# anuragranj/cc

Hardware: AMD Instinct MI355X
Metric: train images/sec (832x256, 5-frame sample, 6-scale CC step) (higher is better)
Workload: dtype f32; 1 GPU; full CC: DispResNet6+PoseNetB6+MaskNet6+Back2Future, all losses; per_gpu_batch=4, global_batch=4, height=256, width=832, scales=6, frames=5, parallelism=dp1, hipgraph=True, trained_nets=all, rccl_ranks=1, dead_occlusion_decoders_elided=False, net_streams=2, pipeline=per_network, grad_chunks=False, deterministic=True

## Files before the change

cc_amd/config.py:

```python
align_corners = False

strict_nan_checks = False

deterministic = True

net_streams = True


grad_chunks = False

bias_table = False

loss_stream = True


class _Debug:
    no_slice_gy = False
    no_wgrad_defer = False
    no_sum_n = False
    no_wgrad_list = False
    no_wgrad_queue = False
    force_comm = False
    capture_mode = "thread_local"
    net_stream_priority = (0, 0, 0)
    chunk_inline = False
    pipe_extra = {}
    pipe_skip_tail = ()
    reduce_trace = None
    library_path = None


debug = _Debug()
```

cc_amd/csrc/conv.hip:

```cpp
#include <stdio.h>
#include <stdlib.h>
#include <stddef.h>
#include <string.h>
#include "cc_common.h"
#include "conv_internal.h"
#include "cc_tools.h"
#include "conv_tail.h"
#include "wino_weights.h"
#include "../../include/ccengine.h"
#include <vector>
#include <string>
#include <mutex>

#ifdef CC_TOOLS
namespace cctiming {
struct Rec { std::string name; double gflop; hipEvent_t e0, e1; };
static std::vector<Rec>* recs = nullptr;
static std::mutex mtx;
Scope::Scope(const char* name, double gflop, hipStream_t st, bool active) : s(st) {
    if (!recs || !active) return;
    hipEvent_t e0 = nullptr;
    (void)hipEventCreate(&e0);
    (void)hipEventCreate(&e1);
    {
// ... 129 lines not shown
    __syncthreads();
    const int l31 = lane & 31, lk = lane >> 5;
    for (int ch = 0; ch < nchunks; ch++) {
        const int buf = ch & 1;
        if (ch + 1 < nchunks) load_chunk((ch + 1) * BK);
#pragma unroll
        for (int ks = 0; ks < BK / 2; ks++) {
            float af[TM], bf[TN];
#pragma unroll
            for (int a = 0; a < TM; a++) af[a] = As[buf][(2 * ks + lk) * AP + wm * WM + a * 32 + l31];
#pragma unroll
            for (int b = 0; b < TN; b++) bf[b] = Bs[buf][(2 * ks + lk) * BN + wn * WN + b * 32 + l31];
#pragma unroll
            for (int a = 0; a < TM; a++)
#pragma unroll
                for (int b = 0; b < TN; b++)
                    acc[a][b] = __builtin_amdgcn_mfma_f32_32x32x2f32(af[a], bf[b], acc[a][b], 0, 0, 0);
        }
        if (ch + 1 < nchunks) store_chunk(buf ^ 1);
        __syncthreads();
    }

    const int y_cs = g.OH * g.OW;
#pragma unroll
    for (int b = 0; b < TN; b++) {
        const long p = p0 + wn * WN + b * 32 + l31;
        if (p >= Ntot) continue;
        const int n = (int)(p / HWt);
        const int t = (int)(p - (long)n * HWt);
        const int ty = t / g.OWt, tx = t - ty * g.OWt;
        const long pix = (long)(g.oy0 + g.so * ty) * g.OW + (g.ox0 + g.so * tx);
        float* yb = g.y + (long)n * g.y_bs + pix;
        const float* rbp = g.res ? g.res + (long)n * g.res_bs + pix : nullptr;
        const float* abp = g.add ? g.add + (long)n * g.add_bs + pix : nullptr;
#pragma unroll
        for (int a = 0; a < TM; a++) {
#pragma unroll
            for (int r = 0; r < 16; r++) {
                const int m = m0 + wm * WM + a * 32 + (r & 3) + 8 * (r >> 2) + 4 * lk;
                if (m < g.M) {
                    float v = acc[a][b][r];
                    if (g.bias) v += g.bias[m];
                    yb[(long)m * y_cs] = conv_tail(v, rbp != nullptr, rbp ? rbp[(long)m * y_cs] : 0.f, g.res_mul, g.act, g.act_a, g.act_b,
                                                   abp ? abp[(long)m * y_cs] : 0.f);
                }
            }
        }
    }
}

constexpr int TH = 4, TW = 32;

struct CP {
    const float* x; const float* wp; const float* zeros; const float* bias; const float* res; float* y; float* part;
    int B, Cin, IH, IW; long x_bs;
    int M, Mpad, Cpad;
    int Rt, St, si, dstep, dy_base, dx_base, ymin, xmin;
    int PH, PWr, PS;
    int tw16;
    int ipt, phi;
    int aligned, shift;
    int OHt, OWt, so, oy0, ox0, OH, OW; long y_bs, res_bs;
    int tiles_x, tiles_y;
    int nsplit, cps; long part_stride;
    int act; float act_a, act_b;
    int res_mul;
    const float* add; long add_bs;
    int vec4;
    int wmajor;
};

__global__ __launch_bounds__(256) void k_repack_w(const float* __restrict__ w, float* __restrict__ wp, float* __restrict__ zeros,
                                                  int M, int Cin, int Mpad, int Cpad, int T, int St, long w_sm, long w_sc,
                                                  int w0, int w_ri, int w_sj) {
    const long e = (long)blockIdx.x * 256 + threadIdx.x;
    if (blockIdx.x == 0 && threadIdx.x < 64) zeros[threadIdx.x] = 0.f;
    const long tot = (long)T * Cpad * Mpad;
    if (e >= tot) return;
    const int m = (int)(e % Mpad);
    const long r = e / Mpad;
    const int c = (int)(r % Cpad), t = (int)(r / Cpad);
    const int i = t / St, j = t - i * St;
    wp[e] = (m < M && c < Cin) ? w[(long)w0 + (long)m * w_sm + (long)c * w_sc + i * w_ri + j * w_sj] : 0.f;
}

__host__ __device__ inline int repack_ct(int T) { const int ct = 72 / T; return ct < 1 ? 1 : (ct > 64 ? 64 : ct); }
inline long repack_blocks(int Mpad, int Cpad, int T) {
    const int ct = repack_ct(T);
    return (long)((Mpad + 63) / 64) * ((Cpad + ct - 1) / ct);
}

template <int TC>
__device__ __forceinline__ void repack_body(const long* __restrict__ d, float* tile, int bid) {
    const float* __restrict__ w = reinterpret_cast<const float*>(d[0]);
    float* __restrict__ wp = reinterpret_cast<float*>(d[1]);
    const int M = (int)d[2], Cin = (int)d[3], Mpad = (int)d[4], Cpad = (int)d[5], St = (int)d[7];
    const int T = TC > 0 ? TC : (int)d[6];
    const long w_sm = d[8], w_sc = d[9], w0 = d[10], w_ri = d[11], w_sj = d[12];
    const int CT = repack_ct(T);
    const int nmt = (Mpad + 63) / 64;
    const int m0 = (bid % nmt) * 64, c0 = (bid / nmt) * CT;
    const int CTT = CT * T, n = 64 * CTT;
    const bool m_slow = w_sm > w_sc;
    for (int e0 = threadIdx.x; e0 < n; e0 += 8 * 256) {
        float v[8];
        int li[8];
#pragma unroll
// ... 216 lines not shown
                                bf[ks][1] = Pl[(4 * ks) * g.PS + (STK ? poff[1] : half)];
                            }
#pragma unroll
                            for (int ks = 0; ks < CK / 4; ks++) {
                                acc16[0] = __builtin_amdgcn_mfma_f32_16x16x4f32(af[ks], bf[ks][0], acc16[0], 0, 0, 0);
                                acc16[1] = __builtin_amdgcn_mfma_f32_16x16x4f32(af[ks], bf[ks][1], acc16[1], 0, 0, 0);
                            }
                            if (++tj == g.St) { tj = 0; ti++; }
                            continue;
                        }
                        const float* Pl = Pb + lk * g.PS + (STK ? 0 : (g.si * (rowstep * row0 + lr)) * g.PWr + g.si * lc) + tapoff;
                        const float* Al = Ab + lk * BM + wm * WM + l31;
                        float af[CK / 2][TM], bf[CK / 2][TN];
#pragma unroll
                        for (int ks = 0; ks < CK / 2; ks++) {
#ifdef CC_ABLATE_LDS
#pragma unroll
                            for (int a = 0; a < TM; a++) af[ks][a] = 1e-3f * (float)((lane & 7) + a);
#pragma unroll
                            for (int b = 0; b < TN; b++) bf[ks][b] = 1e-3f * (float)((lane & 3) + b);
#else
#pragma unroll
                            for (int a = 0; a < TM; a++) af[ks][a] = Al[(2 * ks) * BM + a * 32];
#pragma unroll
                            for (int b = 0; b < TN; b++) bf[ks][b] = Pl[(2 * ks) * g.PS + (STK ? poff[b] : (g.si * rowstep * b) * g.PWr)];
#endif
                        }
#pragma unroll
                        for (int ks = 0; ks < CK / 2; ks++) {
#pragma unroll
                            for (int a = 0; a < TM; a++)
#pragma unroll
                                for (int b = 0; b < TN; b++)
#ifdef CC_ABLATE_MFMA
                                    acc[a][b][0] = fmaf(af[ks][a], bf[ks][b], acc[a][b][0]);
#else
                                    acc[a][b] = __builtin_amdgcn_mfma_f32_32x32x2f32(af[ks][a], bf[ks][b], acc[a][b], 0, 0, 0);
#endif
                        }
                        if (++tj == g.St) { tj = 0; ti++; }
                    }
                }
                CC_WAIT_VMCNT0();
#ifndef CC_ABLATE_BARRIER
                __syncthreads();
#endif
            }
        }
    }

    const int y_cs = g.OH * g.OW;
    if constexpr (BM == 16) {
        const int HWt = g.OHt * g.OWt;
#pragma unroll
        for (int h = 0; h < 2; h++) {
            int ej, ty;
            if (!rowmap(ty0 + rowstep * row0 + (g.tw16 ? h : 0), ej, ty)) continue;
            const int tx = tx0 + (g.tw16 ? 0 : 16 * h) + (lane & 15);
            if (ty >= g.OHt || tx >= g.OWt) continue;
            const int n = STK ? n_tile + ej : n_tile;
            const long pix = (long)(g.oy0 + g.so * ty) * g.OW + (g.ox0 + g.so * tx);
#pragma unroll
            for (int r = 0; r < 4; r++) {
                const int m = m0 + 4 * (lane >> 4) + r;
                if (m >= g.M) continue;
                if (SPLIT == 1 || (SPLIT == 2 && g.nsplit > 1)) {
                    const int Wp16 = g.tiles_x * (g.tw16 ? 16 : TW), Hp16 = g.tiles_y * (g.tw16 ? 8 : TH);
                    g.part[(long)bz_in * g.part_stride + (((long)n * g.M + m) * Hp16 + ty) * Wp16 + tx] = abl_fix(acc16[h][r]);
                } else {
                    float v = abl_fix(acc16[h][r]);
                    if (g.bias) v += g.bias[m];
                    const long o = (long)n * g.y_bs + pix + (long)m * y_cs;
                    const bool hr = g.res != nullptr;
                    g.y[o] = conv_tail(v, hr, hr ? g.res[(long)n * g.res_bs + pix + (long)m * y_cs] : 0.f, g.res_mul, g.act, g.act_a, g.act_b,
                                       g.add ? g.add[(long)n * g.add_bs + pix + (long)m * y_cs] : 0.f);
                }
            }
        }
        return;
    }
    float* Tt = smem + wid * 1024;
    const int c4 = (lane & 7) * 4, rsub = lane >> 3;
    const int lr4 = g.tw16 ? (c4 >> 4) : 0, lc4 = g.tw16 ? (c4 & 15) : c4;
    const int tx = tx0 + lc4;
    const int Wp = g.tiles_x * (g.tw16 ? 16 : TW), Hp = g.tiles_y * (g.tw16 ? 8 : TH);
    const bool split = (SPLIT == 1 || (SPLIT == 2 && g.nsplit > 1));
    const bool vec = g.vec4 != 0;
    auto stage = [&](const f32x16& A) {
#pragma unroll
        for (int r = 0; r < 16; r++) Tt[((r & 3) + 8 * (r >> 2) + 4 * lk) * 32 + l31] = abl_fix(A[r]);
        __builtin_amdgcn_wave_barrier();
    };
    if (split) {
        auto tile = [&](const f32x16& A, const int a, const int b) {
            stage(A);
            int ej, ty;
            const bool rowok = rowmap(ty0 + rowstep * (row0 + b) + lr4, ej, ty);
            const bool live = rowok && ty < g.OHt && tx < g.OWt;
            float* pb = g.part + (long)bz_in * g.part_stride + (((long)(n + ej) * g.M + (m0 + wm * WM + a * 32 + rsub)) * Hp + ty) * Wp + tx;
            const long mstep = (long)8 * Hp * Wp;
#pragma unroll
            for (int k = 0; k < 4; k++) {
                const float4 v = *reinterpret_cast<const float4*>(&Tt[(8 * k + rsub) * 32 + c4]);
                if (m0 + wm * WM + a * 32 + 8 * k + rsub < g.M && live) {
                    *reinterpret_cast<float4*>(pb + k * mstep) = v;
#ifdef CC_ABLATE_STORE
                    *reinterpret_cast<volatile float4*>(pb + k * mstep) = v;
#endif
                }
            }
            __builtin_amdgcn_wave_barrier();
        };
        tile(acc[0][0], 0, 0);
        if constexpr (TN > 1) tile(acc[0][1], 0, 1);
        if constexpr (TM > 1) {
            tile(acc[1][0], 1, 0);
            if constexpr (TN > 1) tile(acc[1][1], 1, 1);
        }
        return;
    }
    const bool hr = g.res != nullptr, ha = g.add != nullptr;
    auto tile = [&](const f32x16& A, const int a, const int b) {
        stage(A);
        int ej, ty;
        const bool rowok = rowmap(ty0 + rowstep * (row0 + b) + lr4, ej, ty);
        const bool inside = rowok && ty < g.OHt && tx < g.OWt;
        const int n = STK ? n_tile + ej : n_tile;
        const long pix = (long)(g.oy0 + g.so * ty) * g.OW + (g.ox0 + g.so * tx);
#pragma unroll
        for (int k = 0; k < 4; k++) {
            const float4 v = *reinterpret_cast<const float4*>(&Tt[(8 * k + rsub) * 32 + c4]);
            const int m = m0 + wm * WM + a * 32 + 8 * k + rsub;
            if (m < g.M && inside) {
                const long o = (long)m * y_cs + pix;
                const float bias = g.bias ? g.bias[m] : 0.f;
                const float v0 = v.x + bias, v1 = v.y + bias, v2 = v.z + bias, v3 = v.w + bias;
                if (vec && tx + 3 < g.OWt) {
                    float4 rr = make_float4(0.f, 0.f, 0.f, 0.f), aa = rr;
                    if (hr) rr = *reinterpret_cast<const float4*>(g.res + (long)n * g.res_bs + o);
                    if (ha) aa = *reinterpret_cast<const float4*>(g.add + (long)n * g.add_bs + o);
                    float4 out;
                    out.x = conv_tail(v0, hr, rr.x, g.res_mul, g.act, g.act_a, g.act_b, aa.x);
                    out.y = conv_tail(v1, hr, rr.y, g.res_mul, g.act, g.act_a, g.act_b, aa.y);
                    out.z = conv_tail(v2, hr, rr.z, g.res_mul, g.act, g.act_a, g.act_b, aa.z);
                    out.w = conv_tail(v3, hr, rr.w, g.res_mul, g.act, g.act_a, g.act_b, aa.w);
                    *reinterpret_cast<float4*>(g.y + (long)n * g.y_bs + o) = out;
#ifdef CC_ABLATE_STORE
                    *reinterpret_cast<volatile float4*>(g.y + (long)n * g.y_bs + o) = out;
#endif
                } else {
                    const long st = g.so;
                    float* yo = g.y + (long)n * g.y_bs + o;
                    const float* ro = hr ? g.res + (long)n * g.res_bs + o : nullptr;
                    const float* ao = ha ? g.add + (long)n * g.add_bs + o : nullptr;
                    yo[0] = conv_tail(v0, hr, hr ? ro[0] : 0.f, g.res_mul, g.act, g.act_a, g.act_b, ao ? ao[0] : 0.f);
                    if (tx + 1 < g.OWt) yo[st] = conv_tail(v1, hr, hr ? ro[st] : 0.f, g.res_mul, g.act, g.act_a, g.act_b, ao ? ao[st] : 0.f);
                    if (tx + 2 < g.OWt) yo[2 * st] = conv_tail(v2, hr, hr ? ro[2 * st] : 0.f, g.res_mul, g.act, g.act_a, g.act_b, ao ? ao[2 * st] : 0.f);
                    if (tx + 3 < g.OWt) yo[3 * st] = conv_tail(v3, hr, hr ? ro[3 * st] : 0.f, g.res_mul, g.act, g.act_a, g.act_b, ao ? ao[3 * st] : 0.f);
                }
            }
        }
        __builtin_amdgcn_wave_barrier();
    };
    tile(acc[0][0], 0, 0);
    if constexpr (TN > 1) tile(acc[0][1], 0, 1);
    if constexpr (TM > 1) {
        tile(acc[1][0], 1, 0);
        if constexpr (TN > 1) tile(acc[1][1], 1, 1);
    }
}

__device__ __forceinline__ void conv_xcd_blocks(int wmajor, int& bx, int& by, int& bz) {
    bx = (int)blockIdx.x; by = (int)blockIdx.y; bz = (int)blockIdx.z;
    if constexpr (!(CC_XCD_MASK & 1)) return;
    if (wmajor < 0) return;
    if (wmajor) {
        const int gx = (int)gridDim.x, gy = (int)gridDim.y;
        const int w = cc_xcd_order(bx + gx * (by + gy * bz), gx * gy * (int)gridDim.z);
        const int r = w / gx;
        bx = w - r * gx;
        bz = r / gy;
        by = r - bz * gy;
    } else {
        bx = cc_xcd_order(bx, (int)gridDim.x);
    }
}

#ifndef CC_PATCH_LB
#define CC_PATCH_LB 4
#endif
template <int BM, int CK, int TPS, int SPLIT>
__global__ __launch_bounds__(256, CC_PATCH_LB) void k_conv_patch(CP g) {
    int bx, by, bz;
    conv_xcd_blocks(g.wmajor, bx, by, bz);
    conv_patch_body<BM, CK, TPS, SPLIT, 0>(g, bx, by, bz);
}
template <int BM, int TPS, int SPLIT>
__global__ __launch_bounds__(256, CC_PATCH_LB) void k_conv_patch_stk(CP g) {
    int bx, by, bz;
    conv_xcd_blocks(g.wmajor, bx, by, bz);
    conv_patch_body<BM, 8, TPS, SPLIT, 1>(g, bx, by, bz);
}

constexpr int MAXCLS = 12;
struct CPM {
    CP c[MAXCLS];
    int n;
    int bx_end[MAXCLS];
    int wmajor;
};

#if defined(__HIP_DEVICE_COMPILE__) && !defined(CC_HIPEMU)
#define CC_MULTI_DESC(a, k) (*(reinterpret_cast<const CP*>((const char*)__builtin_amdgcn_kernarg_segment_ptr() + offsetof(CPM, c)) + (k)))
#else
#define CC_MULTI_DESC(a, k) ((a).c[k])
#endif
#define CC_MULTI_BODY(BM_, CK_, TPS_, STK_)                                                                                   \
    int bx, by, bz;                                                                                                           \
    conv_xcd_blocks(a.wmajor ? 1 : -1, bx, by, bz);        \
    int k = 0, first = 0, end = a.bx_end[0];                                                                                  \
    _Pragma("unroll") for (int q = 0; q < MAXCLS - 1; q++)                                                                    \
        if (q + 1 < a.n && bx >= a.bx_end[q]) { k = q + 1; first = a.bx_end[q]; end = a.bx_end[q + 1]; }                      \
    const CP& g = CC_MULTI_DESC(a, k);                                                                                        \
    if (bz >= g.nsplit || by * BM_ >= g.Mpad) return;                             \
    bx -= first;                                                                                                              \
    if ((CC_XCD_MASK & 1) && !a.wmajor) bx = cc_xcd_order(bx, end - first);                                                   \
    conv_patch_body<BM_, CK_, TPS_, 2, STK_>(g, bx, by, bz);

template <int BM, int CK, int TPS>
__global__ __launch_bounds__(256, CC_PATCH_LB) void k_conv_patch_multi(CPM a) { CC_MULTI_BODY(BM, CK, TPS, 0) }
template <int BM, int TPS>
__global__ __launch_bounds__(256, CC_PATCH_LB) void k_conv_patch_multi_stk(CPM a) { CC_MULTI_BODY(BM, 8, TPS, 1) }

__global__ __launch_bounds__(256) void k_splitk_epilogue(const float* __restrict__ part, int nsplit, long part_stride,
                                                         const float* __restrict__ bias, const float* __restrict__ res,
                                                         float* __restrict__ y, int M, int OHt, int OWt, int so, int oy0,
                                                         int ox0, int OH, int OW, long y_bs, long res_bs, long total,
                                                         int act, float act_a, float act_b, int res_mul,
                                                         const float* add, long add_bs, int Hp, int Wp) {
    const long e = (long)blockIdx.x * 256 + threadIdx.x;
    if (e >= total) return;
    const int HWt = OHt * OWt;
    const long per = (long)M * HWt;
    const int n = (int)(e / per);
    const long r = e - (long)n * per;
    const int m = (int)(r / HWt);
    const int t = (int)(r - (long)m * HWt);
    const int ty = t / OWt, tx = t - ty * OWt;
    const long po = (((long)n * M + m) * Hp + ty) * Wp + tx;
    float v = 0.f;
    {
        for (int k = 0; k < nsplit; k += 8) {
            float p8[8];
#pragma unroll
            for (int u = 0; u < 8; u++) p8[u] = (k + u < nsplit) ? part[(long)(k + u) * part_stride + po] : 0.f;
#pragma unroll
            for (int u = 0; u < 8; u++)
                if (k + u < nsplit) v += p8[u];
        }
    }
    const long o = (long)m * OH * OW + (long)(oy0 + so * ty) * OW + (ox0 + so * tx);
    if (bias) v += bias[m];
    y[(long)n * y_bs + o] = conv_tail(v, res != nullptr, res ? res[(long)n * res_bs + o] : 0.f, res_mul, act, act_a, act_b,
                                      add ? add[(long)n * add_bs + o] : 0.f);
}

struct EPC {
    const float* part; const float* bias; const float* res; const float* add; float* y;
    int nsplit; long part_stride; int OHt, OWt, oy0, ox0; long total;
    int Hp, Wp;
    int M, so, OH, OW; long y_bs, res_bs, add_bs;
    int act; float act_a, act_b;
    int res_mul;
};
struct EPM {
    EPC c[MAXCLS];
    int n;
    int bx_end[MAXCLS];
};

__global__ __launch_bounds__(256) void k_splitk_epilogue_multi(EPM a) {
    int k = 0, first = 0;
#pragma unroll
    for (int q = 0; q < MAXCLS - 1; q++)
        if (q + 1 < a.n && (int)blockIdx.x >= a.bx_end[q]) { k = q + 1; first = a.bx_end[q]; }
    const EPC& c = a.c[k];
    const long e = (long)((int)blockIdx.x - first) * 256 + threadIdx.x;
    if (e >= c.total) return;
    const int HWt = c.OHt * c.OWt;
    const long per = (long)c.M * HWt;
    const int n = (int)(e / per);
    const long r = e - (long)n * per;
    const int m = (int)(r / HWt);
    const int t = (int)(r - (long)m * HWt);
    const int ty = t / c.OWt, tx = t - ty * c.OWt;
    const long po = (((long)n * c.M + m) * c.Hp + ty) * c.Wp + tx;
    float v = 0.f;
    {
        for (int z = 0; z < c.nsplit; z += 8) {
            float p8[8];
#pragma unroll
            for (int u = 0; u < 8; u++) p8[u] = (z + u < c.nsplit) ? c.part[(long)(z + u) * c.part_stride + po] : 0.f;
#pragma unroll
            for (int u = 0; u < 8; u++)
                if (z + u < c.nsplit) v += p8[u];
        }
    }
    const long o = (long)m * c.OH * c.OW + (long)(c.oy0 + c.so * ty) * c.OW + (c.ox0 + c.so * tx);
    if (c.bias) v += c.bias[m];
    c.y[(long)n * c.y_bs + o] = conv_tail(v, c.res != nullptr, c.res ? c.res[(long)n * c.res_bs + o] : 0.f, c.res_mul, c.act, c.act_a, c.act_b,
                                          c.add ? c.add[(long)n * c.add_bs + o] : 0.f);
}


struct ConvPlan {
    bool use_patch;
    int wino;
    ccint::WinoPlan wn;
    int Hp, Wp;
    int tw16;
    int ipt, phi;
    int bm, ck, tps, Mpad, Cpad, PH, PWr, PS, ymin, xmin, tiles_x, tiles_y, nsplit, cps, aligned, shift;
    size_t smem, wp_floats, part_floats;
    int wpad;
    size_t pad_floats;
};


inline long conv_tiles(const GG& g, const ConvPlan& p) { return (long)((g.B + p.ipt - 1) / p.ipt) * p.tiles_x * p.tiles_y; }

inline bool wino_geometry(const GG& g) {
    return g.Rt == 3 && g.St == 3 && g.si == 1 && g.so == 1 && g.oy0 == 0 && g.ox0 == 0 && (g.dstep == 1 || g.dstep == -1) &&
           g.dy0 == -g.dstep && g.dx0 == -g.dstep && g.IH == g.OH && g.IW == g.OW && g.OHt == g.OH && g.OWt == g.OW && g.Cin > 0 &&
           (long)g.B * g.Cin * g.IH * g.IW < (1l << 26);
}

inline ConvPlan plan_conv(const GG& g, int mult = 1) {
    ConvPlan p = {};
    p.ipt = 1;
    if (wino_geometry(g)) {
        const ccint::WinoPlan w = ccint::wino_plan(g.B, g.Cin, g.IH, g.IW, g.M, mult);
        if (w.ok) {
            p.wino = 1;
            p.wn = w;
            p.use_patch = true;
            p.bm = ccwino::WBM; p.ck = ccwino::WCK; p.tps = 1;
            p.Mpad = w.Mpad; p.Cpad = w.Cpad;
            p.nsplit = w.nsplit; p.cps = w.cps;
            p.Hp = w.Hp; p.Wp = w.Wp;
            p.wp_floats = w.u_floats;
            p.part_floats = w.part_floats;
            return p;
        }
        if (!cctools::env_flag("CC_NO_WINO_PAD") && (g.IW % 4) != 0 && g.IH >= 2 && g.M >= cctools::env_int("CC_WINOP_MINM", 256) &&
            g.Cin >= cctools::env_int("CC_WINOP_MINC", 256)) {
            int wp = (g.IW + 3) & ~3;
            while (!(wp / 2 >= 16 || wp / 2 == 8)) wp += 4;
            if (4 * (wp - g.IW) <= wp && (long)g.B * ((g.IH + 1) / 2) * (wp / 2) >= cctools::env_int("CC_WINOP_MINQ", 64)) {
                ccint::WinoPlan wq = ccint::wino_plan(g.B, g.Cin, g.IH, wp, g.M, mult);
                if (wq.ok) {
                    if (wq.nsplit < 2) {
                        if (wq.tile == 2) wq.tile = 1;
                        wq.cps = (wq.nchunk + 1) / 2;
                        wq.nsplit = (wq.nchunk + wq.cps - 1) / wq.cps;
// ... 158 lines not shown
template <int BM, int CK, int TPS>
inline void launch_patch(const CP& c, dim3 grid, size_t smem, hipStream_t s) {
    if constexpr (CK == 8) {
        if (stacked(c)) {
            if (c.nsplit > 1) launch_patch1_stk<BM, TPS, 1>(c, grid, smem, s);
            else launch_patch1_stk<BM, TPS, 0>(c, grid, smem, s);
            return;
        }
    }
    if (c.nsplit > 1) launch_patch1<BM, CK, TPS, 1>(c, grid, smem, s);
    else launch_patch1<BM, CK, TPS, 0>(c, grid, smem, s);
}

template <int BM, int CK, int TPS>
inline void launch_patch(const CPM& c, dim3 grid, size_t smem, hipStream_t s) {
    if constexpr (CK == 8) {
        if (stacked(c)) {
            static bool big = false;
            launch_patch_kernel(&k_conv_patch_multi_stk<BM, TPS>, big, c, grid, smem, s);
            return;
        }
    }
    static bool big = false;
    launch_patch_kernel(&k_conv_patch_multi<BM, CK, TPS>, big, c, grid, smem, s);
}

template <class ARGS>
inline void dispatch_patch(int bm, int ck, int tps, const ARGS& c, dim3 grid, size_t smem, hipStream_t s) {
    if (tps == 3) {
        if (ck == 16) {
            if (bm == 128) launch_patch<128, 16, 3>(c, grid, smem, s);
            else if (bm == 64) launch_patch<64, 16, 3>(c, grid, smem, s);
            else if (bm == 32) launch_patch<32, 16, 3>(c, grid, smem, s);
            else launch_patch<16, 16, 3>(c, grid, smem, s);
        } else {
            if (bm == 128) launch_patch<128, 8, 3>(c, grid, smem, s);
            else if (bm == 64) launch_patch<64, 8, 3>(c, grid, smem, s);
            else if (bm == 32) launch_patch<32, 8, 3>(c, grid, smem, s);
            else launch_patch<16, 8, 3>(c, grid, smem, s);
        }
    } else if (ck == 16) {
        if (bm == 128) launch_patch<128, 16, 1>(c, grid, smem, s);
        else if (bm == 64) launch_patch<64, 16, 1>(c, grid, smem, s);
        else if (bm == 32) launch_patch<32, 16, 1>(c, grid, smem, s);
        else launch_patch<16, 16, 1>(c, grid, smem, s);
    } else {
        if (bm == 128) launch_patch<128, 8, 1>(c, grid, smem, s);
        else if (bm == 64) launch_patch<64, 8, 1>(c, grid, smem, s);
        else if (bm == 32) launch_patch<32, 8, 1>(c, grid, smem, s);
        else launch_patch<16, 8, 1>(c, grid, smem, s);
    }
}

inline CP make_cp(const GG& g, const ConvPlan& p, const float* zeros, const float* wp, float* part) {
    CP c = {};
    c.x = g.x; c.wp = wp; c.zeros = zeros; c.bias = g.bias; c.res = g.res; c.y = g.y; c.part = part;
    c.B = g.B; c.Cin = g.Cin; c.IH = g.IH; c.IW = g.IW; c.x_bs = g.x_bs;
    c.M = g.M; c.Mpad = p.Mpad; c.Cpad = p.Cpad;
    c.Rt = g.Rt; c.St = g.St; c.si = g.si; c.dstep = g.dstep;
    c.dy_base = g.dy0 - p.ymin; c.dx_base = g.dx0 - p.xmin; c.ymin = p.ymin; c.xmin = p.xmin;
    c.PH = p.PH; c.PWr = p.PWr; c.PS = p.PS; c.tw16 = p.tw16; c.ipt = p.ipt; c.phi = p.phi; c.aligned = p.aligned; c.shift = p.shift;
    c.OHt = g.OHt; c.OWt = g.OWt; c.so = g.so; c.oy0 = g.oy0; c.ox0 = g.ox0; c.OH = g.OH; c.OW = g.OW;
    c.y_bs = g.y_bs; c.res_bs = g.res_bs;
    c.tiles_x = p.tiles_x; c.tiles_y = p.tiles_y;
    c.nsplit = p.nsplit; c.cps = p.cps;
    c.part_stride = (long)g.B * g.M * (p.tiles_y * (p.tw16 ? 8 : TH)) * (p.tiles_x * (p.tw16 ? 16 : TW));
    c.act = g.act; c.act_a = g.act_a; c.act_b = g.act_b; c.res_mul = g.res_mul;
    c.add = g.add; c.add_bs = g.add_bs;
#ifndef CC_CONV_WMAJOR
#define CC_CONV_WMAJOR 1
#endif
    c.wmajor = (CC_CONV_WMAJOR && (long)g.M * g.Rt * g.St > (long)g.B * g.IH * g.IW) ? 1 : 0;
    c.vec4 = (g.so == 1) && ((g.OW & 3) == 0) && ((g.ox0 & 3) == 0) && ((((uintptr_t)g.y) & 15) == 0) && ((g.y_bs & 3) == 0) &&
             (!g.res || ((((uintptr_t)g.res) & 15) == 0 && (g.res_bs & 3) == 0)) &&
             (!g.add || ((((uintptr_t)g.add) & 15) == 0 && (g.add_bs & 3) == 0));
    return c;
}

inline ccint::WinoGeom wino_geom(const GG& g) {
    ccint::WinoGeom w = {};
    w.B = g.B; w.Cin = g.Cin; w.H = g.IH; w.W = g.IW; w.x_bs = g.x_bs; w.M = g.M; w.y_bs = g.y_bs; w.res_bs = g.res_bs; w.add_bs = g.add_bs;
    w.act = g.act; w.act_a = g.act_a; w.act_b = g.act_b; w.res_mul = g.res_mul;
    return w;
}

inline void wino_scope_name(const GG& g, const ConvPlan& p, int nprob, char* nm, int cap) {
    int nl = p.wn.tile ? snprintf(nm, cap, "k_wino_f2x3_s<%d, %d>", p.wn.tile, p.nsplit > 1 ? 1 : 0)
                       : snprintf(nm, cap, "k_wino_f2x3<%d>", p.nsplit > 1 ? 1 : 0);
    if (cctools::env_flag("CC_TIMING_DETAIL"))
        snprintf(nm + nl, cap - nl, " %dx[B%d M%d C%d %dx%d%s t9 k%d] wg%d", nprob, g.B, g.M, g.Cin, g.OH, g.OW, p.wpad ? "(pad)" : "", p.nsplit,
                 nprob * p.wn.nqb * p.wn.nmb * p.nsplit);
}

inline double wino_gflop(const GG& g, const ConvPlan& p) { return 2e-9 * 16.0 * g.B * p.wn.TY * p.wn.TX * (double)g.M * g.Cin; }

inline int wino_flip(const GG& g) { return g.dstep < 0 ? 1 : 0; }

struct PadTab { ccint::PadJob j[2 * MAXGRP]; int n, B, W, Wp; long row_end[2 * MAXGRP]; };
__global__ __launch_bounds__(256) void k_pad_rows(PadTab t) {
    const int q4 = t.Wp >> 2;
    const long e = (long)blockIdx.x * 256 + threadIdx.x;
    const long row = e / q4;
    const int c4 = (int)(e - row * q4) * 4;
    int k = 0;
    long first = 0;
#pragma unroll
    for (int q = 0; q < 2 * MAXGRP - 1; q++)
        if (q + 1 < t.n && row >= t.row_end[q]) { k = q + 1; first = t.row_end[q]; }
    if (row >= t.row_end[t.n - 1]) return;
    const ccint::PadJob& j = t.j[k];
    const long r = row - first;
    const int n = (int)(r / j.rows_per_image);
    const long rr = r - (long)n * j.rows_per_image;
    const float* s = j.src + (long)n * j.bs + rr * t.W;
    float4 v;
    v.x = c4 + 0 < t.W ? s[c4 + 0] : 0.f;
    v.y = c4 + 1 < t.W ? s[c4 + 1] : 0.f;
    v.z = c4 + 2 < t.W ? s[c4 + 2] : 0.f;
    v.w = c4 + 3 < t.W ? s[c4 + 3] : 0.f;
    *reinterpret_cast<float4*>(j.dst + (r * t.Wp + c4)) = v;
}
}

void ccint::pad_rows_launch(const PadJob* jobs, int n, int B, int W, int Wp, hipStream_t s) {
    PadTab t = {};
    t.n = n; t.B = B; t.W = W; t.Wp = Wp;
    long rows = 0;
    for (int k = 0; k < n; k++) {
        t.j[k] = jobs[k];
        rows += (long)B * jobs[k].rows_per_image;
        t.row_end[k] = rows;
    }
    const long nf4 = rows * (Wp >> 2);
    hipLaunchKernelGGL(k_pad_rows, dim3((unsigned)((nf4 + 255) / 256)), dim3(256), 0, s, t);
}

namespace {

inline void wino_pad_input(const GG& g, const ConvPlan& p, float* part, hipStream_t s, ccint::WinoProb& pr, ccint::WinoGeom& wg) {
    float* xpad = part + p.part_floats;
    const ccint::PadJob job = {g.x, xpad, g.x_bs, g.Cin * g.IH};
    ccint::pad_rows_launch(&job, 1, g.B, g.IW, p.wpad, s);
    if (cctools::env_flag("CC_WINO_TRACE"))
        fprintf(stderr, "wino padded input: B%d M%d C%d %dx%d -> pitch %d, nsplit %d dstep %d\n", g.B, g.M, g.Cin, g.IH, g.IW, p.wpad, p.nsplit, g.dstep);
    pr.x = xpad;
    wg.W = p.wpad;
    wg.x_bs = (long)g.Cin * g.IH * p.wpad;
}

inline int head_kernel_of(const GG& g, ccint::HeadConv& h) {
    static const int off = cctools::env_int("CC_NO_HEAD_KERNELS", 0);
    if (off == 1 || (g.Cin > 4 && g.M > 4) || g.Cin < 1 || g.Rt != 3 || g.St != 3 || g.si != 1 || g.so != 1 || g.oy0 != 0 || g.ox0 != 0) return 0;
    if (g.OHt != g.OH || g.OWt != g.OW || g.OH != g.IH || g.OW != g.IW || g.w_ri != 3 || g.w_sj != 1) return 0;
    if (!((g.dstep == 1 && g.dy0 == -1 && g.dx0 == -1) || (g.dstep == -1 && g.dy0 == 1 && g.dx0 == 1))) return 0;
    if (g.res_mul && !g.res) return 0;
    h = ccint::HeadConv{g.x, g.w, g.bias, g.res, g.res_mul ? g.add : nullptr, g.y, g.B, g.Cin, g.IH, g.IW, g.M, g.x_bs, g.y_bs, g.res_bs,
                        g.add_bs, g.w_sm, g.w_sc, (long)g.w0, g.dstep, g.act, g.act_a, g.act_b, g.res_mul};
    if (g.Cin <= 4 && off != 3 && ccint::head_conv_thinc_vec(h) != 0) return 1;
    if (g.M <= 4 && off != 2 && ccint::head_conv_thinm_ok(h)) return 2;
    return 0;
}

inline void launch_gg(const GG& g, float* ws, hipStream_t s, const float* prepacked = nullptr, const float* pre_zeros = nullptr) {
    {
        ccint::HeadConv h;
        const int hk = head_kernel_of(g, h);
        if (hk) {
            char nm[96];
            int nl = snprintf(nm, sizeof nm, hk == 1 ? "k_conv_thinc<%d>" : "k_conv_thinm<%d>", hk == 1 ? g.Cin : g.M);
            if (cctools::env_flag("CC_TIMING_DETAIL"))
                snprintf(nm + nl, sizeof nm - nl, " B%d M%d C%d %dx%d t9", g.B, g.M, g.Cin, g.OHt, g.OWt);
            cctiming::Scope tsc(nm, 2e-9 * g.B * g.OHt * g.OWt * (double)g.M * g.Cin * 9, s);
            if (cctools::env_flag("CC_HEAD_TRACE"))
                fprintf(stderr, "head kernel %d: B%d M%d C%d %dx%d dstep %d\n", hk, g.B, g.M, g.Cin, g.OHt, g.OWt, g.dstep);
            if (hk == 1 ? ccint::head_conv_thinc_launch(h, s) : ccint::head_conv_thinm_launch(h, s)) return;
        }
    }
    const ConvPlan p = plan_conv(g);
    if (!p.use_patch || ws == nullptr) { launch_gg_flat(g, s); return; }
    const float* zeros = ws;
    const float* wp = ws + 64;
    float* part = ws + 64 + (prepacked ? 0 : p.wp_floats);
    const int T = g.Rt * g.St;
    if (p.wino) {
        if (!prepacked)
            ccint::wino_weights_launch(g.w, ws + 64, g.M, g.Cin, p.Cpad, p.Mpad, g.w_sm, g.w_sc, g.w0, g.w_ri, g.w_sj, wino_flip(g), s);
        ccint::WinoProb pr = {g.x, prepacked ? prepacked : wp, g.bias, g.res, g.add, g.y, part};
        ccint::WinoGeom wg = wino_geom(g);
        if (p.wpad) wino_pad_input(g, p, part, s, pr, wg);
        bool ok;
        {
            char nm[128];
            wino_scope_name(g, p, 1, nm, sizeof nm);
            cctiming::Scope tsc(nm, wino_gflop(g, p), s);
            ok = ccint::wino_launch(wg, p.wn, &pr, 1, s);
        }
        if (!ok) { launch_gg_flat(g, s); return; }
        if (p.nsplit > 1) {
            const long total = (long)g.B * g.M * g.OHt * g.OWt;
            hipLaunchKernelGGL(k_splitk_epilogue, dim3((unsigned)((total + 255) / 256)), dim3(256), 0, s, (const float*)part,
                               p.nsplit, (long)g.B * g.M * p.Hp * p.Wp, g.bias, g.res, g.y, g.M, g.OHt, g.OWt, g.so, g.oy0, g.ox0, g.OH,
                               g.OW, g.y_bs, g.res_bs, total, g.act, g.act_a, g.act_b, g.res_mul, g.add, g.add_bs, p.Hp, p.Wp);
        }
        return;
    }
    if (prepacked) {
        zeros = pre_zeros;
        wp = prepacked;
    } else {
        hipLaunchKernelGGL(k_repack_w, dim3((unsigned)((p.wp_floats + 255) / 256)), dim3(256), 0, s, g.w, ws + 64, ws, g.M, g.Cin,
                           p.Mpad, p.Cpad, T, g.St, g.w_sm, g.w_sc, g.w0, g.w_ri, g.w_sj);
    }
    const CP c = make_cp(g, p, zeros, wp, part);
    dim3 grid((unsigned)conv_tiles(g, p), (unsigned)(p.Mpad / p.bm), (unsigned)p.nsplit);
    {
        char nm[96];
        int nl = p.ipt > 1 ? snprintf(nm, sizeof nm, "k_conv_patch_stk<%d, %d, %d>", p.bm, p.tps, p.nsplit > 1 ? 1 : 0)
                           : snprintf(nm, sizeof nm, "k_conv_patch<%d, %d, %d, %d>", p.bm, p.ck, p.tps, p.nsplit > 1 ? 1 : 0);
        if (cctools::env_flag("CC_TIMING_DETAIL"))
            snprintf(nm + nl, sizeof nm - nl, " B%d M%d C%d %dx%d t%d k%d wg%d", g.B, g.M, g.Cin, g.OHt, g.OWt, g.Rt * g.St, p.nsplit,
                     (int)(grid.x * grid.y * grid.z));
        cctiming::Scope tsc(nm, 2e-9 * g.B * g.OHt * g.OWt * (double)g.M * g.Cin * g.Rt * g.St, s);
        dispatch_patch(p.bm, p.ck, p.tps, c, grid, p.smem, s);
    }
    if (p.nsplit > 1) {
        const long total = (long)g.B * g.M * g.OHt * g.OWt;
        hipLaunchKernelGGL(k_splitk_epilogue, dim3((unsigned)((total + 255) / 256)), dim3(256), 0, s, (const float*)part,
                           p.nsplit, c.part_stride, g.bias, g.res, g.y, g.M, g.OHt, g.OWt, g.so, g.oy0, g.ox0, g.OH, g.OW,
                           g.y_bs, g.res_bs, total, g.act, g.act_a, g.act_b, g.res_mul, g.add, g.add_bs,
                           p.Hp, p.Wp);
    }
}

struct ClsIn { GG g; ConvPlan p; const float* zeros; const float* wp; float* part; };

inline size_t smem_cls(const ConvPlan& p, int tps) {
    const size_t b = (size_t)(2 * tps * p.ck * p.bm + 2 * p.ck * p.PS) * sizeof(float);
    return (p.bm >= 32 && b < 16384) ? 16384 : b;
}

inline bool same_problem_shape(const GG& a, const GG& b) {
    return a.B == b.B && a.Cin == b.Cin && a.IH == b.IH && a.IW == b.IW && a.x_bs == b.x_bs && a.M == b.M && a.y_bs == b.y_bs &&
           a.res_bs == b.res_bs && a.add_bs == b.add_bs && a.act == b.act && a.act_a == b.act_a && a.act_b == b.act_b &&
           a.res_mul == b.res_mul && a.dstep == b.dstep;
}

inline bool launch_classes(const ClsIn* cs, int n, hipStream_t s, bool idle_taps = false) {
    if (n < 1 || n > MAXCLS) return false;
    {
        int nw = 0;
        for (int k = 0; k < n; k++) nw += cs[k].p.wino ? 1 : 0;

        if (nw) {
            if (nw != n) return false;
            ccint::WinoProb pr[MAXCLS];
            EPM e = {};
            e.n = n;
            int ebx = 0;
            const ConvPlan& p = cs[0].p;
            for (int k = 0; k < n; k++) {
                const GG& g = cs[k].g;
                if (!cs[k].wp || !same_problem_shape(g, cs[0].g) || cs[k].p.nsplit != p.nsplit || cs[k].p.cps != p.cps) {
                    if (cctools::env_flag("CC_WINO_TRACE"))
                        fprintf(stderr, "wino classes declined: k %d wp %p same %d nsplit %d/%d cps %d/%d\n", k, (const void*)cs[k].wp,
                                (int)same_problem_shape(g, cs[0].g), cs[k].p.nsplit, p.nsplit, cs[k].p.cps, p.cps);
                    return false;
                }
                pr[k] = ccint::WinoProb{g.x, cs[k].wp, g.bias, g.res, g.add, g.y, cs[k].part};
                EPC& c = e.c[k];
                c.part = cs[k].part; c.bias = g.bias; c.res = g.res; c.add = g.add; c.y = g.y;
                c.Hp = p.Hp; c.Wp = p.Wp;
                c.part_stride = (long)g.B * g.M * c.Hp * c.Wp;
                c.nsplit = p.nsplit;
                c.OHt = g.OHt; c.OWt = g.OWt; c.oy0 = g.oy0; c.ox0 = g.ox0;
                c.total = p.nsplit > 1 ? (long)g.B * g.M * g.OHt * g.OWt : 0;
                c.M = g.M; c.so = g.so; c.OH = g.OH; c.OW = g.OW; c.y_bs = g.y_bs; c.res_bs = g.res_bs; c.add_bs = g.add_bs;
                c.act = g.act; c.act_a = g.act_a; c.act_b = g.act_b; c.res_mul = g.res_mul;
                ebx += (int)((c.total + 255) / 256);
                e.bx_end[k] = ebx;
            }
            ccint::WinoGeom wg = wino_geom(cs[0].g);
            if (p.wpad) {
                for (int k = 0; k < n; k++)
                    if (cs[k].p.wpad != p.wpad || cs[k].p.part_floats != p.part_floats || !cs[k].part) return false;
                for (int k0 = 0; k0 < n; k0 += 2 * MAXGRP) {
                    ccint::PadJob jobs[2 * MAXGRP];
                    int nj = 0;
                    for (int k = k0; k < n && k < k0 + 2 * MAXGRP; k++) {
                        const GG& g = cs[k].g;
                        float* xpad = cs[k].part + p.part_floats;
                        jobs[nj++] = ccint::PadJob{g.x, xpad, g.x_bs, g.Cin * g.IH};
                        pr[k].x = xpad;
                    }
                    ccint::pad_rows_launch(jobs, nj, cs[0].g.B, cs[0].g.IW, p.wpad, s);
                }
                wg.W = p.wpad;
                wg.x_bs = (long)cs[0].g.Cin * cs[0].g.IH * p.wpad;
                if (cctools::env_flag("CC_WINO_TRACE"))
                    fprintf(stderr, "wino padded input, %d problems: B%d M%d C%d %dx%d -> pitch %d, nsplit %d\n", n, cs[0].g.B, cs[0].g.M,
                            cs[0].g.Cin, cs[0].g.IH, cs[0].g.IW, p.wpad, p.nsplit);
            }
            {
                char nm[128];
                wino_scope_name(cs[0].g, p, n, nm, sizeof nm);
                cctiming::Scope tsc(nm, n * wino_gflop(cs[0].g, p), s);
                if (!ccint::wino_launch(wg, p.wn, pr, n, s)) return false;
            }
            if (p.nsplit > 1) hipLaunchKernelGGL(k_splitk_epilogue_multi, dim3((unsigned)ebx), dim3(256), 0, s, e);
            return true;
        }
    }
    size_t smem = 0;
    int tps = 3, maxsplit = 1, maxy = 1, ref = -1;
    if (cctools::env_int("CC_CONV_IDLE_TAPS", 1)) idle_taps = true;
    for (int k = 0; k < n; k++) {
        const ConvPlan& p = cs[k].p;
        if (cs[k].g.Cin == 0) continue;
        if (ref < 0) ref = k;
        if (!p.use_patch || p.bm != cs[ref].p.bm || p.ck != cs[ref].p.ck || !cs[k].wp) return false;
        if (p.tps != 3 && !(idle_taps && cs[k].g.Rt * cs[k].g.St < 3 && smem_cls(p, 3) <= 80 * 1024)) tps = 1;
        if (p.nsplit > maxsplit) maxsplit = p.nsplit;
        if (p.Mpad / p.bm > maxy) maxy = p.Mpad / p.bm;
    }
    CPM a = {};
    EPM e = {};
    e.n = n;
    int bx = 0, ebx = 0, epi_any = 0, nc = 0;
    double gf = 0;
    for (int k = 0; k < n; k++) {
        const GG& g = cs[k].g;
        const ConvPlan& p = cs[k].p;
        const bool empty = g.Cin == 0;
        EPC& c = e.c[k];
        c.part = empty ? nullptr : cs[k].part; c.bias = g.bias; c.res = g.res; c.add = g.add; c.y = g.y;
        c.Hp = empty ? g.OHt : p.Hp;
        c.Wp = empty ? g.OWt : p.Wp;
        c.part_stride = (long)g.B * g.M * c.Hp * c.Wp;
        c.nsplit = empty ? 0 : p.nsplit;
        c.OHt = g.OHt; c.OWt = g.OWt; c.oy0 = g.oy0; c.ox0 = g.ox0;
        c.total = (empty || p.nsplit > 1) ? (long)g.B * g.M * g.OHt * g.OWt : 0;
        c.M = g.M; c.so = g.so; c.OH = g.OH; c.OW = g.OW; c.y_bs = g.y_bs; c.res_bs = g.res_bs; c.add_bs = g.add_bs;
        c.act = g.act; c.act_a = g.act_a; c.act_b = g.act_b; c.res_mul = g.res_mul;
        ebx += (int)((c.total + 255) / 256);
        e.bx_end[k] = ebx;
        if (c.total) epi_any = 1;
        if (empty) continue;
        const size_t sm = smem_cls(p, tps);
        if (sm > smem) smem = sm;
        a.c[nc] = make_cp(g, p, cs[k].zeros, cs[k].wp, cs[k].part);
        bx += (int)conv_tiles(g, p);
        a.bx_end[nc] = bx;
        nc++;
        gf += 2e-9 * g.B * g.OHt * g.OWt * (double)g.M * g.Cin * g.Rt * g.St;
    }
    a.n = nc;
    {
        double wf = 0, xf = 0;
        for (int k = 0; k < nc; k++) {
            const CP& c = a.c[k];
            wf += (double)c.M * c.Cin * c.Rt * c.St;
            xf += (double)c.B * c.Cin * c.IH * c.IW;
        }
        a.wmajor = (CC_CONV_WMAJOR && wf > xf) ? 1 : 0;
    }
    if (smem > 80 * 1024) return false;
    if (nc > 0) {
        dim3 grid((unsigned)bx, (unsigned)maxy, (unsigned)maxsplit);
        char nm[224];
        int nl = stacked(a) ? snprintf(nm, sizeof nm, "k_conv_patch_multi_stk<%d, %d>", cs[ref].p.bm, tps)
                            : snprintf(nm, sizeof nm, "k_conv_patch_multi<%d, %d, %d>", cs[ref].p.bm, cs[ref].p.ck, tps);
        if (cctools::env_flag("CC_TIMING_DETAIL")) {
            for (int k = 0; k < n && nl < (int)sizeof nm - 48; k++) {
                const GG& g = cs[k].g;
                if (g.Cin == 0) continue;
                int same = 0, first = 1;
                for (int j = 0; j < n; j++) {
                    const GG& h = cs[j].g;
                    const bool eq = h.Cin == g.Cin && h.M == g.M && h.OHt == g.OHt && h.OWt == g.OWt && h.Rt * h.St == g.Rt * g.St &&
                                    cs[j].p.nsplit == cs[k].p.nsplit;
                    if (eq) { same++; if (j < k) first = 0; }
                }
                if (!first) continue;
                nl += snprintf(nm + nl, sizeof nm - nl, " %dx[B%d M%d C%d %dx%d t%d k%d]", same, g.B, g.M, g.Cin, g.OHt, g.OWt,
                               g.Rt * g.St, cs[k].p.nsplit);
            }
            snprintf(nm + nl, sizeof nm - nl, " wg%d", (int)(grid.x * grid.y * grid.z));
        }
        cctiming::Scope tsc(nm, gf, s);
        dispatch_patch(cs[ref].p.bm, cs[ref].p.ck, tps, a, grid, smem, s);
    }
    if (epi_any) hipLaunchKernelGGL(k_splitk_epilogue_multi, dim3((unsigned)ebx), dim3(256), 0, s, e);
    return true;
}

inline bool launch_gg_classes(const GG* gs, int n, int mult, const float* const* zeros, const float* const* wps,
                              float* const* parts, hipStream_t s) {
    if (n < 2 || n > MAXCLS || cctools::env_flag("CC_NO_CLASS_MERGE")) return false;
    ClsIn cs[MAXCLS];
    for (int k = 0; k < n; k++) {
        cs[k].g = gs[k];
        cs[k].p = plan_conv(gs[k], mult);
        cs[k].zeros = zeros[k]; cs[k].wp = wps[k]; cs[k].part = parts[k];
    }
    return launch_classes(cs, n, s);
}

}

extern "C" {

static GG make_fwd(const float* x, const float* w, const float* bias, const float* res, float* y, int B, int Cin, int IH,
                   int IW, long x_bs, int Cout, int R, int S, int stride, int pad, int OH, int OW, long y_bs, long res_bs,
                   int act, float act_a, float act_b) {
    GG g = {};
    g.x = x; g.w = w; g.bias = bias; g.res = res; g.y = y;
    g.B = B; g.Cin = Cin; g.IH = IH; g.IW = IW; g.x_bs = x_bs;
    g.M = Cout; g.w_sm = (long)Cin * R * S; g.w_sc = (long)R * S; g.w0 = 0; g.w_ri = S; g.w_sj = 1;
    g.Rt = R; g.St = S; g.dy0 = -pad; g.dx0 = -pad; g.dstep = 1; g.si = stride;
    g.OHt = OH; g.OWt = OW; g.so = 1; g.oy0 = 0; g.ox0 = 0; g.OH = OH; g.OW = OW; g.y_bs = y_bs; g.res_bs = res_bs;
    g.act = act; g.act_a = act_a; g.act_b = act_b;
    return g;
}

static void fill_desc(const GG& g, const ConvPlan& p, long src, long dst, long* d) {
    if (p.wino) {
        d[0] = src; d[1] = dst; d[2] = g.M; d[3] = g.Cin; d[4] = p.Mpad; d[5] = p.Cpad; d[6] = ccwino::WINO_T; d[7] = wino_flip(g) ? -3 : 3;
        d[8] = g.w_sm; d[9] = g.w_sc; d[10] = g.w0; d[11] = g.w_ri; d[12] = g.w_sj; d[13] = (long)p.wp_floats; d[14] = 0;
        d[15] = ccwino::wino_weight_blocks(p.Mpad, p.Cpad);
        return;
    }
    d[0] = src; d[1] = dst; d[2] = g.M; d[3] = g.Cin; d[4] = p.Mpad; d[5] = p.Cpad; d[6] = (long)g.Rt * g.St; d[7] = g.St;
    d[8] = g.w_sm; d[9] = g.w_sc; d[10] = g.w0; d[11] = g.w_ri; d[12] = g.w_sj; d[13] = (long)p.wp_floats; d[14] = 0;
    d[15] = repack_blocks(p.Mpad, p.Cpad, g.Rt * g.St);
}

size_t cc_conv2d_fwd_pack_floats(int B, int Cin, int IH, int IW, int Cout, int R, int S, int stride, int pad, int OH, int OW) {
    GG g = make_fwd(nullptr, nullptr, nullptr, nullptr, nullptr, B, Cin, IH, IW, 0, Cout, R, S, stride, pad, OH, OW, 0, 0, 0,
                    1.f, 0.f);
    const ConvPlan p = plan_conv(g);
    return (p.use_patch && R * S <= 136) ? 64 + p.wp_floats : 0;
}

int cc_conv2d_fwd_pack_desc(int B, int Cin, int IH, int IW, int Cout, int R, int S, int stride, int pad, int OH, int OW,
                            long src_ptr, long pack_base_ptr, long* desc_out_host) {
    GG g = make_fwd(nullptr, nullptr, nullptr, nullptr, nullptr, B, Cin, IH, IW, 0, Cout, R, S, stride, pad, OH, OW, 0, 0, 0,
                    1.f, 0.f);
    const ConvPlan p = plan_conv(g);
    if (!p.use_patch) return 0;
    fill_desc(g, p, src_ptr, pack_base_ptr + 64 * (long)sizeof(float), desc_out_host);
    return 1;
}

size_t cc_conv2d_fwd_ws_bytes(int B, int Cin, int IH, int IW, int Cout, int R, int S, int stride, int pad, int OH, int OW) {
    GG g = make_fwd(nullptr, nullptr, nullptr, nullptr, nullptr, B, Cin, IH, IW, 0, Cout, R, S, stride, pad, OH, OW, 0, 0, 0,
                    1.f, 0.f);
    return conv_ws_floats(plan_conv(g)) * sizeof(float);
}
// ... 86 lines not shown
            if (!p.use_patch) return 0;
            tot += p.wp_floats;
        }
    return tot;
}

int cc_conv2d_dgrad_pack_desc(int B, int K, int OH, int OW, int C, int R, int S, int stride, int pad, int IH, int IW,
                              long w_k_stride, long w_c_stride, long src_ptr, long pack_base_ptr, long* desc_out_host) {
    int n = 0;
    long off = 64;
    for (int py = 0; py < stride; py++)
        for (int px = 0; px < stride; px++) {
            GG g;
            if (!make_dgrad_class(g, py, px, nullptr, nullptr, nullptr, nullptr, B, K, OH, OW, 0, C, R, S, stride, pad, IH, IW, 0,
                                  w_k_stride, w_c_stride, 0, 1.f, 0.f))
                continue;
            if (g.Cin == 0) continue;
            const ConvPlan p = plan_conv(g);
            if (!p.use_patch) return 0;
            fill_desc(g, p, src_ptr, pack_base_ptr + off * (long)sizeof(float), desc_out_host + 16 * n);
            off += (long)p.wp_floats;
            n++;
        }
    return n;
}

int cc_repack_table(const long* table_dev, int ndesc, long total_blocks, void* stream) {
    if (ndesc <= 0 || total_blocks <= 0) return CC_ERR_ARG;
    hipLaunchKernelGGL(k_repack_table, dim3((unsigned)total_blocks), dim3(256), 0, (hipStream_t)stream, table_dev, ndesc);
    CC_CHECK_LAUNCH();
    return CC_OK;
}

size_t cc_conv2d_dgrad_group_ws_bytes(int G, int B, int K, int OH, int OW, int C, int R, int S, int stride, int pad, int IH, int IW) {
    size_t best = 0;
    for (int mult = 1; mult <= G; mult += (G > 1 ? G - 1 : 1)) {
        size_t wmax = 0, psum = 0;
        for (int py = 0; py < stride; py++)
            for (int px = 0; px < stride; px++) {
                GG g;
                if (!make_dgrad_class(g, py, px, nullptr, nullptr, nullptr, nullptr, B, K, OH, OW, 0, C, R, S, stride, pad, IH, IW,
                                      0, (long)C * R * S, (long)R * S, 0, 1.f, 0.f))
                    continue;
                const ConvPlan p = plan_conv(g, mult);
                if (p.wp_floats > wmax) wmax = p.wp_floats;
                psum += p.part_floats + p.pad_floats;
            }
        const size_t t = 64 + wmax + psum;
        if (t > best) best = t;
    }
    return (size_t)G * best * sizeof(float);
}

static int dgrad_group_impl(int G, const long* gy, const long* w, const long* bias, const long* gx, const long* mul,
                            const long* add, float* ws, const long* prepacked, int B, int K, int OH, int OW, long gy_bs, int C,
                            int R, int S, int stride, int pad, int IH, int IW, long gx_bs, long mul_bs, long add_bs,
                            long w_k_stride, long w_c_stride, int act, float act_a, float act_b, void* stream) {
    if (G <= 0 || G > MAXCLS || B <= 0 || K <= 0 || C <= 0 || stride <= 0) return CC_ERR_ARG;
    hipStream_t s = (hipStream_t)stream;
    const size_t stride_f = cc_conv2d_dgrad_group_ws_bytes(G, B, K, OH, OW, C, R, S, stride, pad, IH, IW) / sizeof(float) / G;
    bool packed = true;
    for (int k = 0; k < G; k++)
        if (!prepacked || !prepacked[k]) packed = false;
    const int ncls = stride * stride;
    if (packed && ws && G * ncls >= 2 && G * ncls <= MAXCLS) {
        GG gs[MAXCLS];
        const float *zeros[MAXCLS], *wps[MAXCLS];
        float* parts[MAXCLS];
        int n = 0;
        bool all = true;
        for (int k = 0; k < G && all; k++) {
            const float* pk = (const float*)prepacked[k];
            long off = 64;
            float* part = ws + k * stride_f + 64;
            for (int py = 0; py < stride && all; py++)
                for (int px = 0; px < stride; px++) {
                    if (!make_dgrad_class(gs[n], py, px, (const float*)gy[k], (const float*)w[k],
                                          bias ? (const float*)bias[k] : nullptr, (float*)gx[k], B, K, OH, OW, gy_bs, C, R, S,
                                          stride, pad, IH, IW, gx_bs, w_k_stride, w_c_stride, act, act_a, act_b,
                                          mul ? (const float*)mul[k] : nullptr, mul_bs)) { all = false; break; }
                    if (add && add[k]) {
                        if (mul && mul[k]) { gs[n].add = (const float*)add[k]; gs[n].add_bs = add_bs; }
                        else { gs[n].res = (const float*)add[k]; gs[n].res_bs = add_bs; gs[n].res_mul = 0; }
                    }
                    const ConvPlan p = plan_conv(gs[n], G);
                    zeros[n] = pk;
                    wps[n] = pk + off;
                    parts[n] = part;
                    off += (long)p.wp_floats;
                    part += p.part_floats;
                    n++;
                }
        }
        if (all && launch_gg_classes(gs, n, G, zeros, wps, parts, s)) {
            CC_CHECK_LAUNCH();
            return CC_OK;
        }
    }
    for (int k = 0; k < G; k++) {
        const float* pk = prepacked ? (const float*)prepacked[k] : nullptr;
        float* wk = ws ? ws + k * stride_f : nullptr;
        long off = 64;
        for (int py = 0; py < stride; py++) {
            for (int px = 0; px < stride; px++) {
                GG g;
                if (!make_dgrad_class(g, py, px, (const float*)gy[k], (const float*)w[k], bias ? (const float*)bias[k] : nullptr,
                                      (float*)gx[k], B, K, OH, OW, gy_bs, C, R, S, stride, pad, IH, IW, gx_bs, w_k_stride,
                                      w_c_stride, act, act_a, act_b, mul ? (const float*)mul[k] : nullptr, mul_bs))
                    continue;
                if (add && add[k]) {
                    if (mul && mul[k]) { g.add = (const float*)add[k]; g.add_bs = add_bs; }
                    else { g.res = (const float*)add[k]; g.res_bs = add_bs; g.res_mul = 0; }
                }
                if (g.Cin == 0) {
                    const long total = (long)g.B * g.M * g.OHt * g.OWt;
                    hipLaunchKernelGGL(k_splitk_epilogue, dim3((unsigned)((total + 255) / 256)), dim3(256), 0, s, (const float*)nullptr,
                                       0, total, g.bias, g.res, g.y, g.M, g.OHt, g.OWt, g.so, g.oy0, g.ox0, g.OH, g.OW, g.y_bs, g.res_bs,
                                       total, g.act, g.act_a, g.act_b, g.res_mul, g.add, g.add_bs, g.OHt, g.OWt);
                } else if (pk) {
                    const ConvPlan p = plan_conv(g);
                    launch_gg(g, wk, s, pk + off, pk);
                    off += (long)p.wp_floats;
                } else {
                    launch_gg(g, wk, s);
                }
            }
        }
    }
    CC_CHECK_LAUNCH();
    return CC_OK;
}

int cc_conv2d_dgrad_group(int G, const long* gy, const long* w, const long* bias, const long* gx, const long* mul, float* ws,
                          const long* prepacked, int B, int K, int OH, int OW, long gy_bs, int C, int R, int S, int stride,
                          int pad, int IH, int IW, long gx_bs, long mul_bs, long w_k_stride, long w_c_stride, int act, float act_a,
                          float act_b, void* stream) {
    return dgrad_group_impl(G, gy, w, bias, gx, mul, nullptr, ws, prepacked, B, K, OH, OW, gy_bs, C, R, S, stride, pad, IH, IW, gx_bs,
                            mul_bs, 0, w_k_stride, w_c_stride, act, act_a, act_b, stream);
}

int cc_conv2d_dgrad_group_add(int G, const long* gy, const long* w, const long* gx, const long* mul, const long* add, float* ws,
                              const long* prepacked, int B, int K, int OH, int OW, long gy_bs, int C, int R, int S, int stride,
                              int pad, int IH, int IW, long gx_bs, long mul_bs, long add_bs, long w_k_stride, long w_c_stride,
                              int act, float act_a, float act_b, void* stream) {
    return dgrad_group_impl(G, gy, w, nullptr, gx, mul, add, ws, prepacked, B, K, OH, OW, gy_bs, C, R, S, stride, pad, IH, IW, gx_bs,
                            mul_bs, add_bs, w_k_stride, w_c_stride, act, act_a, act_b, stream);
}

int cc_conv2d_dgrad(const float* gy, const float* w, const float* bias_or_null, float* gx, float* ws,
                    const float* prepacked_or_null, int B, int K, int OH, int OW, long gy_bs, int C, int R, int S, int stride,
                    int pad, int IH, int IW, long gx_bs, long w_k_stride, long w_c_stride, int act, float act_a, float act_b,
                    void* stream) {
    const long gyp = (long)gy, wp = (long)w, bp = (long)bias_or_null, gxp = (long)gx, pk = (long)prepacked_or_null;
    return cc_conv2d_dgrad_group(1, &gyp, &wp, &bp, &gxp, nullptr, ws, &pk, B, K, OH, OW, gy_bs, C, R, S, stride, pad, IH, IW, gx_bs,
                                 0, w_k_stride, w_c_stride, act, act_a, act_b, stream);
}

constexpr int CL_LONGS = 32;
struct ListCls { ClsIn c; int prob; };

static float bits_to_float(long v) { unsigned u = (unsigned)v; float f; memcpy(&f, &u, 4); return f; }

static int list_classes(int n, const long* d, std::vector<ListCls>& out) {
    for (int i = 0; i < n; i++) {
        const long* r = d + (long)i * CL_LONGS;
        const float act_a = bits_to_float(r[24]), act_b = bits_to_float(r[25]);
        const int B = (int)r[8], Ci = (int)r[9], H0 = (int)r[10], W0 = (int)r[11], Co = (int)r[13], R = (int)r[14], S = (int)r[15];
        const int stride = (int)r[16], pad = (int)r[17], H1 = (int)r[18], W1 = (int)r[19];
        if (B <= 0 || Ci <= 0 || Co <= 0 || R <= 0 || S <= 0 || stride <= 0 || !r[6]) return -1;
        const float* pk = (const float*)r[6];
        if (r[0] == 0) {
            ListCls lc = {};
            lc.c.g = make_fwd((const float*)r[1], (const float*)r[2], (const float*)r[3], (const float*)r[4], (float*)r[5], B, Ci, H0, W0,
                              r[12], Co, R, S, stride, pad, H1, W1, r[20], r[21], (int)r[23], act_a, act_b);
            lc.c.p = plan_conv(lc.c.g);
            lc.c.zeros = pk; lc.c.wp = pk + 64; lc.prob = i;
            out.push_back(lc);
        } else {
            long off = 64;
            for (int py = 0; py < stride; py++)
                for (int px = 0; px < stride; px++) {
                    ListCls lc = {};
                    if (!make_dgrad_class(lc.c.g, py, px, (const float*)r[1], (const float*)r[2], (const float*)r[3], (float*)r[5], B, Ci, H0,
                                          W0, r[12], Co, R, S, stride, pad, H1, W1, r[20], r[26], r[27], (int)r[23], act_a, act_b,
                                          (const float*)r[4], r[21]))
                        continue;
                    lc.c.g.add = (const float*)r[7]; lc.c.g.add_bs = r[22];
                    if (lc.c.g.add && !lc.c.g.res_mul) return -1;
                    lc.c.p = plan_conv(lc.c.g);
                    lc.c.zeros = pk; lc.c.wp = pk + off; lc.prob = i;
                    off += (long)lc.c.p.wp_floats;
                    out.push_back(lc);
                }
        }
    }
    return (int)out.size();
}

static void list_plan_splits(ListCls** cls, int n, int target) {
// ... 196 lines not shown
```

cc_amd/csrc/conv_internal.h:

```cpp
#pragma once
#include <stddef.h>
#include <hip/hip_runtime.h>

namespace cctiming {
#ifdef CC_TOOLS
struct Scope {
    hipEvent_t e1 = nullptr;
    hipStream_t s;
    Scope(const char* name, double gflop, hipStream_t st, bool active = true);
    ~Scope();
};
#else
struct Scope { Scope(const char*, double, hipStream_t, bool = true) {} };
#endif
}

namespace ccint {

constexpr int MAXGRP = 4;
constexpr int BN = 128;
constexpr int BK = 16;
inline int pick_bm(int M) { return M > 64 ? 128 : (M > 32 ? 64 : 32); }

struct PadJob { const float* src; float* dst; long bs; int rows_per_image; };
void pad_rows_launch(const PadJob* jobs, int n, int B, int W, int Wp, hipStream_t s);

constexpr int RD_LONGS = 16;
struct RedSink { long* out; int cap; int n; };
int wgrad_reduce_emit(RedSink* sink, const long* desc, int n, hipStream_t s);
int wgrad_reduce_launch(const long* desc, int n, hipStream_t s);

size_t wgrad_thin_ws_floats(int B, int M, int AH, int AW, int Cin, int R, int S, int si);
bool wgrad_thin_launch(const float* a, const float* x, float* gw, float* ws, int B, int M, int AH, int AW, long a_bs, int Cin,
                       int IH, int IW, long x_bs, int R, int S, int si, int pad, long o_sm, long o_sc, int accumulate, hipStream_t s,
                       RedSink* sink = nullptr);

bool wgrad_thin_park(bool on);
bool wgrad_thin_parking();
double wgrad_thin_parked_gflop();
void wgrad_thin_flush(hipStream_t s);

void wgrad_thin_name(int B, int M, int AH, int AW, int Cin, int IH, int IW, int R, int S, int si, int pad, char* out, int cap);


struct WinoGeom {
    int B, Cin, H, W; long x_bs;
    int M; long y_bs, res_bs, add_bs;
    int act; float act_a, act_b; int res_mul;
};
struct WinoProb { const float* x; const float* U; const float* bias; const float* res; const float* add; float* y; float* part; };
struct WinoPlan {
    int ok;
    int Mpad, Cpad, nchunk;
    int TY, TX, nqb, nmb;
    int nsplit, cps;
    int Hp, Wp;
    size_t u_floats, part_floats;
    int tile;
};
constexpr int WINO_MAXP = 12;
WinoPlan wino_plan(int B, int Cin, int H, int W, int M, int mult);
bool wino_launch(const WinoGeom& g, const WinoPlan& p, const WinoProb* probs, int nprob, hipStream_t s);
void wino_weights_launch(const float* w, float* U, int M, int Cin, int Cpad, int Mpad, long w_sm, long w_sc, long w0, long w_ri,
                         long w_sj, int flip, hipStream_t s);

struct WinoWgradPlan {
    int ok;
    int TX, CPR, CPI, NCH;
    int nmb, ncb, Cp;
    int nsplit, cps;
    size_t ws_floats;
};
WinoWgradPlan wino_wgrad_plan(int B, int M, int H, int W, int Cin, int G, int minq = -1);
WinoWgradPlan wino_wgrad_plan_parked(const WinoWgradPlan& alone, int M);
constexpr int WINO_WGRAD_PARK_CAP = 96;
struct WinoWgradParked {
    struct Desc {
        const float* a; const float* x; float* ws;
        int M, C, H, W; long a_bs, x_bs; unsigned a_bytes, x_bytes;
        int TX, CPR, CPI, NCH, cps, ncb, Cp, nxy, nsplit;
        double gflop;
    };
    Desc d[WINO_WGRAD_PARK_CAP];
    int n;
};
bool wino_wgrad_launch(const WinoWgradPlan& p, const float* const* a, const float* const* x, float* const* ws, int G, int B, int M,
                       int H, int W, long a_bs, int Cin, long x_bs, hipStream_t s, WinoWgradParked* park = nullptr);
void wino_wgrad_launch_parked(WinoWgradParked* c, hipStream_t s);

struct HeadConv {
    const float* x; const float* w; const float* bias; const float* res; const float* add; float* y;
    int B, Cin, H, W, M;
    long x_bs, y_bs, res_bs, add_bs;
    long w_sm, w_sc, w0;
    int dstep;
    int act; float act_a, act_b; int res_mul;
};
int head_conv_thinc_vec(const HeadConv& g);
bool head_conv_thinc_launch(const HeadConv& g, hipStream_t s);
bool head_conv_thinm_ok(const HeadConv& g);
bool head_conv_thinm_launch(const HeadConv& g, hipStream_t s);
struct HeadWgradPlan { int ok, R, nstrips, nblk; size_t ws_floats; };
HeadWgradPlan head_wgrad_plan(int B, int M, int H, int W, int Cin);
bool head_wgrad_launch(const HeadWgradPlan& p, const float* dy, const float* x, float* ws, int B, int M, int H, int W, long dy_bs,
                       int Cin, long x_bs, hipStream_t s);

}
```

cc_amd/csrc/wgrad_reduce.hip:

```cpp
#include "cc_common.h"
#include "conv_internal.h"
#include "../../include/ccengine.h"

namespace {

constexpr int NRD = 32;

struct RD {
    const float* ws; float* gw;
    long o_sm, o_sc;
    int kind, nsplit, accum;
    int p[9];
    int blk_end;
};
struct RT { RD d[NRD]; int n; };

__device__ __forceinline__ void put(float* o, float s, int accum) { *o = accum ? (*o + s) : s; }

__global__ __launch_bounds__(256) void k_wgrad_reduce_table(RT t) {
    __shared__ float4 part[16][16];
    int k = 0, first = 0;
#pragma unroll 1
    for (int q = 0; q + 1 < t.n; q++)
        if ((int)blockIdx.x >= t.d[q].blk_end) { k = q + 1; first = t.d[q].blk_end; }
    const RD& d = t.d[k];
    const int bid = (int)blockIdx.x - first;
    const float* __restrict__ ws = d.ws;
    if (d.kind == 0) {
        const int M = d.p[0], Ntot = d.p[1], RS = d.p[2], St = d.p[3];
        const long tot = (long)M * Ntot;
        if (d.p[6]) {
            const long e = ((long)bid * 256 + threadIdx.x) * 4;
            if (e >= tot) return;
            float4 s = make_float4(0.f, 0.f, 0.f, 0.f);
            for (int z = 0; z < d.nsplit; z += 8) {
                float4 v[8];
#pragma unroll
                for (int u = 0; u < 8; u++)
                    v[u] = (z + u < d.nsplit) ? *(const float4*)(ws + (long)(z + u) * tot + e) : make_float4(0.f, 0.f, 0.f, 0.f);
#pragma unroll
                for (int u = 0; u < 8; u++)
                    if (z + u < d.nsplit) { s.x += v[u].x; s.y += v[u].y; s.z += v[u].z; s.w += v[u].w; }
            }
            float4* o = (float4*)(d.gw + e);
            if (d.accum) { const float4 g = *o; s.x = g.x + s.x; s.y = g.y + s.y; s.z = g.z + s.z; s.w = g.w + s.w; }
            *o = s;
            return;
        }
        const long e = (long)bid * 256 + threadIdx.x;
        if (e >= tot) return;
        float s = 0.f;
        for (int z = 0; z < d.nsplit; z += 8) {
            float v[8];
#pragma unroll
            for (int u = 0; u < 8; u++) v[u] = (z + u < d.nsplit) ? ws[(long)(z + u) * tot + e] : 0.f;
#pragma unroll
            for (int u = 0; u < 8; u++)
                if (z + u < d.nsplit) s += v[u];
        }
        const int m = (int)(e / Ntot), jn = (int)(e - (long)m * Ntot);
        const int c = jn / RS, rem = jn - c * RS;
        const int i = rem / St, j = rem - i * St;
        put(d.gw + (long)m * d.o_sm + (long)c * d.o_sc + i * d.p[4] + j * d.p[5], s, d.accum);
    } else if (d.kind == 1) {
        const int T = d.p[0], M = d.p[1], Cin = d.p[2], Cp32 = d.p[3];
        const long mc = (long)bid * 256 + threadIdx.x;
        const long per = (long)M * Cp32;
        if (mc >= per) return;
        const int c = (int)(mc % Cp32), m = (int)(mc / Cp32);
        if (c >= Cin) return;
        const long tot = (long)T * per;
        float* o = d.gw + (long)m * d.o_sm + (long)c * d.o_sc;
        if (T == 9) {
            float s9[9];
#pragma unroll
            for (int tt = 0; tt < 9; tt++) s9[tt] = 0.f;
            int z = 0;
            for (; z + 2 <= d.nsplit; z += 2) {
                const float* wz = ws + (long)z * tot + mc;
                float v0[9], v1[9];
#pragma unroll
                for (int tt = 0; tt < 9; tt++) { v0[tt] = wz[(long)tt * per]; v1[tt] = wz[tot + (long)tt * per]; }
#pragma unroll
                for (int tt = 0; tt < 9; tt++) { s9[tt] += v0[tt]; s9[tt] += v1[tt]; }
            }
            for (; z < d.nsplit; z++) {
                const float* wz = ws + (long)z * tot + mc;
#pragma unroll
                for (int tt = 0; tt < 9; tt++) s9[tt] += wz[(long)tt * per];
            }
#pragma unroll
            for (int tt = 0; tt < 9; tt++) put(o + tt, s9[tt], d.accum);
        } else {
            for (int tt = 0; tt < T; tt++) {
                float s = 0.f;
                for (int z = 0; z < d.nsplit; z++) s += ws[(long)z * tot + (long)tt * per + mc];
                put(o + tt, s, d.accum);
            }
        }
    } else if (d.kind == 4) {
        const int m = bid * 4 + (threadIdx.x >> 6), lane = threadIdx.x & 63;
        if (m < d.p[0]) {
            float s = 0.f;
            for (int k = lane; k < d.nsplit; k += 64) s += ws[(long)m * d.nsplit + k];
            s = cc::wave_sum(s);
            if (lane == 0) put(d.gw + m, s, d.accum);
        }
    } else {
        const int TS = d.p[0], S = d.p[1], TR = d.p[2], ngc = d.p[3], ngt = d.p[4], M = d.p[5], Cin = d.p[6], R = d.p[7];
        const int npb = d.nsplit;
        const int quarter = bid & 3, ct = bid >> 2;
        const int combo = ct / TS, tt = ct - combo * TS;
        const int sub = threadIdx.x >> 4, q = quarter * 16 + (threadIdx.x & 15);
        float4 s = make_float4(0.f, 0.f, 0.f, 0.f);
        int pb = sub;
        for (; pb + 112 < npb; pb += 128) {
            float4 v[8];
#pragma unroll
            for (int u = 0; u < 8; u++) v[u] = *(const float4*)(ws + (((long)combo * npb + pb + 16 * u) * TS + tt) * 256 + 4 * q);
#pragma unroll
            for (int u = 0; u < 8; u++) { s.x += v[u].x; s.y += v[u].y; s.z += v[u].z; s.w += v[u].w; }
        }
        for (; pb < npb; pb += 16) {
            const float4 v = *(const float4*)(ws + (((long)combo * npb + pb) * TS + tt) * 256 + 4 * q);
            s.x += v.x; s.y += v.y; s.z += v.z; s.w += v.w;
        }
        part[sub][threadIdx.x & 15] = s;
        __syncthreads();
        if (sub == 0) {
            for (int z = 1; z < 16; z++) {
                const float4 v = part[z][threadIdx.x & 15];
                s.x += v.x; s.y += v.y; s.z += v.z; s.w += v.w;
            }
            int cb = combo;
            const int tg = cb % ngt;
            cb /= ngt;
            const int cg = cb % ngc, mg = cb / ngc;
            const int r = tg * TR + tt / S, sc = tt % S;
            const int m = mg * 16 + (q >> 2), c0 = cg * 16 + (q & 3) * 4;
            if (m < M && r < R) {
                float* o = d.gw + (long)m * d.o_sm + (long)r * S + sc;
                const float v[4] = {s.x, s.y, s.z, s.w};
#pragma unroll
                for (int e = 0; e < 4; e++)
                    if (c0 + e < Cin) put(o + (long)(c0 + e) * d.o_sc, v[e], d.accum);
            }
        }
    }
}

long blocks_of(const long* h) {
    switch ((int)h[0]) {
        case 0: return h[13] ? (h[7] * h[8] / 4 + 255) / 256 : (h[7] * h[8] + 255) / 256;
        case 1: return (h[8] * h[10] + 255) / 256;
        case 2: return h[15] * h[7] * 4;
        case 4: return (h[7] + 3) / 4;
        default: return -1;
    }
}

}

namespace ccint {

int wgrad_reduce_launch(const long* desc, int n, hipStream_t s) {
    for (int b = 0; b < n; b += NRD) {
        RT t = {};
        const int m = (n - b) < NRD ? (n - b) : NRD;
        long blk = 0;
        for (int k = 0; k < m; k++) {
            const long* h = desc + (long)(b + k) * RD_LONGS;
            RD& d = t.d[k];
            d.kind = (int)h[0]; d.ws = (const float*)h[1]; d.gw = (float*)h[2]; d.nsplit = (int)h[3]; d.accum = (int)h[4];
            d.o_sm = h[5]; d.o_sc = h[6];
            for (int i = 0; i < 9; i++) d.p[i] = (int)h[7 + i];
            long hv[RD_LONGS];
            for (int i = 0; i < RD_LONGS; i++) hv[i] = h[i];
            if (d.kind == 0) {
                const long tot = h[7] * h[8];
                hv[13] = (d.o_sm == h[8] && d.o_sc == h[9] && h[11] == h[10] && h[12] == 1 && tot % 4 == 0 &&
                          ((uintptr_t)d.ws % 16 == 0) && ((uintptr_t)d.gw % 16 == 0)) ? 1 : 0;
                d.p[6] = (int)hv[13];
            }
            const long nb = blocks_of(hv);
            if (nb <= 0 || !d.ws || !d.gw || d.nsplit <= 0 || blk + nb >= (1l << 31)) return CC_ERR_ARG;
            blk += nb;
            d.blk_end = (int)blk;
        }
        t.n = m;
        hipLaunchKernelGGL(k_wgrad_reduce_table, dim3((unsigned)blk), dim3(256), 0, s, t);
    }
    return CC_OK;
}

int wgrad_reduce_emit(RedSink* sink, const long* desc, int n, hipStream_t s) {
    if (!sink) return wgrad_reduce_launch(desc, n, s);
    if (sink->n + n > sink->cap) return CC_ERR_ARG;
    for (long i = 0; i < (long)n * RD_LONGS; i++) sink->out[(long)sink->n * RD_LONGS + i] = desc[i];
    sink->n += n;
    return CC_OK;
}

}

extern "C" {

int cc_wgrad_reduce_table(const long* desc_host, int n, void* stream) {
    if (!desc_host || n <= 0) return CC_ERR_ARG;
    const int r = ccint::wgrad_reduce_launch(desc_host, n, (hipStream_t)stream);
// ... 7 lines not shown
```

cc_amd/csrc/wino.hip:

```cpp
#include <stddef.h>
#include <stdint.h>
#include <stdio.h>
#include <type_traits>
#include "cc_common.h"
#include "cc_tools.h"
#include "conv_tail.h"
#include "conv_internal.h"
#include "wino_weights.h"

namespace {

using namespace cctail;
using namespace ccwino;

typedef float f32x16 __attribute__((ext_vector_type(16)));

struct WN {
    ccint::WinoProb p[ccint::WINO_MAXP];
    int total, per_prob, nmb;
    int Cin, H, W, HW;
    unsigned x_bytes;
    long x_bs;
    int M;
    long y_bs, res_bs, add_bs;
    int TX, TPI, Q, nchunk, cps;
    long part_stride;
    int Hp, Wp;
    int act;
    float act_a, act_b;
    int res_mul, vec2;
    int mb_major;
};

constexpr int VBLK = 16 * WCK * 64;
constexpr int RROW = 12 * 4, RCH = 4 * RROW, RWAVE = 4 * RCH;
constexpr int WTHREADS = 512;

enum { EPI_LIN = 0, EPI_GRAD = 1, EPI_GEN = 2 };

template <int SPLIT, int EPI, int ABL>
__global__ __launch_bounds__(WTHREADS, 2) void k_wino_f2x3(WN g) {
    HIP_DYNAMIC_SHARED(float, smem)
    float* Us = smem;
    float* Vs = smem + 2 * UBLK;
    float* Rs = smem + 2 * UBLK + 2 * VBLK;

    const int tid = threadIdx.x, lane = tid & 63;
    const int wid = __builtin_amdgcn_readfirstlane(tid >> 6);
    const int st = wid & 3, fh = wid >> 2;
    const int wm = st >> 1, wt = st & 1;
    const int l31 = lane & 31, lk = lane >> 5;

    const int cnt = (int)gridDim.x >> 3;
    const int w = ((int)blockIdx.x & 7) * cnt + ((int)blockIdx.x >> 3);
    if (w >= g.total) return;
    const int prob = w / g.per_prob;
    const int wr = w - prob * g.per_prob;
    int qb, mb;
    if (g.mb_major) { const int nqb = g.per_prob / g.nmb; mb = wr / nqb; qb = wr - mb * nqb; }
    else { qb = wr / g.nmb; mb = wr - qb * g.nmb; }
#if defined(__HIP_DEVICE_COMPILE__) && !defined(CC_HIPEMU)
    const char* ka = (const char*)__builtin_amdgcn_kernarg_segment_ptr();
    const ccint::WinoProb& P = *(reinterpret_cast<const ccint::WinoProb*>(ka + offsetof(WN, p)) + prob);
#else
    const ccint::WinoProb& P = g.p[prob];
#endif
    const int c_beg = (int)blockIdx.z * g.cps;
    int c_end = c_beg + g.cps;
    if (c_end > g.nchunk) c_end = g.nchunk;
    const int odd = (c_end - c_beg) & 1;
    auto dma_U = [&](int kc, int buf) {
        if constexpr (ABL & 4) return;
        const float* src = P.U + ((long)mb * g.nchunk + kc) * UBLK + wid * 1024 + lane * 4;
        CC_GLDS16X4(src, Us + buf * UBLK + wid * 1024);
    };

    if (c_beg < c_end) dma_U(c_beg, odd);
    float bias_w = 0.f;
    if constexpr (!SPLIT) {
        const int mr = mb * WBM + wm * 32 + l31;
        if (P.bias) bias_w = P.bias[mr < g.M ? mr : g.M - 1];
    }

    const int tg = st, qd = fh;
    float* Rw = Rs + wid * RWAVE;
    const int q0 = qb * 64 + 16 * tg;
    int rn[2], riy[2], rxal[2], rlen[2], rjb[2], rxs[2];
    {
        int q = q0;
        int jb = 0;
#pragma unroll
        for (int r = 0; r < 2; r++) {
            const bool v = q < g.Q;
            const int qq = v ? q : 0;
// ... 131 lines not shown
        else CC_WAIT_VMCNT_FENCE(3);
        __builtin_amdgcn_s_waitcnt(0xC07F);
        __builtin_amdgcn_s_barrier();
    };

    if (c_beg < c_end) {
        CC_WAIT_VMCNT0_FENCE();
        read_raw();
#pragma unroll
        for (int b = 0; b < 4; b++) col_step(b);
#pragma unroll
        for (int i = 0; i < 4; i++) row_step(i, odd);
        __builtin_amdgcn_s_waitcnt(0xC07F);
        __builtin_amdgcn_wave_barrier();
#pragma unroll
        for (int i = 0; i < 3; i++) dma_raw(c_beg + 1, i);
        __builtin_amdgcn_s_barrier();
        int kc = c_beg;
        if (odd) {
            stage(I1(), kc);
            kc++;
        }
        for (; kc < c_end; kc += 2) {
            stage(I0(), kc);
            stage(I1(), kc + 1);
        }
    }

    if constexpr (ABL & 32) {
        if (acc[3][5] == 12345.f) P.y[tid] = acc[7][1] + acc[0][0];
        return;
    }
    auto part_tile = [&](int r, float& z00, float& z01, float& z10, float& z11) {
        float p0[4], p1[4];
#pragma unroll
        for (int j = 0; j < 4; j++) {
            if (fh == 0) { p0[j] = acc[j][r] + acc[4 + j][r]; p1[j] = acc[4 + j][r]; }
            else { p0[j] = acc[j][r]; p1[j] = (0.f - acc[j][r]) - acc[4 + j][r]; }
        }
        z00 = (p0[0] + p0[1]) + p0[2];
        z01 = (p0[1] - p0[2]) - p0[3];
        z10 = (p1[0] + p1[1]) + p1[2];
        z11 = (p1[1] - p1[2]) - p1[3];
    };
    const int q = qb * 64 + wt * 32 + l31;
    const bool qv = q < g.Q;
    const int qq = qv ? q : 0;
    const int n = qq / g.TPI;
    const int qr = qq - n * g.TPI;
    const int ty = qr / g.TX, tx = qr - ty * g.TX;
    const int oy = 2 * ty, ox = 2 * tx;
    const int m_base = mb * WBM + wm * 32 + 4 * lk;
    const bool hr = P.res != nullptr, ha = P.add != nullptr;
    const bool row1 = oy + 1 < g.H;
    const long o0 = (long)oy * g.W + ox;
    const int odd_lane = lane & 1;
    const long o4 = (long)(oy + odd_lane) * g.W + (ox - 2 * odd_lane);
    const bool row_ok = odd_lane ? row1 : true;
    float4 res_r[8], add_r[8];
    if constexpr (!SPLIT) {
#pragma unroll
        for (int r8 = 0; r8 < 8; r8++) res_r[r8] = add_r[r8] = make_float4(0.f, 0.f, 0.f, 0.f);
        if (g.vec2 && qv && row_ok) {
            if (hr) {
                const float* rb = P.res + (long)n * g.res_bs + o4;
#pragma unroll
                for (int r8 = 0; r8 < 8; r8++) {
                    const int r = 8 * fh + r8;
                    const int m = m_base + (r & 3) + 8 * (r >> 2);
                    res_r[r8] = *reinterpret_cast<const float4*>(rb + (long)(m < g.M ? m : g.M - 1) * g.HW);
                }
            }
            if (ha) {
                const float* ab = P.add + (long)n * g.add_bs + o4;
#pragma unroll
                for (int r8 = 0; r8 < 8; r8++) {
                    const int r = 8 * fh + r8;
                    const int m = m_base + (r & 3) + 8 * (r >> 2);
                    add_r[r8] = *reinterpret_cast<const float4*>(ab + (long)(m < g.M ? m : g.M - 1) * g.HW);
                }
            }
        }
    }
    float* Xs = smem;
    {
        float* xo = Xs + ((st * 2 + fh) * 32) * 64 + lane;
#pragma unroll
        for (int r8 = 0; r8 < 8; r8++) {
            const int r = 8 * (fh ^ 1) + r8;
            float z00, z01, z10, z11;
            part_tile(r, z00, z01, z10, z11);
            xo[(r8 * 4 + 0) * 64] = z00;
            xo[(r8 * 4 + 1) * 64] = z01;
            xo[(r8 * 4 + 2) * 64] = z10;
            xo[(r8 * 4 + 3) * 64] = z11;
        }
    }
    __syncthreads();
    const float* xi = Xs + ((st * 2 + (fh ^ 1)) * 32) * 64 + lane;
    auto out_tile = [&](int r8, float& y00, float& y01, float& y10, float& y11) {
        part_tile(8 * fh + r8, y00, y01, y10, y11);
        y00 += xi[(r8 * 4 + 0) * 64];
        y01 += xi[(r8 * 4 + 1) * 64];
        y10 += xi[(r8 * 4 + 2) * 64];
        y11 += xi[(r8 * 4 + 3) * 64];
    };
    auto pair4 = [&](float y00, float y01, float y10, float y11) -> float4 {
        const float sx = odd_lane ? y00 : y10, sy = odd_lane ? y01 : y11;
        const float rx = __shfl_xor(sx, 1), ry = __shfl_xor(sy, 1);
        return odd_lane ? make_float4(rx, ry, y10, y11) : make_float4(y00, y01, rx, ry);
    };
    if constexpr (SPLIT) {
        float* pb0 = P.part + (long)blockIdx.z * g.part_stride + (((long)n * g.M) * g.Hp + oy + odd_lane) * g.Wp + (ox - 2 * odd_lane);
        const long mstride = (long)g.Hp * g.Wp;
#pragma unroll
        for (int r8 = 0; r8 < 8; r8++) {
            const int r = 8 * fh + r8;
            const int m = m_base + (r & 3) + 8 * (r >> 2);
            float y00, y01, y10, y11;
            out_tile(r8, y00, y01, y10, y11);
            const float4 v = pair4(y00, y01, y10, y11);
            if (qv && m < g.M) *reinterpret_cast<float4*>(pb0 + (long)m * mstride) = v;
        }
        return;
    }
    const float slope = g.act == ACT_RELU ? 0.f : (g.act == ACT_LRELU ? (g.act_b != 0.f ? g.act_b : 0.2f) : 1.f);
    auto tail = [&](float v, float r, float ad) -> float {
        if constexpr (EPI == EPI_LIN) {
            const float t = v + r;
            return t > 0.f ? t : slope * t + 0.f;
        } else if constexpr (EPI == EPI_GRAD) {
            const float t = v + ad;
            return r > 0.f ? t : slope * t;
        } else {
            return conv_tail(v, hr, r, g.res_mul, g.act, g.act_a, g.act_b, ad);
        }
    };
    if (g.vec2) {
        float* yb = P.y + (long)n * g.y_bs + o4;
#pragma unroll
        for (int r8 = 0; r8 < 8; r8++) {
            const int r = 8 * fh + r8;
            const int m = m_base + (r & 3) + 8 * (r >> 2);
            float y00, y01, y10, y11;
            out_tile(r8, y00, y01, y10, y11);
            const float bv = __shfl(bias_w, 4 * lk + (r & 3) + 8 * (r >> 2));
            float4 v = pair4(y00, y01, y10, y11);
            v.x = tail(v.x + bv, res_r[r8].x, add_r[r8].x);
            v.y = tail(v.y + bv, res_r[r8].y, add_r[r8].y);
            v.z = tail(v.z + bv, res_r[r8].z, add_r[r8].z);
            v.w = tail(v.w + bv, res_r[r8].w, add_r[r8].w);
            if (qv && row_ok && m < g.M) *reinterpret_cast<float4*>(yb + (long)m * g.HW) = v;
        }
        return;
    }
    if (!qv) return;
    const bool col1 = ox + 1 < g.W;
#pragma unroll
    for (int r8 = 0; r8 < 8; r8++) {
        const int r = 8 * fh + r8;
        float y00, y01, y10, y11;
        out_tile(r8, y00, y01, y10, y11);
        const int m = m_base + (r & 3) + 8 * (r >> 2);
        if (m >= g.M) continue;
        const float bv = P.bias ? P.bias[m] : 0.f;
        const long o = (long)m * g.HW + o0;
        float* yo = P.y + (long)n * g.y_bs + o;
        const float* ro = hr ? P.res + (long)n * g.res_bs + o : nullptr;
        const float* ao = ha ? P.add + (long)n * g.add_bs + o : nullptr;
        yo[0] = tail(y00 + bv, hr ? ro[0] : 0.f, ha ? ao[0] : 0.f);
        if (col1) yo[1] = tail(y01 + bv, hr ? ro[1] : 0.f, ha ? ao[1] : 0.f);
        if (row1) {
            yo[g.W] = tail(y10 + bv, hr ? ro[g.W] : 0.f, ha ? ao[g.W] : 0.f);
            if (col1) yo[g.W + 1] = tail(y11 + bv, hr ? ro[g.W + 1] : 0.f, ha ? ao[g.W + 1] : 0.f);
        }
    }
}

constexpr int SBM = 32, SBT = 32;
constexpr int UBLK_S = 16 * WCK * SBM;
constexpr int VBLK_S = 16 * WCK * SBT;
constexpr int SHALF = 2 * UBLK_S + 2 * VBLK_S + 4 * RWAVE;

template <int KS, int SPLIT, int EPI>
__global__ __launch_bounds__(256 * KS, 2) void k_wino_f2x3_s(WN g) {
    HIP_DYNAMIC_SHARED(float, smem)
    const int tid = threadIdx.x, lane = tid & 63;
    const int wid = __builtin_amdgcn_readfirstlane(tid >> 6);
    const int fr = wid & 3, kh = wid >> 2;
    const int l31 = lane & 31, lk = lane >> 5;
    float* Us = smem + kh * SHALF;
    float* Vs = Us + 2 * UBLK_S;
    float* Rs = Vs + 2 * VBLK_S;

    const int cnt = (int)gridDim.x >> 3;
    const int w = ((int)blockIdx.x & 7) * cnt + ((int)blockIdx.x >> 3);
    if (w >= g.total) return;
    const int prob = w / g.per_prob;
    const int wr = w - prob * g.per_prob;
    int qb, mb;
    if (g.mb_major) { const int nqb = g.per_prob / g.nmb; mb = wr / nqb; qb = wr - mb * nqb; }
    else { qb = wr / g.nmb; mb = wr - qb * g.nmb; }
#if defined(__HIP_DEVICE_COMPILE__) && !defined(CC_HIPEMU)
    const char* ka = (const char*)__builtin_amdgcn_kernarg_segment_ptr();
    const ccint::WinoProb& P = *(reinterpret_cast<const ccint::WinoProb*>(ka + offsetof(WN, p)) + prob);
#else
    const ccint::WinoProb& P = g.p[prob];
#endif
    int c_beg = (int)blockIdx.z * g.cps;
    int c_end = c_beg + g.cps;
    if (c_end > g.nchunk) c_end = g.nchunk;
    if constexpr (KS == 2) {
        const int half = (c_end - c_beg) >> 1;
        c_beg += kh * half;
        c_end = c_beg + half;
    }
    const int odd = (c_end - c_beg) & 1;
    unsigned uoff[4];
#pragma unroll
    for (int k = 0; k < 4; k++) uoff[k] = (unsigned)(fr * 8192 + k * 1024 + lk * 1024 + (mb & 1) * 512 + l31 * 16);
    auto dma_U = [&](int kc, int buf) {
        const float* src = P.U + ((long)(mb >> 1) * g.nchunk + kc) * UBLK;
        CC_GLDS16X4_S(src, uoff, Us + buf * UBLK_S + fr * 1024);
    };
    if (c_beg < c_end) dma_U(c_beg, odd);
    float bias_w = 0.f;
    if constexpr (!SPLIT) {
        const int mr = mb * SBM + l31;
        if (P.bias) bias_w = P.bias[mr < g.M ? mr : g.M - 1];
    }

    const int tg = fr & 1, qd = fr >> 1;
    float* Rw = Rs + fr * RWAVE;
    const int q0 = qb * SBT + 16 * tg;
    int rn[2], riy[2], rxal[2], rlen[2], rjb[2], rxs[2];
    {
        int q = q0;
        int jb = 0;
// ... 102 lines not shown
            const int j = i & 3, ks = i >> 2;
            acc[j] = __builtin_amdgcn_mfma_f32_32x32x2f32(av[j][ks], bv[j][ks], acc[j], 0, 0, 0);
            if (i == 0) dma_U(kd, buf ^ 1);
            else if (i == 3) { CC_WAIT_VMCNT_FENCE(4); read_raw(); }
            else if (i >= 4 && i < 12) {
                const int s8 = i - 4;
                if (s8 < 4) col_step(s8);
                else row_step(s8 - 4, buf ^ 1);
            }
            else if (i == 13) { dma_raw(kc + 2, 0); dma_raw(kc + 2, 1); dma_raw(kc + 2, 2); }
            if (i == 0 || (i >= 3 && i < 14)) __builtin_amdgcn_sched_barrier(0);
        }
        __builtin_amdgcn_sched_barrier(0);
        CC_WAIT_VMCNT_FENCE(3);
        __builtin_amdgcn_s_waitcnt(0xC07F);
        __builtin_amdgcn_s_barrier();
    };

    if (c_beg < c_end) {
        CC_WAIT_VMCNT0_FENCE();
        read_raw();
#pragma unroll
        for (int b = 0; b < 4; b++) col_step(b);
#pragma unroll
        for (int i = 0; i < 4; i++) row_step(i, odd);
        __builtin_amdgcn_s_waitcnt(0xC07F);
        __builtin_amdgcn_wave_barrier();
#pragma unroll
        for (int i = 0; i < 3; i++) dma_raw(c_beg + 1, i);
        __builtin_amdgcn_s_barrier();
        int kc = c_beg;
        if (odd) {
            stage(I1(), kc);
            kc++;
        }
        for (; kc < c_end; kc += 2) {
            stage(I0(), kc);
            stage(I1(), kc + 1);
        }
    }
    CC_WAIT_VMCNT0_FENCE();

    constexpr int RPW = 4 / KS;
    const int rbase = 4 * fr + RPW * kh;
    const int q = qb * SBT + l31;
    const bool qv = q < g.Q;
    const int qq = qv ? q : 0;
    const int n = qq / g.TPI;
    const int qr = qq - n * g.TPI;
    const int ty = qr / g.TX, tx = qr - ty * g.TX;
    const int oy = 2 * ty, ox = 2 * tx;
    const int m_base = mb * SBM + 4 * lk + 8 * fr + RPW * kh;
    const bool hr = P.res != nullptr, ha = P.add != nullptr;
    const bool row1 = oy + 1 < g.H;
    const long o0 = (long)oy * g.W + ox;
    const int odd_lane = lane & 1;
    const long o4 = (long)(oy + odd_lane) * g.W + (ox - 2 * odd_lane);
    const bool row_ok = odd_lane ? row1 : true;
    float4 res_r[RPW], add_r[RPW];
    if constexpr (!SPLIT) {
#pragma unroll
        for (int rr = 0; rr < RPW; rr++) res_r[rr] = add_r[rr] = make_float4(0.f, 0.f, 0.f, 0.f);
        if (g.vec2 && qv && row_ok) {
            if (hr) {
                const float* rb = P.res + (long)n * g.res_bs + o4;
#pragma unroll
                for (int rr = 0; rr < RPW; rr++) {
                    const int m = m_base + rr;
                    res_r[rr] = *reinterpret_cast<const float4*>(rb + (long)(m < g.M ? m : g.M - 1) * g.HW);
                }
            }
            if (ha) {
                const float* ab = P.add + (long)n * g.add_bs + o4;
#pragma unroll
                for (int rr = 0; rr < RPW; rr++) {
                    const int m = m_base + rr;
                    add_r[rr] = *reinterpret_cast<const float4*>(ab + (long)(m < g.M ? m : g.M - 1) * g.HW);
                }
            }
        }
    }
    float* Xs = smem;
    __syncthreads();
    {
        float* xo = Xs + ((kh * 4 + fr) * 32) * 64 + lane;
#pragma unroll
        for (int r = 0; r < 16; r++) {
            xo[r * 64] = (acc[0][r] + acc[1][r]) + acc[2][r];
            xo[(16 + r) * 64] = (acc[1][r] - acc[2][r]) - acc[3][r];
        }
    }
    __syncthreads();
    auto out_tile = [&](int rr, float& y00, float& y01, float& y10, float& y11) {
        float pv[4][2];
#pragma unroll
        for (int i = 0; i < 4; i++)
#pragma unroll
            for (int b = 0; b < 2; b++) {
                float v = Xs[((i * 2 + b) * 16 + rbase + rr) * 64 + lane];
                if constexpr (KS == 2) v += Xs[(((4 + i) * 2 + b) * 16 + rbase + rr) * 64 + lane];
                pv[i][b] = v;
            }
        y00 = (pv[0][0] + pv[1][0]) + pv[2][0];
        y01 = (pv[0][1] + pv[1][1]) + pv[2][1];
        y10 = (pv[1][0] - pv[2][0]) - pv[3][0];
        y11 = (pv[1][1] - pv[2][1]) - pv[3][1];
    };
    auto pair4 = [&](float y00, float y01, float y10, float y11) -> float4 {
        const float sx = odd_lane ? y00 : y10, sy = odd_lane ? y01 : y11;
        const float rx = __shfl_xor(sx, 1), ry = __shfl_xor(sy, 1);
        return odd_lane ? make_float4(rx, ry, y10, y11) : make_float4(y00, y01, rx, ry);
    };
    if constexpr (SPLIT) {
        float* pb0 = P.part + (long)blockIdx.z * g.part_stride + (((long)n * g.M) * g.Hp + oy + odd_lane) * g.Wp + (ox - 2 * odd_lane);
        const long mstride = (long)g.Hp * g.Wp;
#pragma unroll
        for (int rr = 0; rr < RPW; rr++) {
            const int m = m_base + rr;
            float y00, y01, y10, y11;
            out_tile(rr, y00, y01, y10, y11);
            const float4 v = pair4(y00, y01, y10, y11);
            if (qv && m < g.M) *reinterpret_cast<float4*>(pb0 + (long)m * mstride) = v;
        }
        return;
    }
    const float slope = g.act == ACT_RELU ? 0.f : (g.act == ACT_LRELU ? (g.act_b != 0.f ? g.act_b : 0.2f) : 1.f);
    auto tail = [&](float v, float r, float ad) -> float {
        if constexpr (EPI == EPI_LIN) {
            const float t = v + r;
            return t > 0.f ? t : slope * t + 0.f;
        } else if constexpr (EPI == EPI_GRAD) {
            const float t = v + ad;
            return r > 0.f ? t : slope * t;
        } else {
            return conv_tail(v, hr, r, g.res_mul, g.act, g.act_a, g.act_b, ad);
        }
    };
    if (g.vec2) {
        float* yb = P.y + (long)n * g.y_bs + o4;
#pragma unroll
        for (int rr = 0; rr < RPW; rr++) {
            const int m = m_base + rr;
            float y00, y01, y10, y11;
            out_tile(rr, y00, y01, y10, y11);
            const float bv = __shfl(bias_w, 4 * lk + 8 * fr + RPW * kh + rr);
            float4 v = pair4(y00, y01, y10, y11);
            v.x = tail(v.x + bv, res_r[rr].x, add_r[rr].x);
            v.y = tail(v.y + bv, res_r[rr].y, add_r[rr].y);
            v.z = tail(v.z + bv, res_r[rr].z, add_r[rr].z);
            v.w = tail(v.w + bv, res_r[rr].w, add_r[rr].w);
            if (qv && row_ok && m < g.M) *reinterpret_cast<float4*>(yb + (long)m * g.HW) = v;
        }
        return;
    }
    if (!qv) return;
    const bool col1 = ox + 1 < g.W;
#pragma unroll
    for (int rr = 0; rr < RPW; rr++) {
        float y00, y01, y10, y11;
        out_tile(rr, y00, y01, y10, y11);
        const int m = m_base + rr;
        if (m >= g.M) continue;
        const float bv = P.bias ? P.bias[m] : 0.f;
        const long o = (long)m * g.HW + o0;
        float* yo = P.y + (long)n * g.y_bs + o;
        const float* ro = hr ? P.res + (long)n * g.res_bs + o : nullptr;
        const float* ao = ha ? P.add + (long)n * g.add_bs + o : nullptr;
        yo[0] = tail(y00 + bv, hr ? ro[0] : 0.f, ha ? ao[0] : 0.f);
        if (col1) yo[1] = tail(y01 + bv, hr ? ro[1] : 0.f, ha ? ao[1] : 0.f);
        if (row1) {
            yo[g.W] = tail(y10 + bv, hr ? ro[g.W] : 0.f, ha ? ao[g.W] : 0.f);
            if (col1) yo[g.W + 1] = tail(y11 + bv, hr ? ro[g.W + 1] : 0.f, ha ? ao[g.W + 1] : 0.f);
        }
    }
}

__global__ __launch_bounds__(256) void k_wino_weights(const float* __restrict__ w, float* __restrict__ U, int M, int Cin, int Cpad,
                                                      long w_sm, long w_sc, long w0, long w_ri, long w_sj, int flip) {
    wino_weight_body(w, U, M, Cin, Cpad, w_sm, w_sc, w0, w_ri, w_sj, flip, (int)blockIdx.x);
}

}

namespace ccint {

WinoPlan wino_plan(int B, int Cin, int H, int W, int M, int mult) {
    WinoPlan p = {};
    if (cctools::env_flag("CC_NO_WINO")) return p;
    const int TY = (H + 1) / 2, TX = (W + 1) / 2;
    const long Q = (long)B * TY * TX;
    if (M < cctools::env_int("CC_WINO_MINM", 32) || Cin < cctools::env_int("CC_WINO_MINC", 24) || Q < cctools::env_int("CC_WINO_MINQ", 48)) return p;
    if (H < 2 || (W % 4) != 0 || !(TX >= 16 || TX == 8)) return p;
    if (Q > (1l << 30)) return p;
    p.ok = 1;
    p.Mpad = ((M + WBM - 1) / WBM) * WBM;
    p.Cpad = ((Cin + WCK - 1) / WCK) * WCK;
    p.nchunk = p.Cpad / WCK;
    p.TY = TY; p.TX = TX;
    p.nqb = (int)((Q + 63) / 64);
    p.nmb = p.Mpad / WBM;
    p.Hp = 2 * TY; p.Wp = 2 * TX;
    p.u_floats = (size_t)16 * p.Cpad * p.Mpad;
    const long mu = mult > 1 ? mult : 1;
    const long blocks = (long)p.nqb * p.nmb * mu;
    p.nsplit = 1;
    p.cps = p.nchunk;
    p.tile = 0;
    const int small_mode = cctools::env_int("CC_WINO_SMALL", 1);
    const int nqb_s = (int)((Q + SBT - 1) / SBT), nmb_s = (M + SBM - 1) / SBM;
    const long blocks_s = (long)nqb_s * nmb_s * mu;
    double best = 1e30;
    auto split_cost = [](int real) { return real > 1 ? 1.0 + 0.25 * real : 0.0; };
    if (small_mode != 2 || blocks_s > (1l << 20)) {
        best = (double)((blocks + 255) / 256) * (p.nchunk + 1.5);
        if (blocks < cctools::env_int("CC_WINO_SPLIT_BELOW", 224) && p.nchunk >= 4) {
            const int cap = p.nchunk / 2 < 16 ? p.nchunk / 2 : 16;
            for (int ns = 2; ns <= cap; ns++) {
                const int cps = (p.nchunk + ns - 1) / ns;
                const int real = (p.nchunk + cps - 1) / cps;
                const double rounds = (double)((blocks * real + 255) / 256);
                const double t = rounds * (cps + 1.5) + split_cost(real);
                if (t < best - 1e-9) { best = t; p.nsplit = real; p.cps = cps; }
            }
        }
    }
    if (small_mode && blocks < cctools::env_int("CC_WINO_SMALL_BELOW", 3000) && blocks_s <= (1l << 20)) {
        const double sst = 0.01 * cctools::env_int("CC_WINO_S_STAGE", 25);
        const double sal = 0.01 * cctools::env_int("CC_WINO_S_ALONE", 42);
        const double sfx = 0.01 * cctools::env_int("CC_WINO_S_FIXED", 100);
        const int only_tile = cctools::env_int("CC_WINO_S_TILE", 0);
        int t_tile = 0, t_ns = 1, t_cps = p.nchunk;
        double t_best = 1e30;
        const int cap = p.nchunk >= 4 ? (p.nchunk / 2 < 16 ? p.nchunk / 2 : 16) : 1;
        for (int ns = 1; ns <= cap; ns++) {
            const int cps = (p.nchunk + ns - 1) / ns;
            const int real = (p.nchunk + cps - 1) / cps;
            const long wgs = blocks_s * real;
            const double t4 = wgs <= 256 ? cps * sal + sfx : (double)((wgs + 511) / 512) * (cps * 2.0 * sst + sfx);
            if (t4 + split_cost(real) < t_best - 1e-9) { t_best = t4 + split_cost(real); t_tile = 1; t_ns = real; t_cps = cps; }
            if (real == 1 && (p.nchunk & 1) == 0 && p.nchunk >= 4 && only_tile != 1) {
                const double t8 = only_tile == 2 ? -1.0 : (double)((wgs + 255) / 256) * ((cps / 2) * 2.0 * sst + sfx + 0.3);
                if (t8 < t_best - 1e-9) { t_best = t8; t_tile = 2; t_ns = 1; t_cps = cps; }
            }
        }
        if (t_best < best || small_mode == 2) { best = t_best; p.tile = t_tile; p.nsplit = t_ns; p.cps = t_cps; }
    }
    if (p.tile) { p.nqb = nqb_s; p.nmb = nmb_s; }
    if (!p.tile && M < 48 && cctools::env_int("CC_WINO_MINM", 32) >= 32) return WinoPlan{};
    p.part_floats = p.nsplit > 1 ? (size_t)p.nsplit * B * M * p.Hp * p.Wp : 0;
    return p;
}

void wino_weights_launch(const float* w, float* U, int M, int Cin, int Cpad, int Mpad, long w_sm, long w_sc, long w0, long w_ri,
                         long w_sj, int flip, hipStream_t s) {
    hipLaunchKernelGGL(k_wino_weights, dim3((unsigned)wino_weight_blocks(Mpad, Cpad)), dim3(256), 0, s, w, U, M, Cin, Cpad, w_sm, w_sc,
                       w0, w_ri, w_sj, flip);
}

bool wino_launch(const WinoGeom& gg, const WinoPlan& p, const WinoProb* probs, int nprob, hipStream_t s) {
    const long xfl = ((long)gg.B - 1) * gg.x_bs + (long)gg.Cin * gg.H * gg.W;
    if ((gg.x_bs % 4) != 0 || xfl * 4 >= (long)CC_BUF_OOB) return false;
    for (int k = 0; k < nprob; k++)
        if (((uintptr_t)probs[k].x % 16) != 0) return false;
    WN a = {};
    for (int k = 0; k < nprob; k++) a.p[k] = probs[k];
    a.per_prob = p.nqb * p.nmb;
    a.total = a.per_prob * nprob;
    a.nmb = p.nmb;
    a.Cin = gg.Cin; a.H = gg.H; a.W = gg.W; a.HW = gg.H * gg.W;
    a.x_bytes = (unsigned)((((long)gg.B - 1) * gg.x_bs + (long)gg.Cin * gg.H * gg.W) * 4);
    a.x_bs = gg.x_bs;
    a.M = gg.M; a.y_bs = gg.y_bs; a.res_bs = gg.res_bs; a.add_bs = gg.add_bs;
    a.TX = p.TX; a.TPI = p.TY * p.TX; a.Q = gg.B * a.TPI; a.nchunk = p.nchunk; a.cps = p.cps;
    a.Hp = p.Hp; a.Wp = p.Wp;
    a.part_stride = (long)gg.B * gg.M * p.Hp * p.Wp;
    a.act = gg.act; a.act_a = gg.act_a; a.act_b = gg.act_b; a.res_mul = gg.res_mul;
    bool v2 = (gg.W % 4 == 0) && (gg.y_bs % 4 == 0) && (gg.res_bs % 4 == 0) && (gg.add_bs % 4 == 0);
    for (int k = 0; k < nprob; k++)
        v2 = v2 && ((((uintptr_t)probs[k].y) | (uintptr_t)probs[k].res | (uintptr_t)probs[k].add | (uintptr_t)probs[k].part) % 16 == 0);
    a.vec2 = v2 ? 1 : 0;
#ifndef CC_WINO_MBMAJOR
#define CC_WINO_MBMAJOR 1
#endif
    a.mb_major = (CC_WINO_MBMAJOR && 16l * gg.M > (long)gg.B * gg.H * gg.W) ? 1 : 0;
    if (cctools::env_flag("CC_WINO_TRACE"))
        fprintf(stderr, "wino: %dx[B%d M%d C%d %dx%d] tile %d nqb %d nmb %d nsplit %d cps %d act %d res_mul %d vec2 %d\n", nprob, gg.B, gg.M,
                gg.Cin, gg.H, gg.W, p.tile, p.nqb, p.nmb, p.nsplit, p.cps, gg.act, gg.res_mul, a.vec2);
    const size_t smem = p.tile ? (size_t)SHALF * p.tile * sizeof(float) : (size_t)(2 * UBLK + 2 * VBLK + 8 * RWAVE) * sizeof(float);
    dim3 grid((unsigned)(((a.total + 7) / 8) * 8), 1, (unsigned)p.nsplit);
    const bool grad = gg.res_mul != 0;
    const int epi = (!grad && (gg.act == ACT_NONE || gg.act == ACT_RELU || gg.act == ACT_LRELU)) ? EPI_LIN
                    : (grad && probs[0].res && (gg.act == ACT_RELU || gg.act == ACT_LRELU)) ? EPI_GRAD : EPI_GEN;
    auto go = [&](auto kern, bool& attr) {
        if (!attr) {
            (void)hipFuncSetAttribute(reinterpret_cast<const void*>(kern), hipFuncAttributeMaxDynamicSharedMemorySize, 160 * 1024);
            attr = true;
        }
        hipLaunchKernelGGL(kern, grid, dim3(WTHREADS), smem, s, a);
    };
    static bool attr_set[4] = {false, false, false, false};
    if (p.tile) {
        static bool attr_s[2][4] = {};
        const unsigned nth = 256u * (unsigned)p.tile;
        auto gos = [&](auto kern, bool& attr) {
            if (!attr) {
                (void)hipFuncSetAttribute(reinterpret_cast<const void*>(kern), hipFuncAttributeMaxDynamicSharedMemorySize, 160 * 1024);
                attr = true;
            }
            hipLaunchKernelGGL(kern, grid, dim3(nth), smem, s, a);
        };
        if (p.tile == 2) {
            if (p.nsplit > 1 || (p.nchunk & 1)) return false;
            if (epi == EPI_LIN) gos(k_wino_f2x3_s<2, 0, EPI_LIN>, attr_s[1][0]);
            else if (epi == EPI_GRAD) gos(k_wino_f2x3_s<2, 0, EPI_GRAD>, attr_s[1][1]);
            else gos(k_wino_f2x3_s<2, 0, EPI_GEN>, attr_s[1][2]);
        } else {
            if (p.nsplit > 1) gos(k_wino_f2x3_s<1, 1, 0>, attr_s[0][3]);
            else if (epi == EPI_LIN) gos(k_wino_f2x3_s<1, 0, EPI_LIN>, attr_s[0][0]);
            else if (epi == EPI_GRAD) gos(k_wino_f2x3_s<1, 0, EPI_GRAD>, attr_s[0][1]);
            else gos(k_wino_f2x3_s<1, 0, EPI_GEN>, attr_s[0][2]);
        }
        return true;
    }
#ifdef CC_TOOLS
    const int abl = cctools::env_int("CC_WINO_ABL", 0);
    static bool attr_abl[16] = {};
    if (abl && p.nsplit == 1 && epi == EPI_LIN) {
        switch (abl) {
            case 1: go(k_wino_f2x3<0, 0, 1>, attr_abl[1]); return true;
            case 2: go(k_wino_f2x3<0, 0, 2>, attr_abl[2]); return true;
            case 3: go(k_wino_f2x3<0, 0, 3>, attr_abl[3]); return true;
            case 4: go(k_wino_f2x3<0, 0, 4>, attr_abl[4]); return true;
            case 7: go(k_wino_f2x3<0, 0, 7>, attr_abl[5]); return true;
            case 8: go(k_wino_f2x3<0, 0, 8>, attr_abl[6]); return true;
            case 16: go(k_wino_f2x3<0, 0, 16>, attr_abl[7]); return true;
            case 23: go(k_wino_f2x3<0, 0, 23>, attr_abl[8]); return true;
            case 32: go(k_wino_f2x3<0, 0, 32>, attr_abl[9]); return true;
            case 64: go(k_wino_f2x3<0, 0, 64>, attr_abl[10]); return true;
            case 128: go(k_wino_f2x3<0, 0, 128>, attr_abl[11]); return true;
            default: break;
        }
    }
#endif
    if (p.nsplit > 1) go(k_wino_f2x3<1, 0, 0>, attr_set[3]);
    else if (epi == EPI_LIN) go(k_wino_f2x3<0, EPI_LIN, 0>, attr_set[0]);
    else if (epi == EPI_GRAD) go(k_wino_f2x3<0, EPI_GRAD, 0>, attr_set[1]);
    else go(k_wino_f2x3<0, EPI_GEN, 0>, attr_set[2]);
    return true;
}

}
```

cc_amd/tape.py:

```python
import ctypes

import torch

from . import config, ops
from ._lib import engine, STREAM

ACT = ops.ACT


def _bs(t):
    return t.stride(0)


def _new(shape, ref):
    return torch.empty(shape, device=ref.device, dtype=torch.float32)


def _dense(t):
    B, C, H, W = t.shape
    st = t.stride()
    return st[3] == 1 and st[2] == W and st[1] == H * W and (B == 1 or st[0] >= C * H * W)



class BnCounters:

    def __init__(self, nets):
        self.mods = [m for n in nets if n is not None for m in n.modules()
                     if getattr(m, "num_batches_tracked", None) is not None and hasattr(m, "running_mean")]
        self.index = {id(m): i for i, m in enumerate(self.mods)}
        self.ran = set()
        self.buf = None
        self.inc = {}
        if self.mods:
            self._adopt()

    def _adopt(self):
        self.buf = torch.stack([m.num_batches_tracked.detach().reshape(()) for m in self.mods]).clone()
        self.inc = {}
        for i, m in enumerate(self.mods):
            m._buffers["num_batches_tracked"] = self.buf[i]

    def begin(self):
        self.ran = set()
        if self.buf is not None and any(m.num_batches_tracked.data_ptr() != self.buf[i].data_ptr() for i, m in enumerate(self.mods)):
            self._adopt()

    def commit(self):
        if self.buf is None or not self.ran:
            return
        key = tuple(sorted(self.index[k] for k in self.ran))
        if key not in self.inc:
            v = torch.zeros(len(self.mods), dtype=self.buf.dtype)
            v[list(key)] = 1
            self.inc[key] = v.to(self.buf.device)
        self.buf.add_(self.inc[key])


BN_COUNTERS = None

NET_DONE = None
NET_MARK = None
TAPS = None

class TT:
    __slots__ = ("t", "act", "act_a", "act_b", "uses", "remaining", "grad", "pend", "pre", "needs", "tapname")

    def __init__(self, t, needs=True, act=0, act_a=1.0, act_b=0.0):
        assert t.dtype == torch.float32 and (t.dim() != 4 or _dense(t)), (tuple(t.shape), t.stride())
        self.t = t
        self.act, self.act_a, self.act_b = act, act_a, act_b
        self.uses = 0
        self.remaining = 0
        self.grad = None
        self.pend = []
        self.pre = False
        self.needs = needs
        self.tapname = None

    def skip(self):
        self.remaining -= 1

    def add_alias(self, g):
        self.remaining -= 1
        if self.needs and g is not None:
            self.pend.append(g)

    def _fold_extra_pend(self):
        if not (len(self.pend) > 1 or (self.pend and self.grad is not None)):
            return
        parts = self.pend
        self.pend = []
        if self.t.dim() == 4 and all(p.dim() == 4 and p.dtype == torch.float32 and _dense(p) and p.shape == self.t.shape for p in parts) \
                and (self.grad is None or _dense(self.grad)) and not ops._dbg.no_sum_n:
            acc = self.grad is not None
            if not acc:
                self.grad = _new(self.t.shape, self.t)
            B, C, H, W = self.t.shape
            for c0 in range(0, len(parts), 8):
                ch = parts[c0:c0 + 8]
                src = (ctypes.c_long * len(ch))(*[p.data_ptr() for p in ch])
                sbs = (ctypes.c_long * len(ch))(*[p.stride(0) if B > 1 else C * H * W for p in ch])
                engine().call("cc_sum_strided", len(ch), ctypes.addressof(src), ctypes.addressof(sbs), self.grad,
                              self.grad.stride(0) if B > 1 else C * H * W, B, C * H * W, int(acc), STREAM)
                acc = True
            return
        while parts:
            g = parts.pop()
            if self.grad is None:
                self.grad = (parts.pop() + g) if parts else g.clone()
            else:
                self.grad.add_(g)

    def from_conv(self, launch, can_mul=True):
        self.remaining -= 1
        if not self.needs:
            return
        self._fold_extra_pend()
        add = self.grad if self.grad is not None else (self.pend.pop() if self.pend else None)
        last = can_mul and self.remaining == 0 and self.act != 0
        if self.grad is None:
            self.grad = _new(self.t.shape, self.t)
        launch(self.grad, add, self.t if last else None)
        if last:
            self.pre = True

    def from_writer(self, write):
        self.remaining -= 1
        if not self.needs:
            return
        if self.grad is None and self.pend:
            self._fold_extra_pend()
            if self.pend:
                self.grad = _new(self.t.shape, self.t)
                self.grad.copy_(self.pend.pop())
        if self.grad is None:
            self.grad = _new(self.t.shape, self.t)
            write(self.grad, False)
        else:
            write(self.grad, True)

    def final(self):
        g, pre = self._final()
        if self.tapname is not None and TAPS is not None:
            TAPS[self.tapname] = (g.detach().clone() if g is not None else None, pre)
        return g, pre

    def _final(self):
        if not self.needs:
            return None, False
        if self.grad is None:
            if not self.pend:
                return None, False
            if len(self.pend) == 1:
                return self.pend[0], False
        self._fold_extra_pend()
        return self.grad, self.pre


class ConcatBuffer:

    def __init__(self, tape, B, chans, H, W, ref):
        self.tape = tape
        self.buf = _new((B, sum(chans), H, W), ref)
        self.offs = [0]
        for c in chans:
            self.offs.append(self.offs[-1] + c)
        self.parts = [None] * len(chans)

    def slot(self, i):
        return self.buf[:, self.offs[i]:self.offs[i + 1]]

    def put(self, i, tt):
        if tt.t.data_ptr() != self.slot(i).data_ptr() or tt.t.stride() != self.slot(i).stride():
            assert tuple(tt.t.shape) == tuple(self.slot(i).shape), (tuple(tt.t.shape), tuple(self.slot(i).shape))
            self.slot(i).copy_(tt.t)
# ... 78 lines not shown
    def _act_bias(self, gs, ys, act, act_a, act_b, biases, ref, targets=None):
        G = len(gs)
        B, C, H, W = gs[0].shape
        want_b = biases is not None and biases[0] is not None and biases[0].requires_grad
        if act == 0 and not want_b:
            return list(gs)
        gbs, acc, tgt = [None] * G, False, None
        if want_b:
            tgt = targets if targets is not None else [self._param_grad(b) for b in biases]
            acc = all(a for _, a in tgt)
            if not acc and any(a for _, a in tgt):
                out = []
                for k in range(G):
                    out += self._act_bias([gs[k]], [ys[k]], act, act_a, act_b, [biases[k]], ref, targets=[tgt[k]])
                return out
            gbs = [t for t, _ in tgt]
        geffs = [_new((B, C, H, W), ref) for _ in range(G)] if act != 0 else [None] * G
        if act == 0 and acc and config.bias_table and ops.wgrad_queue.enabled and not ops._dbg.no_wgrad_defer:
            for g, gb in zip(gs, gbs):
                ops.wgrad_reduces.park_bias(g, gb, B, C, H, W, _bs(g))
            return list(gs)
        gy_bs = _bs(gs[0])
        uniform = all(_bs(g) == gy_bs for g in gs) and (act == 0 or all(_bs(y) == _bs(ys[0]) for y in ys))
        if not uniform:
            out = []
            for k in range(G):
                out += self._act_bias([gs[k]], [ys[k]], act, act_a, act_b, [biases[k]] if want_b else None, ref,
                                      targets=[tgt[k]] if want_b else None)
            return out
        for c0 in range(0, G, 4):
            sl = slice(c0, c0 + 4)
            ops_gys, ops_ys, ops_ge, ops_gb = gs[sl], (ys[sl] if act != 0 else [None] * len(gs[sl])), geffs[sl], gbs[sl]
            n = len(ops_gys)
            a1, a2, a3, a4 = ops._parr(ops_gys), ops._parr(ops_ys), ops._parr(ops_ge), ops._parr(ops_gb)
            ws = ops._ws(self.E.call("cc_act_bwd_ws_bytes", C) * n, ref)
            args = (n, ops._addr(a1), ops._addr(a2) if act != 0 else 0, ops._addr(a3) if act != 0 else 0,
                    ops._addr(a4) if want_b else 0, ws, B, C, H, W, gy_bs, _bs(ops_ys[0]) if act != 0 else C * H * W, C * H * W,
                    act, act_a, act_b, int(acc))
            if want_b and acc and ops.wgrad_queue.enabled and not ops._dbg.no_wgrad_defer:
                ptrs = [t.data_ptr() for t in ops_gb]
                if ops.wgrad_reduces.targets.intersection(ptrs) or len(set(ptrs)) != len(ptrs):
                    ops.wgrad_reduces._cur().flush()
                ops.wgrad_reduces.targets.update(ptrs)
                red = (ctypes.c_long * (16 * n))()
                nred = ctypes.c_int(0)
                self.E.call("cc_act_bwd_bias_group_defer", *args, ctypes.addressof(red), n, ctypes.addressof(nred), STREAM)
                if nred.value:
                    ops.wgrad_reduces.keep.append((ws, ops_gb, ops_gys))
                    ops.wgrad_reduces.desc.extend(red[:16 * nred.value])
            else:
                self.E.call("cc_act_bwd_bias_group", *args, STREAM)
        return geffs if act != 0 else list(gs)

    def _wgrad(self, a_list, x_list, w_list, geom):
        B, M, AH, AW, Cin, IH, IW, R, S, si, pad, o_sm, o_sc = geom
        live = [k for k, w in enumerate(w_list) if w.requires_grad]
        if not live:
            return
        tg = [self._param_grad(w_list[k]) for k in live]
        a_bs, x_bs = _bs(a_list[live[0]]), _bs(x_list[live[0]])
        uniform = all(_bs(a_list[k]) == a_bs and _bs(x_list[k]) == x_bs for k in live)
        if ops.wgrad_queue.enabled and all(acc for _, acc in tg) and all(ops._sink(w_list[k]) is not None for k in live):
            for k, (gw, _) in zip(live, tg):
                ops.wgrad_queue.push(geom + (_bs(a_list[k]), _bs(x_list[k])), a_list[k], x_list[k], gw)
            return
        groups = [live] if (uniform and len({acc for _, acc in tg}) == 1) else [[k] for k in live]
        acc_of = {k: acc for k, (_, acc) in zip(live, tg)}
        gw_of = {k: gw for k, (gw, _) in zip(live, tg)}
        for grp in groups:
            for c0 in range(0, len(grp), 4):
                ch = grp[c0:c0 + 4]
                ops._wgrad_group([a_list[k] for k in ch], [x_list[k] for k in ch], [gw_of[k] for k in ch], x_list[ch[0]], B, M, AH, AW,
                                 _bs(a_list[ch[0]]), Cin, IH, IW, _bs(x_list[ch[0]]), R, S, si, pad, o_sm, o_sc, int(acc_of[ch[0]]))

    def conv(self, x, w, b, stride, pad, act=None, act_a=1.0, act_b=0.0, residual=None, out=None):
        return self.conv_group([x], [w], [b], stride, pad, act, act_a, act_b, [residual] if residual is not None else None,
                               [out] if out is not None else None)[0]

    def conv_group(self, xs, ws_, bs, stride, pad, act=None, act_a=1.0, act_b=0.0, residuals=None, outs=None):
        E = self.E
        G = len(xs)
        act = ACT[act] if not isinstance(act, int) else act
        has_bias = bs is not None and bs[0] is not None
        B, Cin, IH, IW = xs[0].t.shape
        Cout, _, R, S = ws_[0].shape
        OH = (IH + 2 * pad - R) // stride + 1
        OW = (IW + 2 * pad - S) // stride + 1
        ys = [o if o is not None else None for o in outs] if outs is not None else [None] * G
        ys = [y if y is not None else _new((B, Cout, OH, OW), xs[0].t) for y in ys]
        x_bs, y_bs = _bs(xs[0].t), _bs(ys[0])
        rs = [r.t for r in residuals] if residuals is not None else None
        res_bs = _bs(rs[0]) if rs is not None else 0
        uniform = all(_bs(x.t) == x_bs for x in xs) and all(_bs(y) == y_bs for y in ys) and (rs is None or all(_bs(r) == res_bs for r in rs))
        geom = (B, Cin, IH, IW, Cout, R, S, stride, pad, OH, OW)

        def launch(idx):
            n = len(idx)
            wsb = ops._ws(E.call("cc_conv2d_fwd_group_ws_bytes", n, *geom), xs[0].t)
            pks = [ops.packs.get("fwd", ws_[k], geom) for k in idx]
            ax, aw, ab = ops._parr([xs[k].t for k in idx]), ops._parr([ws_[k] for k in idx]), ops._parr([bs[k] if has_bias else None for k in idx])
            ar = ops._parr([rs[k] for k in idx]) if rs is not None else None
            ay, ap = ops._parr([ys[k] for k in idx]), ops._parr(pks)
            E.call("cc_conv2d_fwd_group", n, ops._addr(ax), ops._addr(aw), ops._addr(ab), ops._addr(ar) if ar is not None else 0,
                   ops._addr(ay), wsb, ops._addr(ap), B, Cin, IH, IW, _bs(xs[idx[0]].t), Cout, R, S, stride, pad, OH, OW, _bs(ys[idx[0]]),
                   _bs(rs[idx[0]]) if rs is not None else 0, act, float(act_a), float(act_b), STREAM)
        if uniform:
            launch(list(range(G)))
        else:
            for k in range(G):
                launch([k])
        youts = [self._tt(y, act=act, act_a=float(act_a), act_b=float(act_b)) for y in ys]
        self._use(*xs)
        if residuals is not None:
            self._use(*residuals)
        if not self.record:
            return youts
        xs_, res_ = list(xs), (list(residuals) if residuals is not None else None)

        def bwd():
            fin = [y.final() for y in youts]
            live = [k for k in range(G) if fin[k][0] is not None]
            for k in range(G):
                if k not in live:
                    xs_[k].skip()
                    if res_ is not None:
                        res_[k].skip()
            if not live:
                return
            gz = {}
            for pre in (False, True):
                idx = [k for k in live if fin[k][1] == pre]
                if idx:
                    ge = self._act_bias([fin[k][0] for k in idx], [youts[k].t for k in idx], 0 if pre else act, act_a, act_b,
                                        [bs[k] for k in idx] if has_bias else None, xs_[0].t)
                    for k, g in zip(idx, ge):
                        gz[k] = g
            if res_ is not None:
                for k in live:
                    res_[k].add_alias(gz[k])
            dgeom = (B, Cout, OH, OW, Cin, R, S, stride, pad, IH, IW)
            plan = {}
            for k in live:
                xs_[k].from_conv(lambda gx, add, mul, k=k: plan.__setitem__(k, (gx, add, mul)))
            todo = [k for k in live if k in plan]
            groups, last = [], {}
            for k in todo:
                sg = (plan[k][1] is not None, plan[k][2] is not None, _bs(gz[k]), _bs(plan[k][0]),
                      _bs(plan[k][1]) if plan[k][1] is not None else 0, _bs(xs_[k].t), xs_[k].act, xs_[k].act_a, xs_[k].act_b)
                tgt = plan[k][0].data_ptr()
                first = last.get(tgt, -1) + 1
                for gi in range(first, len(groups)):
                    if groups[gi][0] == sg:
                        groups[gi][1].append(k)
                        last[tgt] = gi
                        break
                else:
                    groups.append((sg, [k]))
                    last[tgt] = len(groups) - 1
            for sg, idx in groups:
                n = len(idx)
                has_add, has_mul = sg[0], sg[1]
                wsb = ops._ws(E.call("cc_conv2d_dgrad_group_ws_bytes", n, *dgeom), xs_[0].t)
                pks = [ops.packs.get("dgrad", ws_[k], dgeom + (Cin * R * S, R * S)) for k in idx]
                a1, a2, a3 = ops._parr([gz[k] for k in idx]), ops._parr([ws_[k] for k in idx]), ops._parr([plan[k][0] for k in idx])
                a4 = ops._parr([plan[k][2] for k in idx]) if has_mul else None
                a5 = ops._parr([plan[k][1] for k in idx]) if has_add else None
                a6 = ops._parr(pks)
                E.call("cc_conv2d_dgrad_group_add", n, ops._addr(a1), ops._addr(a2), ops._addr(a3), ops._addr(a4) if has_mul else 0,
                       ops._addr(a5) if has_add else 0, wsb, ops._addr(a6), B, Cout, OH, OW, sg[2], Cin, R, S, stride, pad, IH, IW,
                       sg[3], sg[5] if has_mul else 0, sg[4], Cin * R * S, R * S, sg[6] if has_mul else 0,
                       sg[7] if has_mul else 1.0, sg[8] if has_mul else 0.0, STREAM)
            self._wgrad([gz[k] for k in live], [xs_[k].t for k in live], [ws_[k] for k in live],
                        (B, Cout, OH, OW, Cin, IH, IW, R, S, stride, pad, Cin * R * S, R * S))

        self._node(bwd)
        return youts

    def conv_transpose(self, x, w, b, stride, pad, out_pad, act=None, act_b=0.0, out=None):
        E = self.E
        act = ACT[act] if not isinstance(act, int) else act
        B, Cin, IH, IW = x.t.shape
        _, Cout, R, S = w.shape
        OH = (IH - 1) * stride - 2 * pad + R + out_pad
        OW = (IW - 1) * stride - 2 * pad + S + out_pad
        y = out if out is not None else _new((B, Cout, OH, OW), x.t)
        tgeom = (B, Cin, IH, IW, Cout, R, S, stride, pad, OH, OW)
        wsb = ops._ws(E.call("cc_conv2d_dgrad_ws_bytes", *tgeom), x.t)
        pk = ops.packs.get("dgrad", w, tgeom + (Cout * R * S, R * S))
        E.call("cc_conv2d_dgrad", x.t, w, b, y, wsb, pk, B, Cin, IH, IW, _bs(x.t), Cout, R, S, stride, pad, OH, OW, _bs(y),
               Cout * R * S, R * S, act, 1.0, float(act_b), STREAM)
        yt = self._tt(y, act=act, act_a=1.0, act_b=float(act_b))
        self._use(x)
        if not self.record:
            return yt

        def bwd():
            g, pre = yt.final()
            if g is None:
                x.skip()
                return
            gz = self._act_bias([g], [yt.t], 0 if pre else act, 1.0, act_b, [b] if b is not None else None, x.t)[0]

            def launch(gx, add, mul):
                fgeom = (B, Cout, OH, OW, Cin, R, S, stride, pad, IH, IW)
                ws2 = ops._ws(E.call("cc_conv2d_fwd_ws_bytes", *fgeom), x.t)
                pk2 = ops.packs.get("fwd", w, fgeom)
                E.call("cc_conv2d_fwd", gz, w, None, add, gx, ws2, pk2, B, Cout, OH, OW, _bs(gz), Cin, R, S, stride, pad, IH, IW, _bs(gx),
                       _bs(add) if add is not None else 0, 0, 1.0, 0.0, STREAM)
                assert mul is None
            x.from_conv(launch, can_mul=False)
            self._wgrad([x.t], [gz], [w], (B, Cin, IH, IW, Cout, OH, OW, R, S, stride, pad, Cout * R * S, R * S))
        self._node(bwd)
        return yt

    def batch_norm(self, x, mod):
        E = self.E
        if not mod.training:
            y = ops.batch_norm(x.t, mod.weight, mod.bias, mod.running_mean, mod.running_var, None, False, mod.momentum, mod.eps)
            yt = self._tt(y)
            self._use(x)
            if self.record:
                def bwd_eval():
                    g, _ = yt.final()
                    if g is None:
                        x.skip()
                        return
                    B, C, H, W = g.shape
                    want_w = mod.weight is not None and mod.weight.requires_grad
                    want_b = mod.bias is not None and mod.bias.requires_grad
                    if want_w or want_b:
                        gw, gb = ops.bn_eval_affine_grads(g.contiguous(), x.t, mod.running_mean, mod.running_var, mod.eps, want_w, want_b)
                        for p_, gp in ((mod.weight, gw), (mod.bias, gb)):
                            if gp is not None:
                                buf, acc = self._param_grad(p_)
                                buf.add_(gp) if acc else buf.copy_(gp)

                    def write(gx, accumulate):
                        dst = gx if not accumulate else torch.empty_like(gx)
                        E.call("cc_bn_eval_fwd", g.contiguous(), mod.weight, None, mod.running_mean, mod.running_var, dst, ops._ws(8 * C, g),
                               B, C, H, W, float(mod.eps), 1, STREAM)
                        if accumulate:
                            gx.add_(dst)
                    x.from_writer(write)
                self._node(bwd_eval)
            return yt
        xt = x.t if x.t.is_contiguous() else x.t.contiguous()
        B, C, H, W = xt.shape
        if B * H * W == 1:
            raise ValueError("Expected more than 1 value per channel when training, got input size %s" % (list(xt.shape),))
        if mod.num_batches_tracked is not None:
            if BN_COUNTERS is not None and id(mod) in BN_COUNTERS.index:
                BN_COUNTERS.ran.add(id(mod))
            else:
                mod.num_batches_tracked.add_(1)
        y = torch.empty_like(xt)
        mean = torch.empty(C, device=xt.device, dtype=torch.float32)
# ... 112 lines not shown
        return yt

    def crop(self, x, H, W):
        if x.t.shape[2] == H and x.t.shape[3] == W:
            return x
        y = x.t[:, :, :H, :W].contiguous()
        yt = self._tt(y, act=x.act, act_a=x.act_a, act_b=x.act_b)
        self._use(x)
        if self.record:
            def bwd():
                g, pre = yt.final()
                if g is None:
                    x.skip()
                    return
                if pre:
                    raise RuntimeError("crop: gradient already passed through the activation")

                def write(gx, acc):
                    if not acc:
                        gx.zero_()
                    gx[:, :, :H, :W].add_(g)
                x.from_writer(write)
            yt.act = 0
            self._node(bwd)
        return yt

    def torch_fn(self, xs, fn):
        if not self.record:
            with torch.no_grad():
                return [self._tt(y) for y in fn(*[x.t for x in xs])]
        ins = [x.t.detach().requires_grad_(True) for x in xs]
        with torch.enable_grad():
            ys = list(fn(*ins))
        outs = [self._tt(y.detach()) for y in ys]
        self._use(*xs)

        def bwd():
            pairs = [(y, o.final()[0]) for y, o in zip(ys, outs)]
            pairs = [(y, g) for y, g in pairs if g is not None and y.requires_grad]
            if not pairs:
                for x in xs:
                    x.skip()
                return
            gs = torch.autograd.grad([y for y, _ in pairs], ins, [g for _, g in pairs], allow_unused=True)
            for x, g in zip(xs, gs):
                x.add_alias(g.contiguous()) if (g is not None and x.needs) else x.skip()
        self._node(bwd)
        return outs

    def backward(self, outputs, grads):
        assert self.record
        for tt in self.tts:
            tt.remaining = tt.uses
            tt.grad, tt.pend, tt.pre = None, [], False
        for o, g in zip(outputs, grads):
            if g is not None:
                o.pend.append(g if (g.dim() != 4 or _dense(g)) else g.contiguous())
        for fn in reversed(self.nodes):
            fn()


class _NetFn(torch.autograd.Function):
    @staticmethod
    def forward(ctx, body, n_in, *tensors):
        need = ctx.needs_input_grad[2:]
        tape = Tape(record=any(need))
        tape.owner = getattr(body, "__self__", None)
        ins = [tape.leaf(t, needs=need[i]) for i, t in enumerate(tensors[:n_in])]
        outs = body(tape, *ins)
        ctx.tape, ctx.ins, ctx.outs, ctx.n_in, ctx.body = tape, ins, outs, n_in, body
        ctx.params = tensors[n_in:]
        ctx.set_materialize_grads(False)
        return tuple(o.t for o in outs)

    @staticmethod
    def backward(ctx, *gouts):
        tape = ctx.tape
        tape.backward(ctx.outs, gouts)
        gin = [tt.final()[0] if tt.needs else None for tt in ctx.ins]
        gpar = []
        for p in ctx.params:
            ent = tape.param_grads.get(id(p))
            gpar.append(ent[1] if ent is not None else None)
        ctx.tape = None
        if NET_DONE is not None:
            NET_DONE(getattr(ctx.body, "__self__", None))
        return (None, None) + tuple(gin) + tuple(gpar)


def run_network(body, inputs, params):
    return _NetFn.apply(body, len(inputs), *inputs, *params)
```

include/ccengine.h:

```cpp
#ifndef CCENGINE_H
#define CCENGINE_H
#include <stddef.h>
#ifdef __cplusplus
extern "C" {
#endif

size_t cc_version(void);


int cc_pixel2cam(const float* depth, const float* Kinv, float* cam, int B, int H, int W, void* stream);
int cc_cam2pixel(const float* cam, const float* P, float* grid, int B, int H, int W, int has_rot, int has_tr, int rewrite_oob,
                 void* stream);
int cc_pixel2cam_bwd(const float* g, const float* depth, const float* Kinv, float* gdepth_or_null, float* gKinv12, float* ws_partials,
                     int B, int H, int W, void* stream);
int cc_cam2pixel_bwd(const float* ggrid, const float* cam, const float* P, float* gcam_or_null, float* gP, float* ws_partials, int B,
                     int H, int W, int has_rot, int has_tr, int rewrite_oob, void* stream);

size_t cc_warp_partials_bytes(int B, int H, int W);

int cc_inverse_warp_fwd(const float* img, const float* depth, const float* P, const float* Kinv, float* out,
                        int B, int C, int H, int W, int padding_border, int align_corners, void* stream);

int cc_inverse_warp_bwd(const float* gout, const float* img, const float* depth, const float* P,
                        const float* Kinv, float* gdepth, float* gP, float* gimg_or_null, float* ws_partials,
// ... 71 lines not shown
                             const float* target_bwd, const float* target_fwd, float* gmask_or_null, float* partials,
                             float* loss_accum, float thresh, float wbce, float gscale, int B, int H, int W,
                             void* stream);
int cc_sum_strided(int n, const long* src, const long* src_bs, float* out, long out_bs, int B, long chw, int accumulate,
                   void* stream);
int cc_scale_by_scalar(const float* a, const float* scalar_dev, float* out, int n, void* stream);
int cc_scale_acc_jobs(const long* jobs_host, int njobs, const float* scalar_dev, void* stream);

int cc_corr9x9_fwd(const float* f1, const float* f2, float* out, const int* chan_of_disp_or_null, int B, int C, int H,
                   int W, int out_channels_total, int out_channel_offset, void* stream);
int cc_corr9x9_bwd(const float* gout, const float* f1, const float* f2, float* g1, float* g2_or_null,
                   const int* chan_of_disp_or_null, int B, int C, int H, int W, int g_channels_total,
                   int g_channel_offset, int accumulate_g1, void* stream);
int cc_corr_patch_fwd(const float* f1, const float* f2, float* out, int B, int C, int H, int W, int patch, int dilation,
                      void* stream);
int cc_corr_patch_bwd(const float* gout, const float* f1, const float* f2, float* g1_or_null, float* g2_or_null, int B, int C,
                      int H, int W, int patch, int dilation, void* stream);

size_t cc_conv2d_fwd_ws_bytes(int B, int Cin, int IH, int IW, int Cout, int R, int S, int stride, int pad, int OH, int OW);
int cc_conv2d_fwd(const float* x, const float* w, const float* bias_or_null, const float* res_or_null, float* y, float* ws,
                  const float* prepacked_or_null, int B, int Cin, int IH, int IW, long x_bs, int Cout, int R, int S, int stride,
                  int pad, int OH, int OW, long y_bs, long res_bs, int act, float act_a, float act_b, void* stream);
size_t cc_conv2d_dgrad_ws_bytes(int B, int K, int OH, int OW, int C, int R, int S, int stride, int pad, int IH, int IW);
int cc_conv2d_dgrad(const float* gy, const float* w, const float* bias_or_null, float* gx, float* ws,
                    const float* prepacked_or_null, int B, int K, int OH, int OW, long gy_bs, int C, int R, int S, int stride,
                    int pad, int IH, int IW, long gx_bs, long w_k_stride, long w_c_stride, int act, float act_a, float act_b,
                    void* stream);
size_t cc_conv2d_fwd_pack_floats(int B, int Cin, int IH, int IW, int Cout, int R, int S, int stride, int pad, int OH, int OW);
int cc_conv2d_fwd_pack_desc(int B, int Cin, int IH, int IW, int Cout, int R, int S, int stride, int pad, int OH, int OW,
                            long src_ptr, long pack_base_ptr, long* desc_out_host);
size_t cc_conv2d_dgrad_pack_floats(int B, int K, int OH, int OW, int C, int R, int S, int stride, int pad, int IH, int IW,
                                   long w_k_stride, long w_c_stride);
int cc_conv2d_dgrad_pack_desc(int B, int K, int OH, int OW, int C, int R, int S, int stride, int pad, int IH, int IW,
                              long w_k_stride, long w_c_stride, long src_ptr, long pack_base_ptr, long* desc_out_host);
int cc_repack_table(const long* table_dev, int ndesc, long total_blocks, void* stream);
size_t cc_conv2d_wgrad_ws_bytes(int B, int M, int AH, int AW, int Cin, int R, int S, int si);
int cc_conv2d_wgrad(const float* a, const float* x, float* gw, float* ws, int B, int M, int AH, int AW, long a_bs, int Cin,
                    int IH, int IW, long x_bs, int R, int S, int si, int pad, long o_sm, long o_sc, int accumulate,
                    void* stream);
size_t cc_conv2d_fwd_group_ws_bytes(int G, int B, int Cin, int IH, int IW, int Cout, int R, int S, int stride, int pad, int OH,
                                    int OW);
int cc_conv2d_fwd_group(int G, const long* x, const long* w, const long* bias, const long* res, const long* y, float* ws,
                        const long* prepacked, int B, int Cin, int IH, int IW, long x_bs, int Cout, int R, int S, int stride,
                        int pad, int OH, int OW, long y_bs, long res_bs, int act, float act_a, float act_b, void* stream);
size_t cc_conv2d_dgrad_group_ws_bytes(int G, int B, int K, int OH, int OW, int C, int R, int S, int stride, int pad, int IH, int IW);
int cc_conv2d_dgrad_group(int G, const long* gy, const long* w, const long* bias, const long* gx, const long* mul, float* ws,
                          const long* prepacked, int B, int K, int OH, int OW, long gy_bs, int C, int R, int S, int stride,
                          int pad, int IH, int IW, long gx_bs, long mul_bs, long w_k_stride, long w_c_stride, int act, float act_a,
                          float act_b, void* stream);
int cc_conv2d_dgrad_group_add(int G, const long* gy, const long* w, const long* gx, const long* mul, const long* add, float* ws,
                              const long* prepacked, int B, int K, int OH, int OW, long gy_bs, int C, int R, int S, int stride,
                              int pad, int IH, int IW, long gx_bs, long mul_bs, long add_bs, long w_k_stride, long w_c_stride,
                              int act, float act_a, float act_b, void* stream);
int cc_conv2d_wgrad_group(int G, const long* a, const long* x, const long* gw, float* ws, int B, int M, int AH, int AW, long a_bs,
                          int Cin, int IH, int IW, long x_bs, int R, int S, int si, int pad, long o_sm, long o_sc, int accumulate,
                          void* stream);
int cc_conv2d_wgrad_group_defer(int G, const long* a, const long* x, const long* gw, float* ws, int B, int M, int AH, int AW,
                                long a_bs, int Cin, int IH, int IW, long x_bs, int R, int S, int si, int pad, long o_sm, long o_sc,
                                int accumulate, const float* zeros64_or_null, long* red_host, int red_cap, int* nred_host,
                                void* stream);
int cc_wgrad_reduce_table(const long* desc_host, int n, void* stream);
int cc_conv2d_wgrad_list(int n, const long* desc_host, const float* zeros64_or_null, long* red_host, int red_cap, int* nred_host,
                         void* stream);
int cc_act_bwd_bias_group(int G, const long* gy, const long* y, const long* geff, const long* gbias, float* ws, int B, int C, int H,
                          int W, long gy_bs, long y_bs, long geff_bs, int act, float act_a, float act_b, int accumulate_bias,
                          void* stream);
size_t cc_conv2d_list_ws_bytes(int n, const long* desc_host, int split_target);
int cc_conv2d_list(int n, const long* desc_host, float* ws, int split_target, void* stream);
int cc_is_tools_build(void);
int cc_timing_enable(int on);
int cc_timing_collect(void* out_host, int cap);
int cc_conv2d_fwd_kernel(int B, int Cin, int IH, int IW, int Cout, int R, int S, int stride, int pad, int OH, int OW,
                         void* name_out_host, int cap);
int cc_conv2d_dgrad_kernel(int B, int K, int OH, int OW, int C, int R, int S, int stride, int pad, int IH, int IW,
                           int prepacked, void* name_out_host, int cap);
int cc_conv2d_wgrad_kernel(int B, int M, int AH, int AW, int Cin, int IH, int IW, int R, int S, int si, int pad,
                           void* name_out_host, int cap);
size_t cc_act_bwd_ws_bytes(int C);
int cc_act_bwd_bias_group_defer(int G, const long* gy, const long* y, const long* geff, const long* gbias, float* ws, int B, int C,
                                int H, int W, long gy_bs, long y_bs, long geff_bs, int act, float act_a, float act_b,
                                int accumulate_bias, long* red_host, int red_cap, int* nred_host, void* stream);
int cc_bias_grad_defer(const float* gy, float* gbias, float* ws, int B, int C, int H, int W, long gy_bs, int accumulate,
                       long* job_host, long* red_host, int* nred_host);
int cc_bias_grad_table(const long* jobs_host, int n, void* stream);
int cc_act_bwd_bias(const float* gy, const float* y_or_null, float* geff_or_null, float* gbias_or_null, float* ws, int B,
                    int C, int H, int W, long gy_bs, long y_bs, long geff_bs, int act, float act_a, float act_b,
                    int accumulate_bias, void* stream);

int cc_frames_to_tensor(const void* src, int src_is_u8, float* dst, const int* geo, int N, int H, int W, int h, int w, float mean0,
                        float mean1, float mean2, float std0, float std1, float std2, void* stream);
size_t cc_frames_resize_ws_bytes(int N, int H, int tmp_w);
int cc_frames_resize_to_tensor(const void* src, int src_is_u8, float* dst, const int* geo, const int* tab, int KT, void* ws, int N,
                               int H, int W, int tmp_w, int max_sw, int h, int w, float mean0, float mean1, float mean2, float std0,
                               float std1, float std2, void* stream);
size_t cc_frames_rotate_ws_bytes(int N);
int cc_frames_rotate(const void* src, int src_is_u8, void* dst_u8, const double* rot, void* ws, int N, int H, int W, void* stream);

size_t cc_bn_ws_bytes(int C);
int cc_bn_train_fwd(const float* x, const float* weight_or_null, const float* bias_or_null, float* running_mean_or_null,
                    float* running_var_or_null, float* y, float* save_mean, float* save_invstd, float* ws, int B, int C,
                    int H, int W, float momentum, float eps, void* stream);
int cc_bn_train_bwd(const float* gy, const float* x, const float* weight_or_null, const float* save_mean,
                    const float* save_invstd, float* gx, float* gweight_or_null, float* gbias_or_null, float* ws, int B, int C,
                    int H, int W, int accumulate_wb, void* stream);
int cc_bn_eval_fwd(const float* x, const float* weight_or_null, const float* bias_or_null, const float* running_mean,
                   const float* running_var, float* y, float* ws, int B, int C, int H, int W, float eps, int grad_only,
// ... 79 lines not shown
```

Measured before the change: 248.8 images/s.

## Fuse bias-gradient partial sums into data-gradient conv epilogues

The data-gradient conv kernels (patch, Winograd and split-K epilogues) now write per-channel partial sums of their outputs into a side buffer. The bias gradient of the upstream layer is then reduced from these partials through the wgrad reduce table, replacing a separate act_bwd_bias pass over the full gradient tensor. This removes one full read of large activation gradients per biased conv, at the cost of extra shuffles, stores and slot bookkeeping in the epilogues, and a fallback path when the kernel layout does not match.

```diff
diff --git a/cc_amd/config.py b/cc_amd/config.py
--- a/cc_amd/config.py
+++ b/cc_amd/config.py
@@ -10,6 +10,8 @@
 grad_chunks = False
 
 bias_table = False
+
+dgrad_bias_sums = True
 
 loss_stream = True
 
diff --git a/cc_amd/csrc/conv.hip b/cc_amd/csrc/conv.hip
--- a/cc_amd/csrc/conv.hip
+++ b/cc_amd/csrc/conv.hip
@@ -205,7 +205,8 @@
 constexpr int TH = 4, TW = 32;
 
 struct CP {
-    const float* x; const float* wp; const float* zeros; const float* bias; const float* res; float* y; float* part;
+    const float* x; const float* wp; const float* zeros; const float* bias; const float* res; float* y;
+    float* part;
     int B, Cin, IH, IW; long x_bs;
     int M, Mpad, Cpad;
     int Rt, St, si, dstep, dy_base, dx_base, ymin, xmin;
@@ -528,6 +529,7 @@
     const int y_cs = g.OH * g.OW;
     if constexpr (BM == 16) {
         const int HWt = g.OHt * g.OWt;
+        float st16[4] = {0.f, 0.f, 0.f, 0.f};
 #pragma unroll
         for (int h = 0; h < 2; h++) {
             int ej, ty;
@@ -548,8 +550,22 @@
                     if (g.bias) v += g.bias[m];
                     const long o = (long)n * g.y_bs + pix + (long)m * y_cs;
                     const bool hr = g.res != nullptr;
-                    g.y[o] = conv_tail(v, hr, hr ? g.res[(long)n * g.res_bs + pix + (long)m * y_cs] : 0.f, g.res_mul, g.act, g.act_a, g.act_b,
-                                       g.add ? g.add[(long)n * g.add_bs + pix + (long)m * y_cs] : 0.f);
+                    const float out = conv_tail(v, hr, hr ? g.res[(long)n * g.res_bs + pix + (long)m * y_cs] : 0.f, g.res_mul, g.act, g.act_a,
+                                                g.act_b, g.add ? g.add[(long)n * g.add_bs + pix + (long)m * y_cs] : 0.f);
+                    g.y[o] = out;
+                    if constexpr (SPLIT != 1) st16[r] += out;
+                }
+            }
+        }
+        if constexpr (SPLIT != 1) {
+            if (g.part && !(SPLIT == 2 && g.nsplit > 1)) {
+                const int bs_np = (int)(g.part_stride & 0xffffffffl), bs_slot0 = (int)(g.part_stride >> 32);
+#pragma unroll
+                for (int r = 0; r < 4; r++) {
+                    float sv = st16[r];
+                    sv += __shfl_xor(sv, 1); sv += __shfl_xor(sv, 2); sv += __shfl_xor(sv, 4); sv += __shfl_xor(sv, 8);
+                    const int m = m0 + 4 * (lane >> 4) + r;
+                    if ((lane & 15) == 0 && m < g.M) g.part[(long)m * bs_np + bs_slot0 + bx_in * 4 + wid] = sv;
                 }
             }
         }
@@ -596,6 +612,12 @@
         return;
     }
     const bool hr = g.res != nullptr, ha = g.add != nullptr;
+    const bool bsw = g.part != nullptr;
+    float bsv[TM][4];
+#pragma unroll
+    for (int a = 0; a < TM; a++)
+#pragma unroll
+        for (int k = 0; k < 4; k++) bsv[a][k] = 0.f;
     auto tile = [&](const f32x16& A, const int a, const int b) {
         stage(A);
         int ej, ty;
@@ -624,15 +646,19 @@
 #ifdef CC_ABLATE_STORE
                     *reinterpret_cast<volatile float4*>(g.y + (long)n * g.y_bs + o) = out;
 #endif
+                    if (bsw) bsv[a][k] += (out.x + out.y) + (out.z + out.w);
                 } else {
                     const long st = g.so;
                     float* yo = g.y + (long)n * g.y_bs + o;
                     const float* ro = hr ? g.res + (long)n * g.res_bs + o : nullptr;
                     const float* ao = ha ? g.add + (long)n * g.add_bs + o : nullptr;
-                    yo[0] = conv_tail(v0, hr, hr ? ro[0] : 0.f, g.res_mul, g.act, g.act_a, g.act_b, ao ? ao[0] : 0.f);
-                    if (tx + 1 < g.OWt) yo[st] = conv_tail(v1, hr, hr ? ro[st] : 0.f, g.res_mul, g.act, g.act_a, g.act_b, ao ? ao[st] : 0.f);
-                    if (tx + 2 < g.OWt) yo[2 * st] = conv_tail(v2, hr, hr ? ro[2 * st] : 0.f, g.res_mul, g.act, g.act_a, g.act_b, ao ? ao[2 * st] : 0.f);
-                    if (tx + 3 < g.OWt) yo[3 * st] = conv_tail(v3, hr, hr ? ro[3 * st] : 0.f, g.res_mul, g.act, g.act_a, g.act_b, ao ? ao[3 * st] : 0.f);
+                    float o1 = 0.f, o2 = 0.f, o3 = 0.f;
+                    const float o0 = conv_tail(v0, hr, hr ? ro[0] : 0.f, g.res_mul, g.act, g.act_a, g.act_b, ao ? ao[0] : 0.f);
+                    yo[0] = o0;
+                    if (tx + 1 < g.OWt) yo[st] = o1 = conv_tail(v1, hr, hr ? ro[st] : 0.f, g.res_mul, g.act, g.act_a, g.act_b, ao ? ao[st] : 0.f);
+                    if (tx + 2 < g.OWt) yo[2 * st] = o2 = conv_tail(v2, hr, hr ? ro[2 * st] : 0.f, g.res_mul, g.act, g.act_a, g.act_b, ao ? ao[2 * st] : 0.f);
+                    if (tx + 3 < g.OWt) yo[3 * st] = o3 = conv_tail(v3, hr, hr ? ro[3 * st] : 0.f, g.res_mul, g.act, g.act_a, g.act_b, ao ? ao[3 * st] : 0.f);
+                    if (bsw) bsv[a][k] += (o0 + o1) + (o2 + o3);
                 }
             }
         }
@@ -643,6 +669,21 @@
     if constexpr (TM > 1) {
         tile(acc[1][0], 1, 0);
         if constexpr (TN > 1) tile(acc[1][1], 1, 1);
+    }
+    if (bsw) {
+        constexpr int WPC = (BM >= 64) ? 2 : 4;
+        const int wsub = (BM >= 64) ? (wid & 1) : wid;
+        const int bs_np = (int)(g.part_stride & 0xffffffffl), bs_slot0 = (int)(g.part_stride >> 32);
+        float* bo = g.part + bs_slot0 + bx_in * WPC + wsub;
+#pragma unroll
+        for (int a = 0; a < TM; a++)
+#pragma unroll
+            for (int k = 0; k < 4; k++) {
+                float sv = bsv[a][k];
+                sv += __shfl_xor(sv, 1); sv += __shfl_xor(sv, 2); sv += __shfl_xor(sv, 4);
+                const int m = m0 + wm * WM + a * 32 + 8 * k + rsub;
+                if ((lane & 7) == 0 && m < g.M) bo[(long)m * bs_np] = sv;
+            }
     }
 }
 
@@ -708,37 +749,66 @@
 template <int BM, int TPS>
 __global__ __launch_bounds__(256, CC_PATCH_LB) void k_conv_patch_multi_stk(CPM a) { CC_MULTI_BODY(BM, 8, TPS, 1) }
 
+struct BSum { float* p = nullptr; int np = 0, slot0 = 0, parts = 0; };
+
+__device__ __forceinline__ void splitk_bsum(float out, bool live, long e, int n, int m, int M, int HWt, float* bsum, int np, int slot0) {
+    const int lane = threadIdx.x & 63;
+    const int key = live ? n * M + m : -1;
+    float sum = live ? out : 0.f;
+#pragma unroll
+    for (int d = 1; d < 64; d <<= 1) {
+        const float t = __shfl_down(sum, d);
+        const int kt = __shfl_down(key, d);
+        if (lane + d < 64 && kt == key) sum += t;
+    }
+    const int kp = __shfl_up(key, 1);
+    if (live && (lane == 0 || kp != key)) {
+        const int P = (HWt + 63) / 64 + 1;
+        const long seg = (long)key * HWt;
+        const int piece = (int)((e >> 6) - (seg >> 6));
+        float* o = bsum + (long)m * np + slot0 + n * P;
+        o[piece] = sum;
+        if ((e >> 6) == ((seg + HWt - 1) >> 6) && piece + 2 == P) o[P - 1] = 0.f;
+    }
+}
+
 __global__ __launch_bounds__(256) void k_splitk_epilogue(const float* __restrict__ part, int nsplit, long part_stride,
                                                          const float* __restrict__ bias, const float* __restrict__ res,
                                                          float* __restrict__ y, int M, int OHt, int OWt, int so, int oy0,
                                                          int ox0, int OH, int OW, long y_bs, long res_bs, long total,
                                                          int act, float act_a, float act_b, int res_mul,
-                                                         const float* add, long add_bs, int Hp, int Wp) {
+                                                         const float* add, long add_bs, int Hp, int Wp, BSum bs) {
     const long e = (long)blockIdx.x * 256 + threadIdx.x;
-    if (e >= total) return;
+    const bool live = e < total;
+    if (!live && !bs.p) return;
     const int HWt = OHt * OWt;
     const long per = (long)M * HWt;
     const int n = (int)(e / per);
     const long r = e - (long)n * per;
     const int m = (int)(r / HWt);
-    const int t = (int)(r - (long)m * HWt);
-    const int ty = t / OWt, tx = t - ty * OWt;
-    const long po = (((long)n * M + m) * Hp + ty) * Wp + tx;
-    float v = 0.f;
-    {
-        for (int k = 0; k < nsplit; k += 8) {
-            float p8[8];
-#pragma unroll
-            for (int u = 0; u < 8; u++) p8[u] = (k + u < nsplit) ? part[(long)(k + u) * part_stride + po] : 0.f;
-#pragma unroll
-            for (int u = 0; u < 8; u++)
-                if (k + u < nsplit) v += p8[u];
-        }
-    }
-    const long o = (long)m * OH * OW + (long)(oy0 + so * ty) * OW + (ox0 + so * tx);
-    if (bias) v += bias[m];
-    y[(long)n * y_bs + o] = conv_tail(v, res != nullptr, res ? res[(long)n * res_bs + o] : 0.f, res_mul, act, act_a, act_b,
-                                      add ? add[(long)n * add_bs + o] : 0.f);
+    float out = 0.f;
+    if (live) {
+        const int t = (int)(r - (long)m * HWt);
+        const int ty = t / OWt, tx = t - ty * OWt;
+        const long po = (((long)n * M + m) * Hp + ty) * Wp + tx;
+        float v = 0.f;
+        {
+            for (int k = 0; k < nsplit; k += 8) {
+                float p8[8];
+#pragma unroll
+                for (int u = 0; u < 8; u++) p8[u] = (k + u < nsplit) ? part[(long)(k + u) * part_stride + po] : 0.f;
+#pragma unroll
+                for (int u = 0; u < 8; u++)
+                    if (k + u < nsplit) v += p8[u];
+            }
+        }
+        const long o = (long)m * OH * OW + (long)(oy0 + so * ty) * OW + (ox0 + so * tx);
+        if (bias) v += bias[m];
+        out = conv_tail(v, res != nullptr, res ? res[(long)n * res_bs + o] : 0.f, res_mul, act, act_a, act_b,
+                        add ? add[(long)n * add_bs + o] : 0.f);
+        y[(long)n * y_bs + o] = out;
+    }
+    if (bs.p) splitk_bsum(out, live, e, n, m, M, HWt, bs.p, bs.np, bs.slot0);
 }
 
 struct EPC {
@@ -748,6 +818,7 @@
     int M, so, OH, OW; long y_bs, res_bs, add_bs;
     int act; float act_a, act_b;
     int res_mul;
+    BSum bs;
 };
 struct EPM {
     EPC c[MAXCLS];
@@ -762,30 +833,50 @@
         if (q + 1 < a.n && (int)blockIdx.x >= a.bx_end[q]) { k = q + 1; first = a.bx_end[q]; }
     const EPC& c = a.c[k];
     const long e = (long)((int)blockIdx.x - first) * 256 + threadIdx.x;
-    if (e >= c.total) return;
+    const bool live = e < c.total;
+    if (!live && !c.bs.p) return;
     const int HWt = c.OHt * c.OWt;
     const long per = (long)c.M * HWt;
     const int n = (int)(e / per);
     const long r = e - (long)n * per;
     const int m = (int)(r / HWt);
-    const int t = (int)(r - (long)m * HWt);
-    const int ty = t / c.OWt, tx = t - ty * c.OWt;
-    const long po = (((long)n * c.M + m) * c.Hp + ty) * c.Wp + tx;
-    float v = 0.f;
-    {
-        for (int z = 0; z < c.nsplit; z += 8) {
-            float p8[8];
-#pragma unroll
-            for (int u = 0; u < 8; u++) p8[u] = (z + u < c.nsplit) ? c.part[(long)(z + u) * c.part_stride + po] : 0.f;
-#pragma unroll
-            for (int u = 0; u < 8; u++)
-                if (z + u < c.nsplit) v += p8[u];
-        }
-    }
-    const long o = (long)m * c.OH * c.OW + (long)(c.oy0 + c.so * ty) * c.OW + (c.ox0 + c.so * tx);
-    if (c.bias) v += c.bias[m];
-    c.y[(long)n * c.y_bs + o] = conv_tail(v, c.res != nullptr, c.res ? c.res[(long)n * c.res_bs + o] : 0.f, c.res_mul, c.act, c.act_a, c.act_b,
-                                          c.add ? c.add[(long)n * c.add_bs + o] : 0.f);
+    float out = 0.f;
+    if (live) {
+        const int t = (int)(r - (long)m * HWt);
+        const int ty = t / c.OWt, tx = t - ty * c.OWt;
+        const long po = (((long)n * c.M + m) * c.Hp + ty) * c.Wp + tx;
+        float v = 0.f;
+        {
+            for (int z = 0; z < c.nsplit; z += 8) {
+                float p8[8];
+#pragma unroll
+                for (int u = 0; u < 8; u++) p8[u] = (z + u < c.nsplit) ? c.part[(long)(z + u) * c.part_stride + po] : 0.f;
+#pragma unroll
+                for (int u = 0; u < 8; u++)
+                    if (z + u < c.nsplit) v += p8[u];
+            }
+        }
+        const long o = (long)m * c.OH * c.OW + (long)(c.oy0 + c.so * ty) * c.OW + (c.ox0 + c.so * tx);
+        if (c.bias) v += c.bias[m];
+        out = conv_tail(v, c.res != nullptr, c.res ? c.res[(long)n * c.res_bs + o] : 0.f, c.res_mul, c.act, c.act_a, c.act_b,
+                        c.add ? c.add[(long)n * c.add_bs + o] : 0.f);
+        c.y[(long)n * c.y_bs + o] = out;
+    }
+    if (c.bs.p) splitk_bsum(out, live, e, n, m, c.M, HWt, c.bs.p, c.bs.np, c.bs.slot0);
+}
+
+__global__ __launch_bounds__(256) void k_bsum_fill(const float* __restrict__ gx, long gx_bs, int B, int HW, float* __restrict__ bsum, int np) {
+    __shared__ float scratch[4];
+    const int m = (int)blockIdx.x;
+    float v[1] = {0.f};
+    for (int n = 0; n < B; n++) {
+        const float* src = gx + (long)n * gx_bs + (long)m * HW;
+        for (int i = threadIdx.x; i < HW; i += 256) v[0] += src[i];
+    }
+    cc::block_sum_256(v, scratch);
+    float* o = bsum + (long)m * np;
+    if (threadIdx.x == 0) o[0] = v[0];
+    for (int i = 1 + (int)threadIdx.x; i < np; i += 256) o[i] = 0.f;
 }
 
 
@@ -1050,9 +1141,14 @@
     }
 }
 
+inline void cp_bsum(CP& c, const BSum& b) {
+    c.part = b.p;
+    c.part_stride = ((long)b.slot0 << 32) | (long)(unsigned)b.np;
+}
 inline CP make_cp(const GG& g, const ConvPlan& p, const float* zeros, const float* wp, float* part) {
     CP c = {};
-    c.x = g.x; c.wp = wp; c.zeros = zeros; c.bias = g.bias; c.res = g.res; c.y = g.y; c.part = part;
+    c.x = g.x; c.wp = wp; c.zeros = zeros; c.bias = g.bias; c.res = g.res; c.y = g.y;
+    c.part = p.nsplit > 1 ? part : nullptr;
     c.B = g.B; c.Cin = g.Cin; c.IH = g.IH; c.IW = g.IW; c.x_bs = g.x_bs;
     c.M = g.M; c.Mpad = p.Mpad; c.Cpad = p.Cpad;
     c.Rt = g.Rt; c.St = g.St; c.si = g.si; c.dstep = g.dstep;
@@ -1062,7 +1158,7 @@
     c.y_bs = g.y_bs; c.res_bs = g.res_bs;
     c.tiles_x = p.tiles_x; c.tiles_y = p.tiles_y;
     c.nsplit = p.nsplit; c.cps = p.cps;
-    c.part_stride = (long)g.B * g.M * (p.tiles_y * (p.tw16 ? 8 : TH)) * (p.tiles_x * (p.tw16 ? 16 : TW));
+    c.part_stride = p.nsplit > 1 ? (long)g.B * g.M * (p.tiles_y * (p.tw16 ? 8 : TH)) * (p.tiles_x * (p.tw16 ? 16 : TW)) : 0;
     c.act = g.act; c.act_a = g.act_a; c.act_b = g.act_b; c.res_mul = g.res_mul;
     c.add = g.add; c.add_bs = g.add_bs;
 #ifndef CC_CONV_WMAJOR
@@ -1159,7 +1255,17 @@
     return 0;
 }
 
-inline void launch_gg(const GG& g, float* ws, hipStream_t s, const float* prepacked = nullptr, const float* pre_zeros = nullptr) {
+inline int bsum_class_parts(const GG& g, const ConvPlan& p) {
+    if (g.Cin == 0 || (p.use_patch && p.nsplit > 1)) return g.B * ((g.OHt * g.OWt + 63) / 64 + 1);
+    if (p.use_patch && !p.wino) return (int)conv_tiles(g, p) * (p.bm >= 64 ? 2 : 4);
+    if (p.use_patch && p.wino) return ccint::wino_sum_parts(p.wn);
+    return 0;
+}
+
+inline bool launch_gg(const GG& g, float* ws, hipStream_t s, const float* prepacked = nullptr, const float* pre_zeros = nullptr,
+                      const BSum* bs = nullptr) {
+    const bool want = bs && bs->p;
+    const BSum none;
     {
         ccint::HeadConv h;
         const int hk = head_kernel_of(g, h);
@@ -1171,11 +1277,13 @@
             cctiming::Scope tsc(nm, 2e-9 * g.B * g.OHt * g.OWt * (double)g.M * g.Cin * 9, s);
             if (cctools::env_flag("CC_HEAD_TRACE"))
                 fprintf(stderr, "head kernel %d: B%d M%d C%d %dx%d dstep %d\n", hk, g.B, g.M, g.Cin, g.OHt, g.OWt, g.dstep);
-            if (hk == 1 ? ccint::head_conv_thinc_launch(h, s) : ccint::head_conv_thinm_launch(h, s)) return;
+            if (hk == 1 ? ccint::head_conv_thinc_launch(h, s) : ccint::head_conv_thinm_launch(h, s)) return !want;
         }
     }
     const ConvPlan p = plan_conv(g);
-    if (!p.use_patch || ws == nullptr) { launch_gg_flat(g, s); return; }
+    if (!p.use_patch || ws == nullptr) { launch_gg_flat(g, s); return !want; }
+    const bool emit = want && bsum_class_parts(g, p) != 0 && bsum_class_parts(g, p) == bs->parts;
+    const BSum& eb = emit ? *bs : none;
     const float* zeros = ws;
     const float* wp = ws + 64;
     float* part = ws + 64 + (prepacked ? 0 : p.wp_floats);
@@ -1187,20 +1295,23 @@
         ccint::WinoGeom wg = wino_geom(g);
         if (p.wpad) wino_pad_input(g, p, part, s, pr, wg);
         bool ok;
+        ccint::WinoSums wsum = {};
+        const bool wemit = emit && p.nsplit == 1 && ccint::wino_sums_ok(wg, g.res != nullptr);
+        if (wemit) { wsum.p[0] = eb.p; wsum.np = eb.np; wsum.slot0 = eb.slot0; }
         {
             char nm[128];
             wino_scope_name(g, p, 1, nm, sizeof nm);
             cctiming::Scope tsc(nm, wino_gflop(g, p), s);
-            ok = ccint::wino_launch(wg, p.wn, &pr, 1, s);
-        }
-        if (!ok) { launch_gg_flat(g, s); return; }
+            ok = ccint::wino_launch(wg, p.wn, &pr, 1, s, wemit ? &wsum : nullptr);
+        }
+        if (!ok) { launch_gg_flat(g, s); return !want; }
         if (p.nsplit > 1) {
             const long total = (long)g.B * g.M * g.OHt * g.OWt;
             hipLaunchKernelGGL(k_splitk_epilogue, dim3((unsigned)((total + 255) / 256)), dim3(256), 0, s, (const float*)part,
                                p.nsplit, (long)g.B * g.M * p.Hp * p.Wp, g.bias, g.res, g.y, g.M, g.OHt, g.OWt, g.so, g.oy0, g.ox0, g.OH,
-                               g.OW, g.y_bs, g.res_bs, total, g.act, g.act_a, g.act_b, g.res_mul, g.add, g.add_bs, p.Hp, p.Wp);
-        }
-        return;
+                               g.OW, g.y_bs, g.res_bs, total, g.act, g.act_a, g.act_b, g.res_mul, g.add, g.add_bs, p.Hp, p.Wp, eb);
+        }
+        return (p.nsplit > 1 ? emit : wemit) || !want;
     }
     if (prepacked) {
         zeros = pre_zeros;
@@ -1209,7 +1320,8 @@
         hipLaunchKernelGGL(k_repack_w, dim3((unsigned)((p.wp_floats + 255) / 256)), dim3(256), 0, s, g.w, ws + 64, ws, g.M, g.Cin,
                            p.Mpad, p.Cpad, T, g.St, g.w_sm, g.w_sc, g.w0, g.w_ri, g.w_sj);
     }
-    const CP c = make_cp(g, p, zeros, wp, part);
+    CP c = make_cp(g, p, zeros, wp, part);
+    if (emit && p.nsplit == 1) cp_bsum(c, eb);
     dim3 grid((unsigned)conv_tiles(g, p), (unsigned)(p.Mpad / p.bm), (unsigned)p.nsplit);
     {
         char nm[96];
@@ -1226,11 +1338,12 @@
         hipLaunchKernelGGL(k_splitk_epilogue, dim3((unsigned)((total + 255) / 256)), dim3(256), 0, s, (const float*)part,
                            p.nsplit, c.part_stride, g.bias, g.res, g.y, g.M, g.OHt, g.OWt, g.so, g.oy0, g.ox0, g.OH, g.OW,
                            g.y_bs, g.res_bs, total, g.act, g.act_a, g.act_b, g.res_mul, g.add, g.add_bs,
-                           p.Hp, p.Wp);
-    }
-}
-
-struct ClsIn { GG g; ConvPlan p; const float* zeros; const float* wp; float* part; };
+                           p.Hp, p.Wp, eb);
+    }
+    return emit || !want;
+}
+
+struct ClsIn { GG g; ConvPlan p; const float* zeros; const float* wp; float* part; BSum bs; };
 
 inline size_t smem_cls(const ConvPlan& p, int tps) {
     const size_t b = (size_t)(2 * tps * p.ck * p.bm + 2 * p.ck * p.PS) * sizeof(float);
@@ -1243,8 +1356,19 @@
            a.res_mul == b.res_mul && a.dstep == b.dstep;
 }
 
-inline bool launch_classes(const ClsIn* cs, int n, hipStream_t s, bool idle_taps = false) {
+inline bool launch_classes(const ClsIn* cs, int n, hipStream_t s, bool idle_taps = false, unsigned* missed = nullptr) {
     if (n < 1 || n > MAXCLS) return false;
+    unsigned miss = 0;
+    auto epi_bsum = [&](int k, const EPC& c) -> BSum {
+        if (!cs[k].bs.p) return BSum();
+        if (bsum_class_parts(cs[k].g, cs[k].p) == cs[k].bs.parts && cs[k].bs.parts != 0) {
+            if (c.total > 0) return cs[k].bs;
+            if (!cs[k].p.wino) return BSum();
+            if (ccint::wino_sums_ok(wino_geom(cs[k].g), cs[k].g.res != nullptr)) return BSum();
+        }
+        miss |= 1u << k;
+        return BSum();
+    };
     {
         int nw = 0;
         for (int k = 0; k < n; k++) nw += cs[k].p.wino ? 1 : 0;
@@ -1274,6 +1398,7 @@
                 c.total = p.nsplit > 1 ? (long)g.B * g.M * g.OHt * g.OWt : 0;
                 c.M = g.M; c.so = g.so; c.OH = g.OH; c.OW = g.OW; c.y_bs = g.y_bs; c.res_bs = g.res_bs; c.add_bs = g.add_bs;
                 c.act = g.act; c.act_a = g.act_a; c.act_b = g.act_b; c.res_mul = g.res_mul;
+                c.bs = epi_bsum(k, c);
                 ebx += (int)((c.total + 255) / 256);
                 e.bx_end[k] = ebx;
             }
@@ -1302,9 +1427,14 @@
                 char nm[128];
                 wino_scope_name(cs[0].g, p, n, nm, sizeof nm);
                 cctiming::Scope tsc(nm, n * wino_gflop(cs[0].g, p), s);
-                if (!ccint::wino_launch(wg, p.wn, pr, n, s)) return false;
+                ccint::WinoSums wsum = {};
+                if (p.nsplit == 1)
+                    for (int k = 0; k < n; k++)
+                        if (cs[k].bs.p && !((miss >> k) & 1)) { wsum.p[k] = cs[k].bs.p; wsum.np = cs[k].bs.np; wsum.slot0 = cs[k].bs.slot0; }
+                if (!ccint::wino_launch(wg, p.wn, pr, n, s, &wsum)) return false;
             }
             if (p.nsplit > 1) hipLaunchKernelGGL(k_splitk_epilogue_multi, dim3((unsigned)ebx), dim3(256), 0, s, e);
+            if (missed) *missed = miss;
             return true;
         }
     }
@@ -1339,6 +1469,7 @@
         c.total = (empty || p.nsplit > 1) ? (long)g.B * g.M * g.OHt * g.OWt : 0;
         c.M = g.M; c.so = g.so; c.OH = g.OH; c.OW = g.OW; c.y_bs = g.y_bs; c.res_bs = g.res_bs; c.add_bs = g.add_bs;
         c.act = g.act; c.act_a = g.act_a; c.act_b = g.act_b; c.res_mul = g.res_mul;
+        c.bs = epi_bsum(k, c);
         ebx += (int)((c.total + 255) / 256);
         e.bx_end[k] = ebx;
         if (c.total) epi_any = 1;
@@ -1346,6 +1477,7 @@
         const size_t sm = smem_cls(p, tps);
         if (sm > smem) smem = sm;
         a.c[nc] = make_cp(g, p, cs[k].zeros, cs[k].wp, cs[k].part);
+        if (cs[k].bs.p && c.total == 0 && !((miss >> k) & 1)) cp_bsum(a.c[nc], cs[k].bs);
         bx += (int)conv_tiles(g, p);
         a.bx_end[nc] = bx;
         nc++;
@@ -1388,19 +1520,21 @@
         dispatch_patch(cs[ref].p.bm, cs[ref].p.ck, tps, a, grid, smem, s);
     }
     if (epi_any) hipLaunchKernelGGL(k_splitk_epilogue_multi, dim3((unsigned)ebx), dim3(256), 0, s, e);
+    if (missed) *missed = miss;
     return true;
 }
 
 inline bool launch_gg_classes(const GG* gs, int n, int mult, const float* const* zeros, const float* const* wps,
-                              float* const* parts, hipStream_t s) {
+                              float* const* parts, hipStream_t s, const BSum* bs = nullptr, unsigned* missed = nullptr) {
     if (n < 2 || n > MAXCLS || cctools::env_flag("CC_NO_CLASS_MERGE")) return false;
     ClsIn cs[MAXCLS];
     for (int k = 0; k < n; k++) {
         cs[k].g = gs[k];
         cs[k].p = plan_conv(gs[k], mult);
         cs[k].zeros = zeros[k]; cs[k].wp = wps[k]; cs[k].part = parts[k];
-    }
-    return launch_classes(cs, n, s);
+        if (bs) cs[k].bs = bs[k];
+    }
+    return launch_classes(cs, n, s, false, missed);
 }
 
 }
@@ -1593,19 +1727,86 @@
     return (size_t)G * best * sizeof(float);
 }
 
+static int dgrad_bsum_layout(int G, int B, int K, int OH, int OW, int C, int R, int S, int stride, int pad, int IH, int IW, int* cls_parts) {
+    if (G <= 0 || G > MAXCLS || B <= 0 || K <= 4 || C <= 4 || stride <= 0 || stride > 2 || R * S > 136) return 0;
+    GG gs[4];
+    ConvPlan pg[4];
+    int n = 0;
+    bool all = true;
+    for (int py = 0; py < stride; py++)
+        for (int px = 0; px < stride; px++) {
+            if (!make_dgrad_class(gs[n], py, px, nullptr, nullptr, nullptr, nullptr, B, K, OH, OW, 0, C, R, S, stride, pad, IH, IW, 0,
+                                  (long)C * R * S, (long)R * S, 0, 1.f, 0.f)) { all = false; continue; }
+            n++;
+        }
+    const int ncls = stride * stride;
+    bool merged = all && G * ncls >= 2 && G * ncls <= MAXCLS && !cctools::env_flag("CC_NO_CLASS_MERGE");
+    if (merged) {
+        int nw = 0, ref = -1, tps = 3;
+        for (int k = 0; k < n; k++) { pg[k] = plan_conv(gs[k], G); nw += pg[k].wino ? 1 : 0; }
+        if (nw) {
+            merged = nw == n;
+        } else {
+            const bool idle_taps = cctools::env_int("CC_CONV_IDLE_TAPS", 1) != 0;
+            for (int k = 0; k < n; k++) {
+                if (gs[k].Cin == 0) continue;
+                if (ref < 0) ref = k;
+                if (!pg[k].use_patch || pg[k].bm != pg[ref].bm || pg[k].ck != pg[ref].ck) merged = false;
+                if (pg[k].tps != 3 && !(idle_taps && gs[k].Rt * gs[k].St < 3 && smem_cls(pg[k], 3) <= 80 * 1024)) tps = 1;
+            }
+            for (int k = 0; k < n && merged; k++)
+                if (gs[k].Cin != 0 && smem_cls(pg[k], tps) > 80 * 1024) merged = false;
+        }
+    }
+    int tot = 0;
+    for (int k = 0; k < n; k++) {
+        const int parts = bsum_class_parts(gs[k], merged ? pg[k] : plan_conv(gs[k]));
+        if (parts == 0) return 0;
+        cls_parts[k] = parts;
+        tot += parts;
+    }
+    return tot;
+}
+
+size_t cc_conv2d_dgrad_bsum_parts(int G, int B, int K, int OH, int OW, int C, int R, int S, int stride, int pad, int IH, int IW) {
+    int cls_parts[4];
+    return (size_t)dgrad_bsum_layout(G, B, K, OH, OW, C, R, S, stride, pad, IH, IW, cls_parts);
+}
+
 static int dgrad_group_impl(int G, const long* gy, const long* w, const long* bias, const long* gx, const long* mul,
                             const long* add, float* ws, const long* prepacked, int B, int K, int OH, int OW, long gy_bs, int C,
                             int R, int S, int stride, int pad, int IH, int IW, long gx_bs, long mul_bs, long add_bs,
-                            long w_k_stride, long w_c_stride, int act, float act_a, float act_b, void* stream) {
+                            long w_k_stride, long w_c_stride, int act, float act_a, float act_b, void* stream,
+                            const long* bsum = nullptr) {
     if (G <= 0 || G > MAXCLS || B <= 0 || K <= 0 || C <= 0 || stride <= 0) return CC_ERR_ARG;
     hipStream_t s = (hipStream_t)stream;
     const size_t stride_f = cc_conv2d_dgrad_group_ws_bytes(G, B, K, OH, OW, C, R, S, stride, pad, IH, IW) / sizeof(float) / G;
+    int bs_np = 0, bs_cls[4] = {0, 0, 0, 0};
+    bool bs_any = false;
+    for (int k = 0; k < G && bsum; k++) bs_any = bs_any || bsum[k] != 0;
+    if (bs_any) {
+        bs_np = dgrad_bsum_layout(G, B, K, OH, OW, C, R, S, stride, pad, IH, IW, bs_cls);
+        if (bs_np <= 0) return CC_ERR_ARG;
+    }
+    auto class_bsum = [&](int k, int cls, int& slot0) -> BSum {
+        BSum b;
+        if (!bs_any || !bsum[k]) return b;
+        b.p = (float*)bsum[k]; b.np = bs_np; b.slot0 = slot0;
+        b.parts = bs_cls[cls];
+        slot0 += b.parts;
+        return b;
+    };
+    auto fill_missed = [&](int k) {
+        hipLaunchKernelGGL(k_bsum_fill, dim3((unsigned)C), dim3(256), 0, s, (const float*)gx[k], gx_bs, B, IH * IW, (float*)bsum[k], bs_np);
+    };
     bool packed = true;
     for (int k = 0; k < G; k++)
         if (!prepacked || !prepacked[k]) packed = false;
     const int ncls = stride * stride;
     if (packed && ws && G * ncls >= 2 && G * ncls <= MAXCLS) {
         GG gs[MAXCLS];
+        BSum bss[MAXCLS];
+        int prob_of[MAXCLS];
         const float *zeros[MAXCLS], *wps[MAXCLS];
         float* parts[MAXCLS];
         int n = 0;
@@ -1614,6 +1815,7 @@
             const float* pk = (const float*)prepacked[k];
             long off = 64;
             float* part = ws + k * stride_f + 64;
+            int slot0 = 0, cls = 0;
             for (int py = 0; py < stride && all; py++)
                 for (int px = 0; px < stride; px++) {
                     if (!make_dgrad_class(gs[n], py, px, (const float*)gy[k], (const float*)w[k],
@@ -1625,6 +1827,8 @@
                         else { gs[n].res = (const float*)add[k]; gs[n].res_bs = add_bs; gs[n].res_mul = 0; }
                     }
                     const ConvPlan p = plan_conv(gs[n], G);
+                    bss[n] = class_bsum(k, cls++, slot0);
+                    prob_of[n] = k;
                     zeros[n] = pk;
                     wps[n] = pk + off;
                     parts[n] = part;
@@ -1633,7 +1837,13 @@
                     n++;
                 }
         }
-        if (all && launch_gg_classes(gs, n, G, zeros, wps, parts, s)) {
+        unsigned missed = 0;
+        if (all && launch_gg_classes(gs, n, G, zeros, wps, parts, s, bss, &missed)) {
+            for (int k = 0; k < G; k++) {
+                bool m = false;
+                for (int j = 0; j < n; j++) m = m || (prob_of[j] == k && ((missed >> j) & 1));
+                if (m) fill_missed(k);
+            }
             CC_CHECK_LAUNCH();
             return CC_OK;
         }
@@ -1642,6 +1852,8 @@
         const float* pk = prepacked ? (const float*)prepacked[k] : nullptr;
         float* wk = ws ? ws + k * stride_f : nullptr;
         long off = 64;
+        int slot0 = 0, cls = 0;
+        bool miss = false;
         for (int py = 0; py < stride; py++) {
             for (int px = 0; px < stride; px++) {
                 GG g;
@@ -1653,20 +1865,22 @@
                     if (mul && mul[k]) { g.add = (const float*)add[k]; g.add_bs = add_bs; }
                     else { g.res = (const float*)add[k]; g.res_bs = add_bs; g.res_mul = 0; }
                 }
+                const BSum b = class_bsum(k, cls++, slot0);
                 if (g.Cin == 0) {
                     const long total = (long)g.B * g.M * g.OHt * g.OWt;
                     hipLaunchKernelGGL(k_splitk_epilogue, dim3((unsigned)((total + 255) / 256)), dim3(256), 0, s, (const float*)nullptr,
                                        0, total, g.bias, g.res, g.y, g.M, g.OHt, g.OWt, g.so, g.oy0, g.ox0, g.OH, g.OW, g.y_bs, g.res_bs,
-                                       total, g.act, g.act_a, g.act_b, g.res_mul, g.add, g.add_bs, g.OHt, g.OWt);
+                                       total, g.act, g.act_a, g.act_b, g.res_mul, g.add, g.add_bs, g.OHt, g.OWt, b);
                 } else if (pk) {
                     const ConvPlan p = plan_conv(g);
-                    launch_gg(g, wk, s, pk + off, pk);
+                    if (!launch_gg(g, wk, s, pk + off, pk, &b)) miss = true;
                     off += (long)p.wp_floats;
                 } else {
-                    launch_gg(g, wk, s);
+                    if (!launch_gg(g, wk, s, nullptr, nullptr, &b)) miss = true;
                 }
             }
         }
+        if (miss) fill_missed(k);
     }
     CC_CHECK_LAUNCH();
     return CC_OK;
@@ -1686,6 +1900,14 @@
                               int act, float act_a, float act_b, void* stream) {
     return dgrad_group_impl(G, gy, w, nullptr, gx, mul, add, ws, prepacked, B, K, OH, OW, gy_bs, C, R, S, stride, pad, IH, IW, gx_bs,
                             mul_bs, add_bs, w_k_stride, w_c_stride, act, act_a, act_b, stream);
+}
+
+int cc_conv2d_dgrad_group_add_bsum(int G, const long* gy, const long* w, const long* gx, const long* mul, const long* add,
+                                   const long* bsum, float* ws, const long* prepacked, int B, int K, int OH, int OW, long gy_bs, int C,
+                                   int R, int S, int stride, int pad, int IH, int IW, long gx_bs, long mul_bs, long add_bs,
+                                   long w_k_stride, long w_c_stride, int act, float act_a, float act_b, void* stream) {
+    return dgrad_group_impl(G, gy, w, nullptr, gx, mul, add, ws, prepacked, B, K, OH, OW, gy_bs, C, R, S, stride, pad, IH, IW, gx_bs,
+                            mul_bs, add_bs, w_k_stride, w_c_stride, act, act_a, act_b, stream, bsum);
 }
 
 int cc_conv2d_dgrad(const float* gy, const float* w, const float* bias_or_null, float* gx, float* ws,
diff --git a/cc_amd/csrc/conv_internal.h b/cc_amd/csrc/conv_internal.h
--- a/cc_amd/csrc/conv_internal.h
+++ b/cc_amd/csrc/conv_internal.h
@@ -60,7 +60,13 @@
 };
 constexpr int WINO_MAXP = 12;
 WinoPlan wino_plan(int B, int Cin, int H, int W, int M, int mult);
-bool wino_launch(const WinoGeom& g, const WinoPlan& p, const WinoProb* probs, int nprob, hipStream_t s);
+bool wino_launch(const WinoGeom& g, const WinoPlan& p, const WinoProb* probs, int nprob, hipStream_t s, const struct WinoSums* sums = nullptr);
+struct WinoSums { float* p[WINO_MAXP]; int np, slot0; };
+inline int wino_sum_parts(const WinoPlan& p) { return p.nsplit > 1 ? 0 : (p.tile ? p.nqb : 2 * p.nqb); }
+inline bool wino_sums_ok(const WinoGeom& g, bool has_res) {
+    const bool lin3 = g.act == 0 || g.act == 1 || g.act == 2;
+    return g.res_mul ? (has_res && (g.act == 1 || g.act == 2)) : lin3;
+}
 void wino_weights_launch(const float* w, float* U, int M, int Cin, int Cpad, int Mpad, long w_sm, long w_sc, long w0, long w_ri,
                          long w_sj, int flip, hipStream_t s);
 
diff --git a/cc_amd/csrc/wgrad_reduce.hip b/cc_amd/csrc/wgrad_reduce.hip
--- a/cc_amd/csrc/wgrad_reduce.hip
+++ b/cc_amd/csrc/wgrad_reduce.hip
@@ -5,6 +5,7 @@
 namespace {
 
 constexpr int NRD = 32;
+constexpr int K4_WIDE = 512;
 
 struct RD {
     const float* ws; float* gw;
@@ -98,6 +99,22 @@
                 put(o + tt, s, d.accum);
             }
         }
+    } else if (d.kind == 4 && d.nsplit > K4_WIDE) {
+        const int m = bid, lane = threadIdx.x & 63, wv = threadIdx.x >> 6;
+        const float* __restrict__ w = ws + (long)m * d.nsplit;
+        float s = 0.f;
+        for (int k = threadIdx.x; k < d.nsplit; k += 8 * 256) {
+            float v[8];
+#pragma unroll
+            for (int u = 0; u < 8; u++) v[u] = (k + 256 * u < d.nsplit) ? w[k + 256 * u] : 0.f;
+#pragma unroll
+            for (int u = 0; u < 8; u++) s += v[u];
+        }
+        s = cc::wave_sum(s);
+        float* red = reinterpret_cast<float*>(&part[0][0]);
+        if (lane == 0) red[wv] = s;
+        __syncthreads();
+        if (threadIdx.x == 0) put(d.gw + m, (red[0] + red[1]) + (red[2] + red[3]), d.accum);
     } else if (d.kind == 4) {
         const int m = bid * 4 + (threadIdx.x >> 6), lane = threadIdx.x & 63;
         if (m < d.p[0]) {
@@ -154,7 +171,7 @@
         case 0: return h[13] ? (h[7] * h[8] / 4 + 255) / 256 : (h[7] * h[8] + 255) / 256;
         case 1: return (h[8] * h[10] + 255) / 256;
         case 2: return h[15] * h[7] * 4;
-        case 4: return (h[7] + 3) / 4;
+        case 4: return h[3] > K4_WIDE ? h[7] : (h[7] + 3) / 4;
         default: return -1;
     }
 }
diff --git a/cc_amd/csrc/wino.hip b/cc_amd/csrc/wino.hip
--- a/cc_amd/csrc/wino.hip
+++ b/cc_amd/csrc/wino.hip
@@ -36,10 +36,19 @@
 constexpr int RROW = 12 * 4, RCH = 4 * RROW, RWAVE = 4 * RCH;
 constexpr int WTHREADS = 512;
 
-enum { EPI_LIN = 0, EPI_GRAD = 1, EPI_GEN = 2 };
-
-template <int SPLIT, int EPI, int ABL>
+enum { EPI_LIN = 0, EPI_GRAD = 1, EPI_GEN = 2, EPI_GRAD_BS = 3, EPI_LIN_BS = 4 };
+constexpr int epi_form(int e) { return e == EPI_GRAD_BS ? EPI_GRAD : (e == EPI_LIN_BS ? EPI_LIN : e); }
+
+__device__ __forceinline__ float half_wave_sum(float v) {
+#pragma unroll
+    for (int m = 16; m >= 1; m >>= 1) v += __shfl_xor(v, m);
+    return v;
+}
+
+template <int SPLIT, int EPIX, int ABL>
 __global__ __launch_bounds__(WTHREADS, 2) void k_wino_f2x3(WN g) {
+    constexpr int EPI = epi_form(EPIX);
+    constexpr bool BS = EPIX != EPI;
     HIP_DYNAMIC_SHARED(float, smem)
     float* Us = smem;
     float* Vs = smem + 2 * UBLK;
@@ -277,6 +286,13 @@
     const int oy = 2 * ty, ox = 2 * tx;
     const int m_base = mb * WBM + wm * 32 + 4 * lk;
     const bool hr = P.res != nullptr, ha = P.add != nullptr;
+    float* bsum = nullptr;
+    int bslot = 0, bs_np = 0;
+    if constexpr (BS) {
+        bs_np = (int)(g.part_stride & 0xffffffffl);
+        bsum = P.part;
+        bslot = (int)(g.part_stride >> 32) + qb * 2 + wt;
+    }
     const bool row1 = oy + 1 < g.H;
     const long o0 = (long)oy * g.W + ox;
     const int odd_lane = lane & 1;
@@ -375,9 +391,49 @@
             v.y = tail(v.y + bv, res_r[r8].y, add_r[r8].y);
             v.z = tail(v.z + bv, res_r[r8].z, add_r[r8].z);
             v.w = tail(v.w + bv, res_r[r8].w, add_r[r8].w);
-            if (qv && row_ok && m < g.M) *reinterpret_cast<float4*>(yb + (long)m * g.HW) = v;
+            const bool st_ok = qv && row_ok && m < g.M;
+            if (st_ok) *reinterpret_cast<float4*>(yb + (long)m * g.HW) = v;
+            if constexpr (BS) {
+                if (bsum) {
+                    const float sv = half_wave_sum(st_ok ? (v.x + v.y) + (v.z + v.w) : 0.f);
+                    if (l31 == 0 && m < g.M) bsum[(long)m * bs_np + bslot] = sv;
+                }
+            }
         }
         return;
+    }
+    if constexpr (BS) {
+        if (bsum) {
+            const bool col1 = ox + 1 < g.W;
+#pragma unroll
+            for (int r8 = 0; r8 < 8; r8++) {
+                const int r = 8 * fh + r8;
+                float y00, y01, y10, y11;
+                out_tile(r8, y00, y01, y10, y11);
+                const int m = m_base + (r & 3) + 8 * (r >> 2);
+                const bool ok = qv && m < g.M;
+                float sv = 0.f;
+                if (ok) {
+                    const float bv = P.bias ? P.bias[m] : 0.f;
+                    const long o = (long)m * g.HW + o0;
+                    float* yo = P.y + (long)n * g.y_bs + o;
+                    const float* ro = hr ? P.res + (long)n * g.res_bs + o : nullptr;
+                    const float* ao = ha ? P.add + (long)n * g.add_bs + o : nullptr;
+                    float o01 = 0.f, o10 = 0.f, o11 = 0.f;
+                    const float o00 = tail(y00 + bv, hr ? ro[0] : 0.f, ha ? ao[0] : 0.f);
+                    yo[0] = o00;
+                    if (col1) yo[1] = o01 = tail(y01 + bv, hr ? ro[1] : 0.f, ha ? ao[1] : 0.f);
+                    if (row1) {
+                        yo[g.W] = o10 = tail(y10 + bv, hr ? ro[g.W] : 0.f, ha ? ao[g.W] : 0.f);
+                        if (col1) yo[g.W + 1] = o11 = tail(y11 + bv, hr ? ro[g.W + 1] : 0.f, ha ? ao[g.W + 1] : 0.f);
+                    }
+                    sv = (o00 + o01) + (o10 + o11);
+                }
+                sv = half_wave_sum(sv);
+                if (l31 == 0 && m < g.M) bsum[(long)m * bs_np + bslot] = sv;
+            }
+            return;
+        }
     }
     if (!qv) return;
     const bool col1 = ox + 1 < g.W;
@@ -407,8 +463,10 @@
 constexpr int VBLK_S = 16 * WCK * SBT;
 constexpr int SHALF = 2 * UBLK_S + 2 * VBLK_S + 4 * RWAVE;
 
-template <int KS, int SPLIT, int EPI>
+template <int KS, int SPLIT, int EPIX>
 __global__ __launch_bounds__(256 * KS, 2) void k_wino_f2x3_s(WN g) {
+    constexpr int EPI = epi_form(EPIX);
+    constexpr bool BS = EPIX != EPI;
     HIP_DYNAMIC_SHARED(float, smem)
     const int tid = threadIdx.x, lane = tid & 63;
     const int wid = __builtin_amdgcn_readfirstlane(tid >> 6);
@@ -617,6 +675,13 @@
     const int oy = 2 * ty, ox = 2 * tx;
     const int m_base = mb * SBM + 4 * lk + 8 * fr + RPW * kh;
     const bool hr = P.res != nullptr, ha = P.add != nullptr;
+    float* bsum = nullptr;
+    int bslot = 0, bs_np = 0;
+    if constexpr (BS) {
+        bs_np = (int)(g.part_stride & 0xffffffffl);
+        bsum = P.part;
+        bslot = (int)(g.part_stride >> 32) + qb;
+    }
     const bool row1 = oy + 1 < g.H;
     const long o0 = (long)oy * g.W + ox;
     const int odd_lane = lane & 1;
@@ -714,9 +779,48 @@
             v.y = tail(v.y + bv, res_r[rr].y, add_r[rr].y);
             v.z = tail(v.z + bv, res_r[rr].z, add_r[rr].z);
             v.w = tail(v.w + bv, res_r[rr].w, add_r[rr].w);
-            if (qv && row_ok && m < g.M) *reinterpret_cast<float4*>(yb + (long)m * g.HW) = v;
+            const bool st_ok = qv && row_ok && m < g.M;
+            if (st_ok) *reinterpret_cast<float4*>(yb + (long)m * g.HW) = v;
+            if constexpr (BS) {
+                if (bsum) {
+                    const float sv = half_wave_sum(st_ok ? (v.x + v.y) + (v.z + v.w) : 0.f);
+                    if (l31 == 0 && m < g.M) bsum[(long)m * bs_np + bslot] = sv;
+                }
+            }
         }
         return;
+    }
+    if constexpr (BS) {
+        if (bsum) {
+            const bool col1 = ox + 1 < g.W;
+#pragma unroll
+            for (int rr = 0; rr < RPW; rr++) {
+                float y00, y01, y10, y11;
+                out_tile(rr, y00, y01, y10, y11);
+                const int m = m_base + rr;
+                const bool ok = qv && m < g.M;
+                float sv = 0.f;
+                if (ok) {
+                    const float bv = P.bias ? P.bias[m] : 0.f;
+                    const long o = (long)m * g.HW + o0;
+                    float* yo = P.y + (long)n * g.y_bs + o;
+                    const float* ro = hr ? P.res + (long)n * g.res_bs + o : nullptr;
+                    const float* ao = ha ? P.add + (long)n * g.add_bs + o : nullptr;
+                    float o01 = 0.f, o10 = 0.f, o11 = 0.f;
+                    const float o00 = tail(y00 + bv, hr ? ro[0] : 0.f, ha ? ao[0] : 0.f);
+                    yo[0] = o00;
+                    if (col1) yo[1] = o01 = tail(y01 + bv, hr ? ro[1] : 0.f, ha ? ao[1] : 0.f);
+                    if (row1) {
+                        yo[g.W] = o10 = tail(y10 + bv, hr ? ro[g.W] : 0.f, ha ? ao[g.W] : 0.f);
+                        if (col1) yo[g.W + 1] = o11 = tail(y11 + bv, hr ? ro[g.W + 1] : 0.f, ha ? ao[g.W + 1] : 0.f);
+                    }
+                    sv = (o00 + o01) + (o10 + o11);
+                }
+                sv = half_wave_sum(sv);
+                if (l31 == 0 && m < g.M) bsum[(long)m * bs_np + bslot] = sv;
+            }
+            return;
+        }
     }
     if (!qv) return;
     const bool col1 = ox + 1 < g.W;
@@ -822,7 +926,7 @@
                        w0, w_ri, w_sj, flip);
 }
 
-bool wino_launch(const WinoGeom& gg, const WinoPlan& p, const WinoProb* probs, int nprob, hipStream_t s) {
+bool wino_launch(const WinoGeom& gg, const WinoPlan& p, const WinoProb* probs, int nprob, hipStream_t s, const WinoSums* sums) {
     const long xfl = ((long)gg.B - 1) * gg.x_bs + (long)gg.Cin * gg.H * gg.W;
     if ((gg.x_bs % 4) != 0 || xfl * 4 >= (long)CC_BUF_OOB) return false;
     for (int k = 0; k < nprob; k++)
@@ -854,8 +958,17 @@
     const size_t smem = p.tile ? (size_t)SHALF * p.tile * sizeof(float) : (size_t)(2 * UBLK + 2 * VBLK + 8 * RWAVE) * sizeof(float);
     dim3 grid((unsigned)(((a.total + 7) / 8) * 8), 1, (unsigned)p.nsplit);
     const bool grad = gg.res_mul != 0;
-    const int epi = (!grad && (gg.act == ACT_NONE || gg.act == ACT_RELU || gg.act == ACT_LRELU)) ? EPI_LIN
-                    : (grad && probs[0].res && (gg.act == ACT_RELU || gg.act == ACT_LRELU)) ? EPI_GRAD : EPI_GEN;
+    int epi = (!grad && (gg.act == ACT_NONE || gg.act == ACT_RELU || gg.act == ACT_LRELU)) ? EPI_LIN
+              : (grad && probs[0].res && (gg.act == ACT_RELU || gg.act == ACT_LRELU)) ? EPI_GRAD : EPI_GEN;
+    if (sums && p.nsplit == 1 && epi != EPI_GEN) {
+        bool any = false;
+        for (int k = 0; k < nprob; k++) any = any || sums->p[k] != nullptr;
+        if (any) {
+            for (int k = 0; k < nprob; k++) a.p[k].part = sums->p[k];
+            a.part_stride = ((long)sums->slot0 << 32) | (long)(unsigned)sums->np;
+            epi = epi == EPI_GRAD ? EPI_GRAD_BS : EPI_LIN_BS;
+        }
+    }
     auto go = [&](auto kern, bool& attr) {
         if (!attr) {
             (void)hipFuncSetAttribute(reinterpret_cast<const void*>(kern), hipFuncAttributeMaxDynamicSharedMemorySize, 160 * 1024);
@@ -863,9 +976,9 @@
         }
         hipLaunchKernelGGL(kern, grid, dim3(WTHREADS), smem, s, a);
     };
-    static bool attr_set[4] = {false, false, false, false};
+    static bool attr_set[6] = {false, false, false, false, false, false};
     if (p.tile) {
-        static bool attr_s[2][4] = {};
+        static bool attr_s[2][6] = {};
         const unsigned nth = 256u * (unsigned)p.tile;
         auto gos = [&](auto kern, bool& attr) {
             if (!attr) {
@@ -878,11 +991,15 @@
             if (p.nsplit > 1 || (p.nchunk & 1)) return false;
             if (epi == EPI_LIN) gos(k_wino_f2x3_s<2, 0, EPI_LIN>, attr_s[1][0]);
             else if (epi == EPI_GRAD) gos(k_wino_f2x3_s<2, 0, EPI_GRAD>, attr_s[1][1]);
+            else if (epi == EPI_GRAD_BS) gos(k_wino_f2x3_s<2, 0, EPI_GRAD_BS>, attr_s[1][4]);
+            else if (epi == EPI_LIN_BS) gos(k_wino_f2x3_s<2, 0, EPI_LIN_BS>, attr_s[1][5]);
             else gos(k_wino_f2x3_s<2, 0, EPI_GEN>, attr_s[1][2]);
         } else {
             if (p.nsplit > 1) gos(k_wino_f2x3_s<1, 1, 0>, attr_s[0][3]);
             else if (epi == EPI_LIN) gos(k_wino_f2x3_s<1, 0, EPI_LIN>, attr_s[0][0]);
             else if (epi == EPI_GRAD) gos(k_wino_f2x3_s<1, 0, EPI_GRAD>, attr_s[0][1]);
+            else if (epi == EPI_GRAD_BS) gos(k_wino_f2x3_s<1, 0, EPI_GRAD_BS>, attr_s[0][4]);
+            else if (epi == EPI_LIN_BS) gos(k_wino_f2x3_s<1, 0, EPI_LIN_BS>, attr_s[0][5]);
             else gos(k_wino_f2x3_s<1, 0, EPI_GEN>, attr_s[0][2]);
         }
         return true;
@@ -910,6 +1027,8 @@
     if (p.nsplit > 1) go(k_wino_f2x3<1, 0, 0>, attr_set[3]);
     else if (epi == EPI_LIN) go(k_wino_f2x3<0, EPI_LIN, 0>, attr_set[0]);
     else if (epi == EPI_GRAD) go(k_wino_f2x3<0, EPI_GRAD, 0>, attr_set[1]);
+    else if (epi == EPI_GRAD_BS) go(k_wino_f2x3<0, EPI_GRAD_BS, 0>, attr_set[4]);
+    else if (epi == EPI_LIN_BS) go(k_wino_f2x3<0, EPI_LIN_BS, 0>, attr_set[5]);
     else go(k_wino_f2x3<0, EPI_GEN, 0>, attr_set[2]);
     return true;
 }
diff --git a/cc_amd/tape.py b/cc_amd/tape.py
--- a/cc_amd/tape.py
+++ b/cc_amd/tape.py
@@ -62,9 +62,11 @@
 NET_DONE = None
 NET_MARK = None
 TAPS = None
+BSUM_TRACE = None
+
 
 class TT:
-    __slots__ = ("t", "act", "act_a", "act_b", "uses", "remaining", "grad", "pend", "pre", "needs", "tapname")
+    __slots__ = ("t", "act", "act_a", "act_b", "uses", "remaining", "grad", "pend", "pre", "needs", "tapname", "want_bsum", "bsum", "nosum")
 
     def __init__(self, t, needs=True, act=0, act_a=1.0, act_b=0.0):
         assert t.dtype == torch.float32 and (t.dim() != 4 or _dense(t)), (tuple(t.shape), t.stride())
@@ -77,6 +79,9 @@
         self.pre = False
         self.needs = needs
         self.tapname = None
+        self.want_bsum = False
+        self.bsum = None
+        self.nosum = None
 
     def skip(self):
         self.remaining -= 1
@@ -119,9 +124,11 @@
         self._fold_extra_pend()
         add = self.grad if self.grad is not None else (self.pend.pop() if self.pend else None)
         last = can_mul and self.remaining == 0 and self.act != 0
+        sums = (config.dgrad_bias_sums and self.want_bsum and can_mul and self.remaining == 0 and (last or self.act == 0)
+                and not self.pend)
         if self.grad is None:
             self.grad = _new(self.t.shape, self.t)
-        launch(self.grad, add, self.t if last else None)
+        launch(self.grad, add, self.t if last else None, sums)
         if last:
             self.pre = True
 
@@ -306,6 +313,20 @@
                 self.E.call("cc_act_bwd_bias_group", *args, STREAM)
         return geffs if act != 0 else list(gs)
 
+    def _bias_from_sums(self, tt, bias, C):
+        buf, parts = tt.bsum
+        gb, acc = self._param_grad(bias)
+        desc = [4, buf.data_ptr(), gb.data_ptr(), parts, int(acc), 0, 0, C] + [0] * 8
+        if acc and ops.wgrad_queue.enabled and not ops._dbg.no_wgrad_defer:
+            if gb.data_ptr() in ops.wgrad_reduces.targets:
+                ops.wgrad_reduces._cur().flush()
+            ops.wgrad_reduces.targets.add(gb.data_ptr())
+            ops.wgrad_reduces.keep.append((buf, gb))
+            ops.wgrad_reduces.desc.extend(desc)
+        else:
+            arr = (ctypes.c_long * 16)(*desc)
+            self.E.call("cc_wgrad_reduce_table", ctypes.addressof(arr), 1, STREAM)
+
     def _wgrad(self, a_list, x_list, w_list, geom):
         B, M, AH, AW, Cin, IH, IW, R, S, si, pad, o_sm, o_sc = geom
         live = [k for k, w in enumerate(w_list) if w.requires_grad]
@@ -364,6 +385,9 @@
             for k in range(G):
                 launch([k])
         youts = [self._tt(y, act=act, act_a=float(act_a), act_b=float(act_b)) for y in ys]
+        if has_bias:
+            for k in range(G):
+                youts[k].want_bsum = bool(bs[k] is not None and bs[k].requires_grad)
         self._use(*xs)
         if residuals is not None:
             self._use(*residuals)
@@ -382,8 +406,17 @@
             if not live:
                 return
             gz = {}
+            for k in live:
+                if youts[k].bsum is not None and (fin[k][1] or act == 0) and fin[k][0] is youts[k].grad:
+                    self._bias_from_sums(youts[k], bs[k], Cout)
+                    gz[k] = fin[k][0]
+            if BSUM_TRACE is not None and has_bias:
+                for k in live:
+                    if k not in gz and (fin[k][1] or act == 0) and bs[k].requires_grad:
+                        BSUM_TRACE.append((tuple(fin[k][0].shape), ("kernel without sums: " + youts[k].nosum) if youts[k].nosum else
+                                           "the last contribution is not a data-gradient launch" if config.dgrad_bias_sums else "switch off"))
             for pre in (False, True):
-                idx = [k for k in live if fin[k][1] == pre]
+                idx = [k for k in live if fin[k][1] == pre and k not in gz]
                 if idx:
                     ge = self._act_bias([fin[k][0] for k in idx], [youts[k].t for k in idx], 0 if pre else act, act_a, act_b,
                                         [bs[k] for k in idx] if has_bias else None, xs_[0].t)
@@ -395,12 +428,13 @@
             dgeom = (B, Cout, OH, OW, Cin, R, S, stride, pad, IH, IW)
             plan = {}
             for k in live:
-                xs_[k].from_conv(lambda gx, add, mul, k=k: plan.__setitem__(k, (gx, add, mul)))
+                xs_[k].from_conv(lambda gx, add, mul, sums, k=k: plan.__setitem__(k, (gx, add, mul, sums)))
             todo = [k for k in live if k in plan]
             groups, last = [], {}
             for k in todo:
                 sg = (plan[k][1] is not None, plan[k][2] is not None, _bs(gz[k]), _bs(plan[k][0]),
-                      _bs(plan[k][1]) if plan[k][1] is not None else 0, _bs(xs_[k].t), xs_[k].act, xs_[k].act_a, xs_[k].act_b)
+                      _bs(plan[k][1]) if plan[k][1] is not None else 0, _bs(xs_[k].t), xs_[k].act, xs_[k].act_a, xs_[k].act_b,
+                      plan[k][3])
                 tgt = plan[k][0].data_ptr()
                 first = last.get(tgt, -1) + 1
                 for gi in range(first, len(groups)):
@@ -420,10 +454,24 @@
                 a4 = ops._parr([plan[k][2] for k in idx]) if has_mul else None
                 a5 = ops._parr([plan[k][1] for k in idx]) if has_add else None
                 a6 = ops._parr(pks)
-                E.call("cc_conv2d_dgrad_group_add", n, ops._addr(a1), ops._addr(a2), ops._addr(a3), ops._addr(a4) if has_mul else 0,
-                       ops._addr(a5) if has_add else 0, wsb, ops._addr(a6), B, Cout, OH, OW, sg[2], Cin, R, S, stride, pad, IH, IW,
-                       sg[3], sg[5] if has_mul else 0, sg[4], Cin * R * S, R * S, sg[6] if has_mul else 0,
-                       sg[7] if has_mul else 1.0, sg[8] if has_mul else 0.0, STREAM)
+                tail = (wsb, ops._addr(a6), B, Cout, OH, OW, sg[2], Cin, R, S, stride, pad, IH, IW,
+                        sg[3], sg[5] if has_mul else 0, sg[4], Cin * R * S, R * S, sg[6] if has_mul else 0,
+                        sg[7] if has_mul else 1.0, sg[8] if has_mul else 0.0, STREAM)
+                parts = E.call("cc_conv2d_dgrad_bsum_parts", n, *dgeom) if sg[9] else 0
+                if sg[9] and not parts and BSUM_TRACE is not None:
+                    nm = ctypes.create_string_buffer(160)
+                    E.call("cc_conv2d_dgrad_kernel", *dgeom, int(pks[0] is not None), ctypes.addressof(nm), 160)
+                    for k in idx:
+                        xs_[k].nosum = nm.value.decode()
+                if parts:
+                    for k in idx:
+                        xs_[k].bsum = (torch.empty(Cin * parts, device=xs_[k].t.device, dtype=torch.float32), parts)
+                    a7 = ops._parr([xs_[k].bsum[0] for k in idx])
+                    E.call("cc_conv2d_dgrad_group_add_bsum", n, ops._addr(a1), ops._addr(a2), ops._addr(a3),
+                           ops._addr(a4) if has_mul else 0, ops._addr(a5) if has_add else 0, ops._addr(a7), *tail)
+                else:
+                    E.call("cc_conv2d_dgrad_group_add", n, ops._addr(a1), ops._addr(a2), ops._addr(a3),
+                           ops._addr(a4) if has_mul else 0, ops._addr(a5) if has_add else 0, *tail)
             self._wgrad([gz[k] for k in live], [xs_[k].t for k in live], [ws_[k] for k in live],
                         (B, Cout, OH, OW, Cin, IH, IW, R, S, stride, pad, Cin * R * S, R * S))
 
@@ -453,9 +501,11 @@
             if g is None:
                 x.skip()
                 return
+            if BSUM_TRACE is not None and (pre or act == 0) and b is not None and b.requires_grad:
+                BSUM_TRACE.append((tuple(g.shape), "bias of a transposed convolution (its tensor asks for no sums)"))
             gz = self._act_bias([g], [yt.t], 0 if pre else act, 1.0, act_b, [b] if b is not None else None, x.t)[0]
 
-            def launch(gx, add, mul):
+            def launch(gx, add, mul, sums=False):
                 fgeom = (B, Cout, OH, OW, Cin, R, S, stride, pad, IH, IW)
                 ws2 = ops._ws(E.call("cc_conv2d_fwd_ws_bytes", *fgeom), x.t)
                 pk2 = ops.packs.get("fwd", w, fgeom)
@@ -674,7 +724,7 @@
         assert self.record
         for tt in self.tts:
             tt.remaining = tt.uses
-            tt.grad, tt.pend, tt.pre = None, [], False
+            tt.grad, tt.pend, tt.pre, tt.bsum, tt.nosum = None, [], False, None, None
         for o, g in zip(outputs, grads):
             if g is not None:
                 o.pend.append(g if (g.dim() != 4 or _dense(g)) else g.contiguous())
diff --git a/include/ccengine.h b/include/ccengine.h
--- a/include/ccengine.h
+++ b/include/ccengine.h
@@ -147,6 +147,11 @@
                               const long* prepacked, int B, int K, int OH, int OW, long gy_bs, int C, int R, int S, int stride,
                               int pad, int IH, int IW, long gx_bs, long mul_bs, long add_bs, long w_k_stride, long w_c_stride,
                               int act, float act_a, float act_b, void* stream);
+size_t cc_conv2d_dgrad_bsum_parts(int G, int B, int K, int OH, int OW, int C, int R, int S, int stride, int pad, int IH, int IW);
+int cc_conv2d_dgrad_group_add_bsum(int G, const long* gy, const long* w, const long* gx, const long* mul, const long* add,
+                                   const long* bsum, float* ws, const long* prepacked, int B, int K, int OH, int OW, long gy_bs, int C,
+                                   int R, int S, int stride, int pad, int IH, int IW, long gx_bs, long mul_bs, long add_bs,
+                                   long w_k_stride, long w_c_stride, int act, float act_a, float act_b, void* stream);
 int cc_conv2d_wgrad_group(int G, const long* a, const long* x, const long* gw, float* ws, int B, int M, int AH, int AW, long a_bs,
                           int Cin, int IH, int IW, long x_bs, int R, int S, int si, int pad, long o_sm, long o_sc, int accumulate,
                           void* stream);
```

Result: no change. 248.3 images/s (-0.2%).
